# uzh-rpg/rpg_ramnet

Measured on AMD Instinct MI355X. Metric: depth samples/sec (346x260 cropped to 256x344, 5-bin grids, K=5 grids + 1 frame per sample; training step), higher is better.
Workload: dtype f32; 1 GPU; EventScape-shaped 346x260 -> 256x344 crop, 5 event bins, K=5, batch 8/GPU, seq-len 8, 1xMI355X-per-rank train, state=convgru, SI loss on [image,events4], Adam, backward-weights co-scheduled on a side stream, decoders on a second stream; global_batch=8, seq_len=8, parallelism=dp1

## Files before the change

include/ramnet_hip.h:

```cpp
#ifndef RAMNET_HIP_H
#define RAMNET_HIP_H
#include <stddef.h>
#include <stdint.h>

#ifdef __cplusplus
extern "C" {
#endif

#define RAMNET_ABI_VERSION 27
#define RAMNET_E_BADARG 10001
#define RAMNET_E_UNSUPPORTED 10002

enum ramnet_in_mode {
    RAMNET_IN_PLAIN = 0,
    RAMNET_IN_CAT = 1,
    RAMNET_IN_CAT_MUL = 2,
    RAMNET_IN_UP2X = 3,
    RAMNET_IN_UP2X_SKIP = 4,
    RAMNET_IN_RELUMASK = 5,
    RAMNET_IN_S2D = 6,
    RAMNET_IN_PARITY4 = 7
};

enum ramnet_algo { RAMNET_ALGO_DIRECT = 0, RAMNET_ALGO_WINOGRAD = 1, RAMNET_ALGO_HEAD = 2, RAMNET_ALGO_WINOGRAD24 = 3, RAMNET_ALGO_WINOGRAD_2X4 = 4,
                   RAMNET_ALGO_WINOGRAD_2X4_SPLIT = 5, RAMNET_ALGO_DIRECT_SPLIT = 6, RAMNET_ALGO_WINOGRAD24_2X3 = 7 };

enum ramnet_epilogue {
    RAMNET_EPI_LINEAR = 0,
    RAMNET_EPI_RELU = 1,
    RAMNET_EPI_SIGMOID = 2,
    RAMNET_EPI_RES_RELU = 3,
    RAMNET_EPI_GRU_BLEND = 4,
    RAMNET_EPI_LSTM = 5,
    RAMNET_EPI_GRU_BWD = 6,
    RAMNET_EPI_SIGMOID_HR = 7
};

typedef struct ramnet_conv_desc {
    const float *x0, *x1, *xm;
    int ld0, ld1, ldm;
    int C0, C1;
    int in_mode;
    int B, Hin, Win;
    int ntaps, stride;
    int8_t dy[25], dx[25];
    uint8_t wtap[25];
    const float *w;
    const float *bias;
    int Cout;
    int Ho, Wo;
    int HoF, WoF;
    int osy, osx, ooy, oox;
    int epi;
    float beta;
    const float *e0, *e1;
    int lde0, lde1;
    float *out, *o1, *o2;
    int ldo, ldo1, ldo2;
    int algo;
    int frame;
    int out_s2d;
    int head_cin;
    int s2d_5x5;
    float *splitk_ws;
    size_t splitk_floats;
    const int *active;
} ramnet_conv_desc;

#define RAMNET_WGRAD_MAX_SEGMENTS 48
typedef struct ramnet_wgrad_seg {
    const float *x0, *x1, *xm, *dout, *gmask;
} ramnet_wgrad_seg;

typedef struct ramnet_wgrad_desc {
    const float *x0, *x1, *xm;
    int ld0, ld1, ldm, C0, C1, in_mode;
    int B, Hin, Win;
    int ntaps, stride;
    int8_t dy[25], dx[25];
    const float *dout, *gmask;
    int ldg, ldgm;
    int Cout, Ho, Wo;
    float *dw;
    float *dbias;
    int algo;
    int gsy, gsx, goy, gox;
    int HoG, WoG;
    int head_cin;
    int dw_slabs;
    int nseg;
    const ramnet_wgrad_seg *segs;
} ramnet_wgrad_desc;

int ramnet_set_option(const char *name, int value);
int ramnet_get_option(const char *name);
const char *ramnet_last_error(void);
int ramnet_abi_version(void);
const char *ramnet_last_kernel(void);
int ramnet_stream_fork(void *from, void *to);

int ramnet_gemm(const float *A, const float *B, float *C, int M, int N, int K, int lda, int ldb, int ldc, int trans_a,
                int accumulate, int batch, long stride_a, long stride_b, long stride_c, void *stream);
int ramnet_gemm2(const float *A, const float *B, float *C, int M, long stride_a, long stride_b, long stride_c, int batch, const float *A2,
                 const float *B2, float *C2, int M2, long stride_a2, long stride_b2, long stride_c2, int batch2, int N, int K, int K2, int lda,
                 int ldb, int ldc, int trans_a, int accumulate, void *stream);

size_t ramnet_gemm_partial_floats(int M, int N, int K, int batch, int M2, int K2, int batch2);
int ramnet_gemm_ordered(const float *A, const float *B, float *C, int M, int N, int K, int lda, int ldb, int ldc, int trans_a, int batch,
                        long stride_a, long stride_b, long stride_c, float *partial, void *stream);
int ramnet_gemm2_ordered(const float *A, const float *B, float *C, int M, long stride_a, long stride_b, long stride_c, int batch, const float *A2,
                         const float *B2, float *C2, int M2, long stride_a2, long stride_b2, long stride_c2, int batch2, int N, int K, int K2,
                         int lda, int ldb, int ldc, int trans_a, float *partial, void *stream);

int ramnet_nchw_to_nhwc_pad(const float *src, float *dst, int B, int C, int H, int W, int Cpad, void *stream);
int ramnet_reflect_pad(const float *src, float *dst, int B, int C, int H, int W, int Cpad, int top, int left, int Hc, int Wc, int nhwc,
                       void *stream);
int ramnet_wgrad_wino_slabs(int Cin, int Cout);
int ramnet_wgrad_wino2x4_slabs(int Cin, int Cout);
int ramnet_wgrad_dsplit_slabs(int Cin, int Cout);
#define RAMNET_WGRAD_SLAB_CAP 64
int ramnet_wgrad_slabs(const ramnet_wgrad_desc *d);
size_t ramnet_wgrad_dsplit_ws_floats(int Cin, int Cout);
int ramnet_unpack_wgrad_dsplit(const float *ws, float *grad, int Cout, int Cin, int CinWs, int CoutWs, int n_off, void *stream);
size_t ramnet_wgrad_wino2x4_ws_floats(int Cin, int Cout);
int ramnet_reduce_slabs(float *ws, int slabs, size_t n, void *stream);
size_t ramnet_packed_weight_elems(int Cout, int Cin, int KH, int KW, int transposed, int gates);
size_t ramnet_packed_weight_elems_wino(int Cout, int Cin, int transposed, int gates);
int ramnet_pack_weight_wino(const float *w_oihw, float *wp, int Cout, int Cin, int transposed, int gates, void *stream);
size_t ramnet_packed_weight_elems_wino2x4(int Cout, int Cin, int transposed);
int ramnet_pack_weight_wino2x4(const float *w_oihw, float *wp, int Cout, int Cin, int transposed, void *stream);
size_t ramnet_packed_weight_elems_wino2x4_gates(int Cout, int Cin, int transposed, int gates);
int ramnet_pack_weight_wino2x4_gates(const float *w_oihw, float *wp, int Cout, int Cin, int transposed, int gates, void *stream);
int ramnet_conv_wino_variant(const ramnet_conv_desc *d, int force);
int ramnet_conv_wino_split_ok(const ramnet_conv_desc *d, int force);
size_t ramnet_packed_weight_elems_wino2x4_split(int Cout, int Cin, int transposed);
int ramnet_pack_weight_wino2x4_split(const float *w_oihw, float *wp, int Cout, int Cin, int transposed, void *stream);
size_t ramnet_conv_splitk_floats(const ramnet_conv_desc *d);
int ramnet_wino2x4_config(int min_wgs);
int ramnet_fold_wino_supported(int Cout, int Cin);
size_t ramnet_packed_weight_elems_fold_wino(int Cout, int Cin);
int ramnet_pack_weight_fold_wino(const float *w_oihw, float *wp, int Cout, int Cin, void *stream);
int ramnet_pack_weight_fold_wino_dgrad(const float *w_oihw, float *wp, int Cout, int Cin, void *stream);
int ramnet_pack_border_weights(const float *w_oihw, float *rows, float *cols, float *rows_t, float *cols_t, int Cout, int Cin, void *stream);
int ramnet_fold_wino_variant(const ramnet_conv_desc *d, int force);
size_t ramnet_packed_weight_elems_fold_wino2x3(int Cout, int Cin);
int ramnet_pack_weight_fold_wino2x3(const float *w_oihw, float *wp, int Cout, int Cin, void *stream);
int ramnet_pack_weight_fold_wino2x3_dgrad(const float *w_oihw, float *wp, int Cout, int Cin, void *stream);
int ramnet_fold_unpack_wgrad(float *w4, float *dU, float *wr, float *wc, float *grad, int Cout, int Cin, int CinWs, void *stream);
int ramnet_fold_wgrad_variant(const ramnet_wgrad_desc *d, int force);
int ramnet_fold_unpack_wgrad2x3(float *w4, float *dU, float *dU3, float *wr, float *wc, float *grad, int Cout, int Cin, int CinWs, void *stream);
size_t ramnet_packed_weight_elems_head(int Cin);
int ramnet_head_supported(int Cin, int Cout);
int ramnet_pack_weight_head(const float *w_oihw, float *wp, int Cout, int Cin, void *stream);
int ramnet_pack_weight(const float *w_oihw, float *wp, int Cout, int Cin, int KH, int KW,
                       int transposed, int gates, void *stream);
int ramnet_unpack_wgrad(const float *ws, float *grad_oihw, int Cout, int Cin, int CinWs, int CoutWs, int n_off,
                        int KH, int KW, void *stream);

int ramnet_unpack_wgrad_wino(const float *ws, float *grad_oihw, int Cout, int Cin, int CinWs, int CoutWs, int n_off,
                             void *stream);
int ramnet_unpack_wgrad_wino2x4(const float *ws, float *grad_oihw, int Cout, int Cin, int CinWs, int CoutWs, int n_off,
                                void *stream);

int ramnet_conv_launch(const ramnet_conv_desc *d, void *stream);
int ramnet_conv_launch_multi(const ramnet_conv_desc *descs, int n, void *stream);
int ramnet_wgrad_launch(const ramnet_wgrad_desc *d, void *stream);

int ramnet_pred_sigmoid_fwd(const float *x, int ldx, int C, const float *w, const float *b, float *y,
                            size_t npix, void *stream);
int ramnet_pred_sigmoid_bwd(const float *x, int ldx, int C, const float *w, const float *y, const float *dy,
                            float *dx, int lddx, float *dw, float *db, size_t npix, void *stream);
#define RAMNET_PRED_SI_MAX_SEGMENTS 8
size_t ramnet_pred_si_scratch_doubles(size_t seg_pix, int nseg);
int ramnet_pred_sigmoid_si_fwd(const float *x, int ldx, int C, const float *w, const float *b, float *y, size_t seg_pix, int nseg,
                               const float *const *targets, float weight, float lambda, double *scratch, double *stats, float *loss,
                               void *stream);
int ramnet_pred_sigmoid_si_bwd(const float *x, int ldx, int C, const float *w, const float *y, const float *dy, size_t seg_pix, int nseg,
                               const float *const *targets, const double *stats, const float *gscale, float weight, float lambda,
                               float *dx, int lddx, float *dw, float *db, double *scratch, int mask_x, void *stream);
int ramnet_pred_linear_fwd(const float *x, int ldx, int C, const float *w, const float *b, float *z, size_t npix, void *stream);
int ramnet_pred_linear_bwd(const float *x, int ldx, int C, const float *w, const float *dz, float *dx, int lddx, float *dw, float *db,
                           size_t npix, void *stream);
int ramnet_pred_sigmoid_dgrad(int C, const float *w, const float *y, const float *dy, float *dx, int lddx, size_t npix, void *stream);
int ramnet_pred_linear_dgrad(int C, const float *w, const float *dz, float *dx, int lddx, size_t npix, void *stream);
int ramnet_pred_sigmoid_si_dgrad(const float *x, int ldx, int C, const float *w, const float *y, const float *dy, size_t seg_pix, int nseg,
                                 const float *const *targets, const double *stats, const float *gscale, float weight, float lambda,
                                 float *dx, int lddx, int mask_x, void *stream);
int ramnet_relu_bwd(const float *dy, const float *y, float *dx, size_t n, void *stream);
int ramnet_pad2_sum(const float *x, const float *skip, float *out, int B, int H, int W, int C, void *stream);
int ramnet_up2x_border_im2col(const float *x, const float *skip, float *rows, float *cols, int B, int H, int W, int C, void *stream);
int ramnet_pad2_sum_im2col(const float *x, const float *skip, float *out, float *rows, float *cols, int B, int H, int W, int C, void *stream);
int ramnet_unpad2_fold(const float *dxpad, float *dx, int B, int H, int W, int C, void *stream);
int ramnet_up2x_border_col2im(const float *rows, const float *cols, float *dx, int B, int H, int W, int C, void *stream);
int ramnet_frame_gather(const float *dy, const float *mask, float *rows, float *cols, int B, int H2, int W2, int C, void *stream);
int ramnet_space_to_depth2(const float *x, float *out, int B, int H, int W, int C, int inverse, void *stream);
int ramnet_upsample2x_bwd(const float *dup, float *dx, int B, int H, int W, int C, void *stream);
int ramnet_gru_bwd_a(const float *dhn, const float *ur, const float *o, const float *h, float *dpo,
                     float *dpur, float *dh, size_t npix, int C, int ld_dhn ,
                     void *stream);
int ramnet_gru_bwd_a2(const float *dhn, const float *ur, const float *o, const float *h, float *dpo,
                      float *dpur, float *dh, size_t npix, int C, int ld_dhn, int ld_dh ,
                      void *stream);
int ramnet_gru_bwd_b(const float *dxhr, const float *ur, const float *h, float *dpur, float *dh,
                     size_t npix, int C, void *stream);
int ramnet_lstm_bwd(const float *gates, const float *cprev, const float *cnew, const float *dhn,
                    const float *dcn, float *dpre, float *dcprev, size_t npix, int C, void *stream);
int ramnet_lstm_bwd_masked(const float *gates, const float *cprev, const float *cnew, const float *dhn, const float *dcn,
                           const int *active, float *dpre, float *dcprev, float *dxh, size_t npix, int hw, int C, void *stream);
int ramnet_bias_grad(const float *dy, const float *mask, float *db, size_t npix, int C, void *stream);
size_t ramnet_bias_grad_partial_floats(int C);
int ramnet_bias_grad_ordered(const float *dy, const float *mask, float *db, size_t npix, int C, float *partial, void *stream);
size_t ramnet_pred_bwd_partial_floats(void);
int ramnet_pred_sigmoid_bwd_ordered(const float *x, int ldx, int C, const float *w, const float *y, const float *dy, float *dx, int lddx,
                                    float *dw, float *db, size_t npix, float *partial, void *stream);
int ramnet_pred_linear_bwd_ordered(const float *x, int ldx, int C, const float *w, const float *dz, float *dx, int lddx, float *dw, float *db,
                                   size_t npix, float *partial, void *stream);
int ramnet_norm_slabs(int groups, long npix, int C);
int ramnet_norm_partial(const float *a, int lda, const float *y, int ldy, int act, const float *b, int ldb, int groups, long npix,
                        int C, int nslab, double *part, void *stream);
int ramnet_norm_finalize(const double *part, int groups, int nslab, int C, long npix, double eps, const float *gamma, const float *beta,
                         float *running_mean, float *running_var, double momentum, int update_running, int use_running,
                         long long *num_batches_tracked, double *mean, double *rstd, float *scale, float *shift, void *stream);
int ramnet_norm_finalize_bwd(const double *part, int groups, int nslab, int C, long npix, const double *mean, const double *rstd,
                             const float *gamma, int batch_stats, float *c1, float *c2, float *c3, float *dgamma, float *dbeta, void *stream);
int ramnet_norm_apply(const float *x, int ldx, const float *scale, const float *shift, const float *res, int ldr, int act, float *out,
                      int ldo, int groups, long npix, int C, void *stream);
int ramnet_norm_bwd(const float *dy, int lddy, const float *y, int ldy, int act, const float *x, int ldx, const float *c1, const float *c2,
                    const float *c3, float *dx, int lddx, float *dres, int lddres, int groups, long npix, int C, void *stream);
int ramnet_add(const float *a, const float *b, float *y, size_t n, void *stream);
int ramnet_concat2(const float *a, int lda, int Ca, const float *b, int ldb, int Cb, float *y, size_t npix, void *stream);
int ramnet_cat_batch_add(const float *const *parts, int n, size_t npix, int C, int ld, const float *base, float *out, void *stream);
int ramnet_cat_batch_add_masked(const float *const *parts, int n, size_t npix, int C, int ld, const float *base, const float *mask, float *out,
                                void *stream);
int ramnet_split2(const float *y, int ldy, int Ca, int Cb, float *a, float *b, size_t npix, void *stream);

int ramnet_si_loss_fwd(const float *pred, const float *target, size_t n, float weight, float lambda,
                       double *stats, float *loss, void *stream);
int ramnet_si_loss_from_stats(const double *stats, float weight, float lambda, float *loss, void *stream);
int ramnet_si_loss_bwd(const float *pred, const float *target, size_t n, float weight, float lambda,
                       const double *stats, const float *gscale, float *dpred, void *stream);

int ramnet_si_log_loss_fwd(const float *pred, const float *target, size_t n, float lambda, double *stats, float *loss, void *stream);
int ramnet_si_log_loss_bwd(const float *pred, const float *target, size_t n, float lambda, const double *stats, const float *gscale,
                           float *dpred, void *stream);
int ramnet_mse_loss_fwd(const float *pred, const float *target, int B, int H, int W, int half, double *stats, float *loss, void *stream);
int ramnet_mse_loss_bwd(const float *pred, const float *target, int B, int H, int W, int half, const double *stats, const float *gscale,
                        float *dpred, void *stream);

int ramnet_depth_metrics(const float *pred, const float *target, size_t n, float clip_distance, float reg_factor,
                         float cutoff, double *out11, void *stream);

size_t ramnet_msg_workspace_elems(int B, int H, int W, int num_scales);
int ramnet_msg_loss_fwd(const float *pred, const float *target, int B, int H, int W, int num_scales, float *ws,
                        double *stats, float *loss, void *stream);
int ramnet_msg_loss_bwd(const float *ws, const double *stats, const float *gscale, int B, int H, int W, int num_scales,
                        float *dws, float *dpred, void *stream);

int ramnet_voxelize(const double *events, size_t n_events, int bins, int W, int H, float *grid, void *stream);
int ramnet_voxel_indices(const double *events, size_t n_events, int bins, int W, int H,
                         long long *idx_left, long long *idx_right, void *stream);
int ramnet_normalize_nonzero(float *grid, size_t n, double *scratch, void *stream);
int ramnet_voxelize_batch(const double *events, const long long *offsets, int n_grids, size_t max_events, int bins, int W, int H,
                          float *grids, void *stream);
int ramnet_normalize_nonzero_batch(float *grids, int n_grids, size_t n, double *scratch, void *stream);
int ramnet_nonzero_stats_batch(const float *grids, int n_grids, size_t n, double *stats, void *stream);

int ramnet_voxelize_batch_sorted(const double *events, const long long *offsets, int n_grids, size_t max_events, int bins, int W, int H,
                                 float *grids, void *stream);
size_t ramnet_nonzero_stats_scratch_doubles(int n_grids, size_t n);
int ramnet_nonzero_stats_batch_ordered(const float *grids, int n_grids, size_t n, double *stats, double *scratch, void *stream);
int ramnet_normalize_nonzero_batch_ordered(float *grids, int n_grids, size_t n, double *stats, double *scratch, void *stream);
int ramnet_normalize_nonzero_ordered(float *grid, size_t n, double *stats, double *scratch, void *stream);

int ramnet_augment_batch(const float *const *src, float *const *dst, const int *pidx, const float *theta, const int *win,
                         const int *win_host, const double *stats, const float *bx, const float *by, int G, int n_params, int C,
                         int H, int W, int th, int tw, int Cpad, int nhwc, void *stream);

#define RAMNET_BATCH_METRICS_TICKET_BYTES 262144
size_t ramnet_batch_metrics_workspace(int G, int N, size_t npix);
int ramnet_batch_metrics(const float *const *pred, const float *const *target, int G, int N, size_t npix, void *workspace,
                         double *out, void *stream);

#define RAMNET_EVAL_TABLE_TICKET_BYTES 262144
int ramnet_metric_depth(const float *y, size_t n, float clip_distance, float reg_factor, int clamp, float *out, void *stream);
size_t ramnet_eval_table_workspace(int G, size_t npix, int ncut, int has_mask);
int ramnet_eval_table(const float *const *pred, const float *const *target, const unsigned char *const *mask, int G, size_t npix,
                      float clip_distance, float reg_factor, const float *cutoffs, int ncut, void *workspace, double *out, void *stream);
#define RAMNET_EVAL_RESCALE 1
#define RAMNET_EVAL_TARGET_METRIC 2
size_t ramnet_eval_table_ex_workspace(int G, size_t npix, int ncut, int has_mask, int flags);
int ramnet_eval_table_ex(const float *const *pred, const float *const *target, const unsigned char *const *mask, int G, size_t npix,
                         float clip_distance, float reg_factor, const float *cutoffs, int ncut, int flags, void *workspace, double *out,
                         void *stream);
int ramnet_resize_metric_target(const float *const *target, int G, int H, int W, double scale_factor, float clip_distance, float reg_factor,
                                float *out, void *stream);

int ramnet_fill_pointer_table(const void **table, const void *const *host_ptrs, int n, void *stream);
size_t ramnet_grad_loss_workspace(int G, int B, int H, int W);
int ramnet_grad_loss_stats(const float *const *pred, const float *const *target, int G, int B, int H, int W, int num_scales,
                           void *workspace, double *stats, const float *weights, float *loss, float *wsum, void *stream);
int ramnet_grad_loss_from_stats(const double *stats, int G, int num_scales, double Bg, const double *Bg_dev, const float *weights,
                                float *loss, float *wsum, void *stream);
int ramnet_grad_loss_bwd(const float *const *pred, const float *const *target, int G, int B, int H, int W, int num_scales,
                         const double *stats, double Bg, const double *Bg_dev, double gain, const float *weights, const float *up,
                         const float *up_sum, float *dpred, void *stream);

#define RAMNET_RENDER_TICKET_BYTES 262144
#define RAMNET_RENDER_EVENTS 0
#define RAMNET_RENDER_FRAME 1
size_t ramnet_render_depth_workspace(int G, int n_scale, size_t npix);
int ramnet_render_depth(const float *const *maps, int G, int H, int W, double vmin, double vmax, const unsigned char *lut,
                        const float *const *scale_pred, const float *const *scale_target, int n_scale, float clip_distance,
                        float reg_factor, void *workspace, unsigned char *grey, unsigned char *color, double *scale, void *stream);
int ramnet_least_squares_scale(const float *const *pred, const float *const *target, int G, size_t npix, float clip_distance,
                               float reg_factor, void *workspace, double *scale, void *stream);
int ramnet_render_inputs(const float *const *inputs, const int *channels, const int *kinds, int G, int H, int W, unsigned char *rgb,
                         void *stream);

#ifdef __cplusplus
}
#endif
#endif
```

rpg_ramnet_amd/_hip.py:

```python
import ctypes as C
import os

_PKG = os.path.dirname(os.path.abspath(__file__))
LIB_PATH = os.environ.get("RAMNET_HIP_LIB") or os.path.join(_PKG, "librpg_ramnet_hip.so")

IN_PLAIN, IN_CAT, IN_CAT_MUL, IN_UP2X, IN_UP2X_SKIP, IN_RELUMASK, IN_S2D, IN_PARITY4 = range(8)
ALGO_DIRECT, ALGO_WINOGRAD, ALGO_HEAD, ALGO_WINOGRAD24, ALGO_WINOGRAD_2X4, ALGO_WINOGRAD_2X4_SPLIT, ALGO_DIRECT_SPLIT = 0, 1, 2, 3, 4, 5, 6
ALGO_WINOGRAD24_2X3 = 7
EPI_LINEAR, EPI_RELU, EPI_SIGMOID, EPI_RES_RELU, EPI_GRU_BLEND, EPI_LSTM, EPI_GRU_BWD, EPI_SIGMOID_HR = range(8)

_fp = C.c_void_p


class ConvDesc(C.Structure):
    _fields_ = [
        ("x0", _fp), ("x1", _fp), ("xm", _fp),
        ("ld0", C.c_int), ("ld1", C.c_int), ("ldm", C.c_int),
        ("C0", C.c_int), ("C1", C.c_int), ("in_mode", C.c_int),
        ("B", C.c_int), ("Hin", C.c_int), ("Win", C.c_int),
        ("ntaps", C.c_int), ("stride", C.c_int),
        ("dy", C.c_int8 * 25), ("dx", C.c_int8 * 25), ("wtap", C.c_uint8 * 25),
        ("w", _fp), ("bias", _fp),
        ("Cout", C.c_int), ("Ho", C.c_int), ("Wo", C.c_int), ("HoF", C.c_int), ("WoF", C.c_int),
        ("osy", C.c_int), ("osx", C.c_int), ("ooy", C.c_int), ("oox", C.c_int),
        ("epi", C.c_int), ("beta", C.c_float),
        ("e0", _fp), ("e1", _fp), ("lde0", C.c_int), ("lde1", C.c_int),
        ("out", _fp), ("o1", _fp), ("o2", _fp),
        ("ldo", C.c_int), ("ldo1", C.c_int), ("ldo2", C.c_int),
        ("algo", C.c_int),
        ("frame", C.c_int),
        ("out_s2d", C.c_int),
        ("head_cin", C.c_int),
        ("s2d_5x5", C.c_int),
        ("splitk_ws", C.c_void_p), ("splitk_floats", C.c_size_t),
        ("active", _fp),
    ]


class WgradSeg(C.Structure):
    _fields_ = [("x0", _fp), ("x1", _fp), ("xm", _fp), ("dout", _fp), ("gmask", _fp)]


WGRAD_MAX_SEGMENTS = 48


class WgradDesc(C.Structure):
    _fields_ = [
        ("x0", _fp), ("x1", _fp), ("xm", _fp),
        ("ld0", C.c_int), ("ld1", C.c_int), ("ldm", C.c_int),
        ("C0", C.c_int), ("C1", C.c_int), ("in_mode", C.c_int),
        ("B", C.c_int), ("Hin", C.c_int), ("Win", C.c_int),
        ("ntaps", C.c_int), ("stride", C.c_int),
        ("dy", C.c_int8 * 25), ("dx", C.c_int8 * 25),
        ("dout", _fp), ("gmask", _fp), ("ldg", C.c_int), ("ldgm", C.c_int),
        ("Cout", C.c_int), ("Ho", C.c_int), ("Wo", C.c_int),
        ("dw", _fp), ("dbias", _fp),
        ("algo", C.c_int),
        ("gsy", C.c_int), ("gsx", C.c_int), ("goy", C.c_int), ("gox", C.c_int), ("HoG", C.c_int), ("WoG", C.c_int),
        ("head_cin", C.c_int),
        ("dw_slabs", C.c_int),
        ("nseg", C.c_int), ("segs", C.POINTER(WgradSeg)),
    ]


_SIGS = {
    "ramnet_abi_version": (C.c_int, []),
    "ramnet_last_error": (C.c_char_p, []),
    "ramnet_set_option": (C.c_int, [C.c_char_p, C.c_int]),
    "ramnet_get_option": (C.c_int, [C.c_char_p]),
    "ramnet_last_kernel": (C.c_char_p, []),
    "ramnet_stream_fork": (C.c_int, [_fp, _fp]),
    "ramnet_gemm": (C.c_int, [_fp, _fp, _fp] + [C.c_int] * 9 + [C.c_long] * 3 + [_fp]),
    "ramnet_gemm2": (C.c_int, [_fp, _fp, _fp, C.c_int, C.c_long, C.c_long, C.c_long, C.c_int, _fp, _fp, _fp, C.c_int, C.c_long, C.c_long, C.c_long,
                               C.c_int, C.c_int, C.c_int, C.c_int, C.c_int, C.c_int, C.c_int, C.c_int, C.c_int, _fp]),
    "ramnet_nchw_to_nhwc_pad": (C.c_int, [_fp, _fp, C.c_int, C.c_int, C.c_int, C.c_int, C.c_int, _fp]),
    "ramnet_reflect_pad": (C.c_int, [_fp, _fp] + [C.c_int] * 10 + [_fp]),
    "ramnet_wgrad_wino_slabs": (C.c_int, [C.c_int, C.c_int]),
    "ramnet_wgrad_wino2x4_slabs": (C.c_int, [C.c_int, C.c_int]),
    "ramnet_wgrad_dsplit_slabs": (C.c_int, [C.c_int, C.c_int]),
    "ramnet_wgrad_dsplit_ws_floats": (C.c_size_t, [C.c_int, C.c_int]),
    "ramnet_unpack_wgrad_dsplit": (C.c_int, [_fp, _fp, C.c_int, C.c_int, C.c_int, C.c_int, C.c_int, _fp]),
    "ramnet_wgrad_wino2x4_ws_floats": (C.c_size_t, [C.c_int, C.c_int]),
    "ramnet_reduce_slabs": (C.c_int, [_fp, C.c_int, C.c_size_t, _fp]),
    "ramnet_packed_weight_elems": (C.c_size_t, [C.c_int] * 6),
    "ramnet_pack_weight": (C.c_int, [_fp, _fp, C.c_int, C.c_int, C.c_int, C.c_int, C.c_int, C.c_int, _fp]),
    "ramnet_packed_weight_elems_wino": (C.c_size_t, [C.c_int] * 4),
    "ramnet_pack_weight_wino": (C.c_int, [_fp, _fp, C.c_int, C.c_int, C.c_int, C.c_int, _fp]),
    "ramnet_packed_weight_elems_wino2x4": (C.c_size_t, [C.c_int] * 3),
    "ramnet_pack_weight_wino2x4": (C.c_int, [_fp, _fp, C.c_int, C.c_int, C.c_int, _fp]),
    "ramnet_packed_weight_elems_wino2x4_gates": (C.c_size_t, [C.c_int] * 4),
    "ramnet_pack_weight_wino2x4_gates": (C.c_int, [_fp, _fp, C.c_int, C.c_int, C.c_int, C.c_int, _fp]),
    "ramnet_wino2x4_config": (C.c_int, [C.c_int]),
    "ramnet_conv_wino_variant": (C.c_int, [C.POINTER(ConvDesc), C.c_int]),
    "ramnet_conv_wino_split_ok": (C.c_int, [C.POINTER(ConvDesc), C.c_int]),
    "ramnet_packed_weight_elems_wino2x4_split": (C.c_size_t, [C.c_int] * 3),
    "ramnet_pack_weight_wino2x4_split": (C.c_int, [_fp, _fp, C.c_int, C.c_int, C.c_int, _fp]),
    "ramnet_conv_splitk_floats": (C.c_size_t, [C.POINTER(ConvDesc)]),
    "ramnet_packed_weight_elems_head": (C.c_size_t, [C.c_int]),
    "ramnet_head_supported": (C.c_int, [C.c_int, C.c_int]),
    "ramnet_pack_weight_head": (C.c_int, [_fp, _fp, C.c_int, C.c_int, _fp]),
    "ramnet_fold_wino_supported": (C.c_int, [C.c_int, C.c_int]),
    "ramnet_packed_weight_elems_fold_wino": (C.c_size_t, [C.c_int, C.c_int]),
    "ramnet_pack_weight_fold_wino": (C.c_int, [_fp, _fp, C.c_int, C.c_int, _fp]),
    "ramnet_pack_weight_fold_wino_dgrad": (C.c_int, [_fp, _fp, C.c_int, C.c_int, _fp]),
    "ramnet_fold_wino_variant": (C.c_int, [C.POINTER(ConvDesc), C.c_int]),
    "ramnet_packed_weight_elems_fold_wino2x3": (C.c_size_t, [C.c_int, C.c_int]),
    "ramnet_pack_weight_fold_wino2x3": (C.c_int, [_fp, _fp, C.c_int, C.c_int, _fp]),
    "ramnet_pack_weight_fold_wino2x3_dgrad": (C.c_int, [_fp, _fp, C.c_int, C.c_int, _fp]),
    "ramnet_pack_border_weights": (C.c_int, [_fp] * 5 + [C.c_int, C.c_int, _fp]),
    "ramnet_fold_unpack_wgrad": (C.c_int, [_fp] * 5 + [C.c_int, C.c_int, C.c_int, _fp]),
    "ramnet_fold_unpack_wgrad2x3": (C.c_int, [_fp] * 6 + [C.c_int, C.c_int, C.c_int, _fp]),
    "ramnet_unpad2_fold": (C.c_int, [_fp, _fp, C.c_int, C.c_int, C.c_int, C.c_int, _fp]),
    "ramnet_up2x_border_col2im": (C.c_int, [_fp, _fp, _fp, C.c_int, C.c_int, C.c_int, C.c_int, _fp]),
    "ramnet_pad2_sum": (C.c_int, [_fp, _fp, _fp, C.c_int, C.c_int, C.c_int, C.c_int, _fp]),
    "ramnet_up2x_border_im2col": (C.c_int, [_fp, _fp, _fp, _fp, C.c_int, C.c_int, C.c_int, C.c_int, _fp]),
    "ramnet_pad2_sum_im2col": (C.c_int, [_fp, _fp, _fp, _fp, _fp, C.c_int, C.c_int, C.c_int, C.c_int, _fp]),
    "ramnet_space_to_depth2": (C.c_int, [_fp, _fp, C.c_int, C.c_int, C.c_int, C.c_int, C.c_int, _fp]),
    "ramnet_frame_gather": (C.c_int, [_fp, _fp, _fp, _fp, C.c_int, C.c_int, C.c_int, C.c_int, _fp]),
    "ramnet_unpack_wgrad": (C.c_int, [_fp, _fp] + [C.c_int] * 7 + [_fp]),
    "ramnet_unpack_wgrad_wino": (C.c_int, [_fp, _fp] + [C.c_int] * 5 + [_fp]),
    "ramnet_unpack_wgrad_wino2x4": (C.c_int, [_fp, _fp] + [C.c_int] * 5 + [_fp]),
    "ramnet_conv_launch": (C.c_int, [C.POINTER(ConvDesc), _fp]),
    "ramnet_conv_launch_multi": (C.c_int, [C.POINTER(ConvDesc), C.c_int, _fp]),
    "ramnet_wgrad_launch": (C.c_int, [C.POINTER(WgradDesc), _fp]),
    "ramnet_fold_wgrad_variant": (C.c_int, [C.POINTER(WgradDesc), C.c_int]),
    "ramnet_pred_sigmoid_fwd": (C.c_int, [_fp, C.c_int, C.c_int, _fp, _fp, _fp, C.c_size_t, _fp]),
    "ramnet_pred_sigmoid_bwd": (C.c_int, [_fp, C.c_int, C.c_int, _fp, _fp, _fp, _fp, C.c_int, _fp, _fp, C.c_size_t, _fp]),
    "ramnet_pred_si_scratch_doubles": (C.c_size_t, [C.c_size_t, C.c_int]),
    "ramnet_pred_sigmoid_si_fwd": (C.c_int, [_fp, C.c_int, C.c_int, _fp, _fp, _fp, C.c_size_t, C.c_int, C.POINTER(C.c_void_p), C.c_float, C.c_float,
                                             _fp, _fp, _fp, _fp]),
    "ramnet_pred_sigmoid_si_bwd": (C.c_int, [_fp, C.c_int, C.c_int, _fp, _fp, _fp, C.c_size_t, C.c_int, C.POINTER(C.c_void_p), _fp, _fp, C.c_float,
                                             C.c_float, _fp, C.c_int, _fp, _fp, _fp, C.c_int, _fp]),
    "ramnet_pred_linear_fwd": (C.c_int, [_fp, C.c_int, C.c_int, _fp, _fp, _fp, C.c_size_t, _fp]),
    "ramnet_pred_linear_bwd": (C.c_int, [_fp, C.c_int, C.c_int, _fp, _fp, _fp, C.c_int, _fp, _fp, C.c_size_t, _fp]),
    "ramnet_pred_sigmoid_dgrad": (C.c_int, [C.c_int, _fp, _fp, _fp, _fp, C.c_int, C.c_size_t, _fp]),
    "ramnet_pred_linear_dgrad": (C.c_int, [C.c_int, _fp, _fp, _fp, C.c_int, C.c_size_t, _fp]),
    "ramnet_pred_sigmoid_si_dgrad": (C.c_int, [_fp, C.c_int, C.c_int, _fp, _fp, _fp, C.c_size_t, C.c_int, C.POINTER(C.c_void_p), _fp, _fp, C.c_float,
                                               C.c_float, _fp, C.c_int, C.c_int, _fp]),
    "ramnet_cat_batch_add": (C.c_int, [_fp, C.c_int, C.c_size_t, C.c_int, C.c_int, _fp, _fp, _fp]),
    "ramnet_cat_batch_add_masked": (C.c_int, [_fp, C.c_int, C.c_size_t, C.c_int, C.c_int, _fp, _fp, _fp, _fp]),
    "ramnet_relu_bwd": (C.c_int, [_fp, _fp, _fp, C.c_size_t, _fp]),
    "ramnet_upsample2x_bwd": (C.c_int, [_fp, _fp, C.c_int, C.c_int, C.c_int, C.c_int, _fp]),
    "ramnet_gru_bwd_a": (C.c_int, [_fp] * 7 + [C.c_size_t, C.c_int, C.c_int, _fp]),
    "ramnet_gru_bwd_a2": (C.c_int, [_fp] * 7 + [C.c_size_t, C.c_int, C.c_int, C.c_int, _fp]),
    "ramnet_gru_bwd_b": (C.c_int, [_fp] * 5 + [C.c_size_t, C.c_int, _fp]),
    "ramnet_lstm_bwd": (C.c_int, [_fp] * 7 + [C.c_size_t, C.c_int, _fp]),
    "ramnet_lstm_bwd_masked": (C.c_int, [_fp, _fp, _fp, _fp, _fp, _fp, _fp, _fp, _fp, C.c_size_t, C.c_int, C.c_int, _fp]),
    "ramnet_norm_slabs": (C.c_int, [C.c_int, C.c_long, C.c_int]),
    "ramnet_norm_partial": (C.c_int, [_fp, C.c_int, _fp, C.c_int, C.c_int, _fp, C.c_int, C.c_int, C.c_long, C.c_int, C.c_int, _fp, _fp]),
    "ramnet_norm_finalize": (C.c_int, [_fp, C.c_int, C.c_int, C.c_int, C.c_long, C.c_double, _fp, _fp, _fp, _fp, C.c_double, C.c_int, C.c_int,
                                       _fp, _fp, _fp, _fp, _fp, _fp]),
    "ramnet_norm_finalize_bwd": (C.c_int, [_fp, C.c_int, C.c_int, C.c_int, C.c_long, _fp, _fp, _fp, C.c_int, _fp, _fp, _fp, _fp, _fp, _fp]),
    "ramnet_norm_apply": (C.c_int, [_fp, C.c_int, _fp, _fp, _fp, C.c_int, C.c_int, _fp, C.c_int, C.c_int, C.c_long, C.c_int, _fp]),
    "ramnet_norm_bwd": (C.c_int, [_fp, C.c_int, _fp, C.c_int, C.c_int, _fp, C.c_int, _fp, _fp, _fp, _fp, C.c_int, _fp, C.c_int,
                                  C.c_int, C.c_long, C.c_int, _fp]),
    "ramnet_add": (C.c_int, [_fp, _fp, _fp, C.c_size_t, _fp]),
    "ramnet_split2": (C.c_int, [_fp, C.c_int, C.c_int, C.c_int, _fp, _fp, C.c_size_t, _fp]),
    "ramnet_concat2": (C.c_int, [_fp, C.c_int, C.c_int, _fp, C.c_int, C.c_int, _fp, C.c_size_t, _fp]),
    "ramnet_bias_grad": (C.c_int, [_fp, _fp, _fp, C.c_size_t, C.c_int, _fp]),
    "ramnet_si_loss_fwd": (C.c_int, [_fp, _fp, C.c_size_t, C.c_float, C.c_float, _fp, _fp, _fp]),
    "ramnet_si_loss_from_stats": (C.c_int, [_fp, C.c_float, C.c_float, _fp, _fp]),
    "ramnet_si_loss_bwd": (C.c_int, [_fp, _fp, C.c_size_t, C.c_float, C.c_float, _fp, _fp, _fp, _fp]),
    "ramnet_si_log_loss_fwd": (C.c_int, [_fp, _fp, C.c_size_t, C.c_float, _fp, _fp, _fp]),
    "ramnet_si_log_loss_bwd": (C.c_int, [_fp, _fp, C.c_size_t, C.c_float, _fp, _fp, _fp, _fp]),
    "ramnet_mse_loss_fwd": (C.c_int, [_fp, _fp, C.c_int, C.c_int, C.c_int, C.c_int, _fp, _fp, _fp]),
    "ramnet_mse_loss_bwd": (C.c_int, [_fp, _fp, C.c_int, C.c_int, C.c_int, C.c_int, _fp, _fp, _fp, _fp]),
    "ramnet_depth_metrics": (C.c_int, [_fp, _fp, C.c_size_t, C.c_float, C.c_float, C.c_float, _fp, _fp]),
    "ramnet_msg_workspace_elems": (C.c_size_t, [C.c_int] * 4),
    "ramnet_msg_loss_fwd": (C.c_int, [_fp, _fp, C.c_int, C.c_int, C.c_int, C.c_int, _fp, _fp, _fp, _fp]),
    "ramnet_msg_loss_bwd": (C.c_int, [_fp, _fp, _fp, C.c_int, C.c_int, C.c_int, C.c_int, _fp, _fp, _fp]),
    "ramnet_voxelize": (C.c_int, [_fp, C.c_size_t, C.c_int, C.c_int, C.c_int, _fp, _fp]),
    "ramnet_voxel_indices": (C.c_int, [_fp, C.c_size_t, C.c_int, C.c_int, C.c_int, _fp, _fp, _fp]),
    "ramnet_normalize_nonzero": (C.c_int, [_fp, C.c_size_t, _fp, _fp]),
    "ramnet_voxelize_batch": (C.c_int, [_fp, _fp, C.c_int, C.c_size_t, C.c_int, C.c_int, C.c_int, _fp, _fp]),
    "ramnet_normalize_nonzero_batch": (C.c_int, [_fp, C.c_int, C.c_size_t, _fp, _fp]),
    "ramnet_nonzero_stats_batch": (C.c_int, [_fp, C.c_int, C.c_size_t, _fp, _fp]),
    "ramnet_augment_batch": (C.c_int, [_fp] * 9 + [C.c_int] * 9 + [_fp]),
    "ramnet_batch_metrics_workspace": (C.c_size_t, [C.c_int, C.c_int, C.c_size_t]),
    "ramnet_batch_metrics": (C.c_int, [_fp, _fp, C.c_int, C.c_int, C.c_size_t, _fp, _fp, _fp]),
    "ramnet_metric_depth": (C.c_int, [_fp, C.c_size_t, C.c_float, C.c_float, C.c_int, _fp, _fp]),
    "ramnet_eval_table_workspace": (C.c_size_t, [C.c_int, C.c_size_t, C.c_int, C.c_int]),
    "ramnet_eval_table": (C.c_int, [_fp, _fp, _fp, C.c_int, C.c_size_t, C.c_float, C.c_float, C.POINTER(C.c_float), C.c_int, _fp, _fp, _fp]),
    "ramnet_eval_table_ex_workspace": (C.c_size_t, [C.c_int, C.c_size_t, C.c_int, C.c_int, C.c_int]),
    "ramnet_eval_table_ex": (C.c_int, [_fp, _fp, _fp, C.c_int, C.c_size_t, C.c_float, C.c_float, C.POINTER(C.c_float), C.c_int, C.c_int, _fp, _fp,
                                       _fp]),
    "ramnet_resize_metric_target": (C.c_int, [_fp, C.c_int, C.c_int, C.c_int, C.c_double, C.c_float, C.c_float, _fp, _fp]),
    "ramnet_fill_pointer_table": (C.c_int, [_fp, C.POINTER(C.c_void_p), C.c_int, _fp]),
    "ramnet_grad_loss_workspace": (C.c_size_t, [C.c_int] * 4),
    "ramnet_grad_loss_stats": (C.c_int, [_fp, _fp] + [C.c_int] * 5 + [_fp] * 6),
    "ramnet_grad_loss_from_stats": (C.c_int, [_fp, C.c_int, C.c_int, C.c_double, _fp, _fp, _fp, _fp, _fp]),
    "ramnet_grad_loss_bwd": (C.c_int, [_fp, _fp] + [C.c_int] * 5 + [_fp, C.c_double, _fp, C.c_double, _fp, _fp, _fp, _fp, _fp]),
    "ramnet_render_depth_workspace": (C.c_size_t, [C.c_int, C.c_int, C.c_size_t]),
    "ramnet_render_depth": (C.c_int, [_fp, C.c_int, C.c_int, C.c_int, C.c_double, C.c_double, _fp, _fp, _fp, C.c_int, C.c_float, C.c_float,
                                      _fp, _fp, _fp, _fp, _fp]),
    "ramnet_least_squares_scale": (C.c_int, [_fp, _fp, C.c_int, C.c_size_t, C.c_float, C.c_float, _fp, _fp, _fp]),
    "ramnet_render_inputs": (C.c_int, [_fp, C.POINTER(C.c_int), C.POINTER(C.c_int), C.c_int, C.c_int, C.c_int, _fp, _fp]),
    "ramnet_wgrad_slabs": (C.c_int, [C.POINTER(WgradDesc)]),
    "ramnet_gemm_partial_floats": (C.c_size_t, [C.c_int] * 7),
    "ramnet_gemm_ordered": (C.c_int, [_fp, _fp, _fp] + [C.c_int] * 8 + [C.c_long] * 3 + [_fp, _fp]),
    "ramnet_gemm2_ordered": (C.c_int, [_fp, _fp, _fp, C.c_int, C.c_long, C.c_long, C.c_long, C.c_int, _fp, _fp, _fp, C.c_int, C.c_long, C.c_long, C.c_long,
                                       C.c_int, C.c_int, C.c_int, C.c_int, C.c_int, C.c_int, C.c_int, C.c_int, _fp, _fp]),
    "ramnet_bias_grad_partial_floats": (C.c_size_t, [C.c_int]),
    "ramnet_bias_grad_ordered": (C.c_int, [_fp, _fp, _fp, C.c_size_t, C.c_int, _fp, _fp]),
    "ramnet_pred_bwd_partial_floats": (C.c_size_t, []),
    "ramnet_pred_sigmoid_bwd_ordered": (C.c_int, [_fp, C.c_int, C.c_int, _fp, _fp, _fp, _fp, C.c_int, _fp, _fp, C.c_size_t, _fp, _fp]),
    "ramnet_pred_linear_bwd_ordered": (C.c_int, [_fp, C.c_int, C.c_int, _fp, _fp, _fp, C.c_int, _fp, _fp, C.c_size_t, _fp, _fp]),
    "ramnet_voxelize_batch_sorted": (C.c_int, [_fp, _fp, C.c_int, C.c_size_t, C.c_int, C.c_int, C.c_int, _fp, _fp]),
    "ramnet_nonzero_stats_scratch_doubles": (C.c_size_t, [C.c_int, C.c_size_t]),
    "ramnet_nonzero_stats_batch_ordered": (C.c_int, [_fp, C.c_int, C.c_size_t, _fp, _fp, _fp]),
    "ramnet_normalize_nonzero_batch_ordered": (C.c_int, [_fp, C.c_int, C.c_size_t, _fp, _fp, _fp]),
    "ramnet_normalize_nonzero_ordered": (C.c_int, [_fp, C.c_size_t, _fp, _fp, _fp]),
}
EXPORTS = tuple(_SIGS)

_lib = None
_tracer = None


class _Traced:
    def __init__(self, l):
        self._l = l

    def __getattr__(self, name):
        fn = getattr(self._l, name)
        tr = _tracer
        if tr is None:
            return fn
        return lambda *a: tr(name, fn, a)


def set_tracer(fn):
    global _tracer
    _tracer = fn


class HipLibraryMissing(RuntimeError):
    pass


def lib():
    global _lib
    if _lib is None:
        if not os.path.exists(LIB_PATH):
            raise HipLibraryMissing(
                "%s not found: build it with `python -c 'import __graft_entry__ as g; g.build()'` "
                "(hipcc --offload-arch=gfx950). rpg_ramnet_amd has no CPU fallback." % LIB_PATH)
        import torch
        rt = os.path.join(os.path.dirname(torch.__file__), "lib", "libamdhip64.so")
        if os.path.exists(rt):
            C.CDLL(rt, mode=C.RTLD_GLOBAL)
        l = C.CDLL(LIB_PATH)
        for name, (res, args) in _SIGS.items():
            fn = getattr(l, name)
            fn.restype, fn.argtypes = res, args
        if l.ramnet_abi_version() != 27:
            raise RuntimeError("ABI version mismatch in %s" % LIB_PATH)
        _lib = l
    return _lib if _tracer is None else _Traced(_lib)


def check(code, what):
    if code != 0:
        msg = lib().ramnet_last_error()
        raise RuntimeError("%s failed (code %d): %s" % (what, code, msg.decode() if msg else "?"))
```

rpg_ramnet_amd/csrc/common.hpp:

```cpp
#pragma once
#include <hip/hip_runtime.h>
#include <stdint.h>
#include <stdio.h>
#include "../../include/ramnet_hip.h"

typedef float f32x16 __attribute__((ext_vector_type(16)));

namespace ramnet {

constexpr int CK = 16;
constexpr int LDP = CK + 4;
constexpr int TWID = 16;
constexpr int WCK = 32;

extern int g_opt_voxel_sorted, g_opt_fold_pair, g_opt_wgrad_blocks, g_opt_wgrad_wino_blocks, g_opt_wino_ksplit, g_opt_wgrad_wino_nf, g_opt_pred_si_cap, g_opt_pred_si_bwd_cap, g_opt_ordered_only;
void set_error(const char *fmt, ...);
void note_kernel(const char *fmt, ...);
int launch_wino(const ramnet_conv_desc &d, hipStream_t st);
size_t wino24_splitk_floats(const ramnet_conv_desc &d);
int launch_wino6(const ramnet_conv_desc &d, hipStream_t st);
int launch_wino6s(const ramnet_conv_desc &d, hipStream_t st);
int launch_head(const ramnet_conv_desc &d, hipStream_t st);
int launch_wino24(const ramnet_conv_desc &d, hipStream_t st);
int launch_wgrad_wino24(const ramnet_wgrad_desc &d, hipStream_t st);
int launch_head_wgrad(const ramnet_wgrad_desc &d, hipStream_t st);
int wgrad_wino24_splits(const ramnet_wgrad_desc &d);
int head_wgrad_slabs(const ramnet_wgrad_desc &d);
int launch_wgrad_wino(const ramnet_wgrad_desc &d, hipStream_t st);
int launch_wgrad_wino6(const ramnet_wgrad_desc &d, hipStream_t st);
int launch_wgrad_dsplit(const ramnet_wgrad_desc &d, hipStream_t st);

#define RAMNET_CHECK_ARG(cond)                                                        \
    do {                                                                              \
        if (!(cond)) {                                                                \
            ramnet::set_error("%s:%d: bad argument: %s", __FILE__, __LINE__, #cond);  \
            return RAMNET_E_BADARG;                                                   \
        }                                                                             \
    } while (0)

#define RAMNET_HIP(call)                                                                        \
    do {                                                                                        \
        hipError_t e_ = (call);                                                                 \
        if (e_ != hipSuccess) {                                                                 \
            ramnet::set_error("%s:%d: %s -> %s", __FILE__, __LINE__, #call, hipGetErrorString(e_)); \
            return (int)e_;                                                                     \
        }                                                                                       \
    } while (0)

#define RAMNET_LAUNCH_CHECK() RAMNET_HIP(hipGetLastError())

hipError_t allow_full_lds(const void *kernel);
#define RAMNET_FULL_LDS(kern) RAMNET_HIP(ramnet::allow_full_lds(reinterpret_cast<const void *>(kern)))

__device__ __forceinline__ float4 ld4(const float *p) { return *reinterpret_cast<const float4 *>(p); }
__device__ __forceinline__ void st4(float *p, float4 v) { *reinterpret_cast<float4 *>(p) = v; }
__device__ __forceinline__ float4 f4zero() { return make_float4(0.f, 0.f, 0.f, 0.f); }
__device__ __forceinline__ float4 f4add(float4 a, float4 b) { return make_float4(a.x + b.x, a.y + b.y, a.z + b.z, a.w + b.w); }
__device__ __forceinline__ float4 f4mul(float4 a, float4 b) { return make_float4(a.x * b.x, a.y * b.y, a.z * b.z, a.w * b.w); }
__device__ __forceinline__ float4 f4scale(float4 a, float s) { return make_float4(a.x * s, a.y * s, a.z * s, a.w * s); }
__device__ __forceinline__ float sigmoidf_(float x) { return __builtin_amdgcn_rcpf(1.0f + __expf(-x)); }
__device__ __forceinline__ float tanhf_(float x) { return 1.0f - 2.0f * __builtin_amdgcn_rcpf(1.0f + __expf(2.0f * x)); }

__device__ __forceinline__ auto wino_rsrc(const void *p, unsigned bytes) {
    const unsigned long long a = (unsigned long long)p;
    const unsigned lo = __builtin_amdgcn_readfirstlane((unsigned)a), hi = __builtin_amdgcn_readfirstlane((unsigned)(a >> 32));
    return __builtin_amdgcn_make_buffer_rsrc((void *)(((unsigned long long)hi << 32) | lo), (short)0, (int)bytes, 0x00020000);
}
constexpr unsigned WOOB = 0x7fffff00u;

struct InSrc {
    const float *x0, *x1, *xm;
    int ld0, ld1, ldm, C0, Cin, mode, Hin, Win;
};

__device__ __forceinline__ void up2x_coord(int d, int n_src, int &i0, int &i1, float &l1) {
    float s = fmaxf(0.5f * (float)d - 0.25f, 0.0f);
    i0 = (int)s;
    i1 = i0 + (i0 < n_src - 1 ? 1 : 0);
    l1 = s - (float)i0;
}

__device__ __forceinline__ float4 load_in4(const InSrc &s, int b, int iy, int ix, int c) {
    if ((unsigned)iy >= (unsigned)s.Hin || (unsigned)ix >= (unsigned)s.Win || c >= s.Cin) return f4zero();
    if (s.mode == RAMNET_IN_UP2X || s.mode == RAMNET_IN_UP2X_SKIP) {
        const int Hs = s.Hin >> 1, Ws = s.Win >> 1;
        int y0, y1, x0, x1;
        float ly, lx;
        up2x_coord(iy, Hs, y0, y1, ly);
        up2x_coord(ix, Ws, x0, x1, lx);
        const float hy = 1.0f - ly, hx = 1.0f - lx;
        const size_t r0 = ((size_t)b * Hs + y0) * Ws, r1 = ((size_t)b * Hs + y1) * Ws;
        float4 v00 = ld4(s.x0 + (r0 + x0) * s.ld0 + c), v01 = ld4(s.x0 + (r0 + x1) * s.ld0 + c);
        float4 v10 = ld4(s.x0 + (r1 + x0) * s.ld0 + c), v11 = ld4(s.x0 + (r1 + x1) * s.ld0 + c);
        if (s.mode == RAMNET_IN_UP2X_SKIP) {
            v00 = f4add(v00, ld4(s.x1 + (r0 + x0) * s.ld1 + c));
            v01 = f4add(v01, ld4(s.x1 + (r0 + x1) * s.ld1 + c));
            v10 = f4add(v10, ld4(s.x1 + (r1 + x0) * s.ld1 + c));
            v11 = f4add(v11, ld4(s.x1 + (r1 + x1) * s.ld1 + c));
        }
        float4 top = f4add(f4scale(v00, hx), f4scale(v01, lx));
        float4 bot = f4add(f4scale(v10, hx), f4scale(v11, lx));
        return f4add(f4scale(top, hy), f4scale(bot, ly));
    }
    const size_t pix = ((size_t)b * s.Hin + iy) * s.Win + ix;
    if (s.mode == RAMNET_IN_PLAIN) return ld4(s.x0 + pix * s.ld0 + c);
    if (s.mode == RAMNET_IN_RELUMASK) {
        float4 v = ld4(s.x0 + pix * s.ld0 + c), m = ld4(s.xm + pix * s.ldm + c);
        return make_float4(m.x > 0.f ? v.x : 0.f, m.y > 0.f ? v.y : 0.f, m.z > 0.f ? v.z : 0.f, m.w > 0.f ? v.w : 0.f);
    }
    if (c < s.C0) return ld4(s.x0 + pix * s.ld0 + c);
    float4 v = ld4(s.x1 + pix * s.ld1 + (c - s.C0));
    if (s.mode == RAMNET_IN_CAT_MUL) v = f4mul(v, ld4(s.xm + pix * s.ldm + (c - s.C0)));
    return v;
}

template <int QPP, int LDX, int NB, int NT>
__device__ __forceinline__ void stage_patch(float *__restrict__ patch, const InSrc &s, int b, int iy0, int ix0, int c0,
                                            int PH, int PW, int tid) {
    constexpr int PXS = LDX, QS = 4;
    const int nslots = PH * PW * QPP;
    if (s.mode == RAMNET_IN_UP2X || s.mode == RAMNET_IN_UP2X_SKIP) {
        for (int sl = tid; sl < nslots; sl += NT) {
            const int pix = sl / QPP, qd = sl - pix * QPP;
            const int py = pix / PW, px = pix - py * PW;
            st4(patch + pix * PXS + qd * QS, load_in4(s, b, iy0 + py, ix0 + px, c0 + qd * 4));
        }
        return;
    }
    const bool two = s.mode == RAMNET_IN_CAT_MUL || s.mode == RAMNET_IN_RELUMASK;
    for (int base = tid; base < nslots; base += NB * NT) {
        float4 v[NB], m[NB];
        int dst[NB];
        bool ok[NB], hasm[NB];
#pragma unroll
        for (int i = 0; i < NB; ++i) {
            const int sl = base + i * NT;
            const int pix = sl / QPP, qd = sl - pix * QPP;
            const int py = pix / PW, px = pix - py * PW;
            const int iy = iy0 + py, ix = ix0 + px, c = c0 + qd * 4;
            ok[i] = sl < nslots && (unsigned)iy < (unsigned)s.Hin && (unsigned)ix < (unsigned)s.Win && c < s.Cin;
            dst[i] = sl < nslots ? pix * PXS + qd * QS : -1;
            const size_t gp = ((size_t)b * s.Hin + iy) * s.Win + ix;
            const bool second = s.mode != RAMNET_IN_PLAIN && s.mode != RAMNET_IN_RELUMASK && c >= s.C0;
            const float *p0 = second ? s.x1 + gp * s.ld1 + (c - s.C0) : s.x0 + gp * s.ld0 + c;
            hasm[i] = two && (s.mode == RAMNET_IN_RELUMASK || second);
            const float *p1 = s.mode == RAMNET_IN_RELUMASK ? s.xm + gp * s.ldm + c : s.xm + gp * s.ldm + (c - s.C0);
            v[i] = ld4(ok[i] ? p0 : s.x0);
            if (two) m[i] = ld4(ok[i] && hasm[i] ? p1 : s.x0);
        }
#pragma unroll
        for (int i = 0; i < NB; ++i) {
            float4 r = v[i];
            if (two && hasm[i]) {
                if (s.mode == RAMNET_IN_RELUMASK)
                    r = make_float4(m[i].x > 0.f ? r.x : 0.f, m[i].y > 0.f ? r.y : 0.f, m[i].z > 0.f ? r.z : 0.f, m[i].w > 0.f ? r.w : 0.f);
                else
                    r = f4mul(r, m[i]);
            }
            if (!ok[i]) r = f4zero();
            if (dst[i] >= 0) st4(patch + dst[i], r);
        }
    }
}

template <int QPP, int NB, int NT>
struct PatchRegs {
    float4 v[NB], m[NB];
    unsigned okmask, mmask;

    __device__ __forceinline__ void load(const InSrc &s, int b, int iy0, int ix0, int c0, int PH, int PW, int tid) {
        const int nslots = PH * PW * QPP;
        const bool two = s.mode == RAMNET_IN_CAT_MUL || s.mode == RAMNET_IN_RELUMASK;
        okmask = 0, mmask = 0;
#pragma unroll
        for (int i = 0; i < NB; ++i) {
            const int sl = tid + i * NT;
            const int pix = sl / QPP, qd = sl - pix * QPP;
            const int py = pix / PW, px = pix - py * PW;
            const int iy = iy0 + py, ix = ix0 + px, c = c0 + qd * 4;
            const bool ok = sl < nslots && (unsigned)iy < (unsigned)s.Hin && (unsigned)ix < (unsigned)s.Win && c < s.Cin;
            const size_t gp = ((size_t)b * s.Hin + iy) * s.Win + ix;
            const bool second = s.mode != RAMNET_IN_PLAIN && s.mode != RAMNET_IN_RELUMASK && c >= s.C0;
            const float *p0 = second ? s.x1 + gp * s.ld1 + (c - s.C0) : s.x0 + gp * s.ld0 + c;
            const bool hm = two && (s.mode == RAMNET_IN_RELUMASK || second);
            const float *p1 = s.mode == RAMNET_IN_RELUMASK ? s.xm + gp * s.ldm + c : s.xm + gp * s.ldm + (c - s.C0);
            v[i] = ld4(ok ? p0 : s.x0);
            m[i] = two ? ld4(ok && hm ? p1 : s.x0) : f4zero();
            okmask |= (ok ? 1u : 0u) << i;
            mmask |= (hm ? 1u : 0u) << i;
        }
    }

    __device__ __forceinline__ float4 value(const InSrc &s, int i) const {
        float4 r = v[i];
        if ((mmask >> i) & 1u) {
            if (s.mode == RAMNET_IN_RELUMASK)
                r = make_float4(m[i].x > 0.f ? r.x : 0.f, m[i].y > 0.f ? r.y : 0.f, m[i].z > 0.f ? r.z : 0.f, m[i].w > 0.f ? r.w : 0.f);
            else
                r = f4mul(r, m[i]);
        }
        if (!((okmask >> i) & 1u)) r = f4zero();
        return r;
    }

    template <int ROWF, int PS>
    __device__ __forceinline__ void store_planes(float *__restrict__ patch, const InSrc &s, int PH, int PW, int tid) const {
        const int nslots = PH * PW * QPP;
#pragma unroll
        for (int i = 0; i < NB; ++i) {
            const int sl = tid + i * NT;
            const float4 r = value(s, i);
            const int pix = sl / QPP, qd = sl - pix * QPP;
            const int py = pix / PW, px = pix - py * PW;
            if (sl < nslots) {
                float *d = patch + (2 * qd) * PS + py * ROWF + px * 2;
                *reinterpret_cast<float2 *>(d) = make_float2(r.x, r.y);
                *reinterpret_cast<float2 *>(d + PS) = make_float2(r.z, r.w);
            }
        }
    }

    template <int LDX>
    __device__ __forceinline__ void store(float *__restrict__ patch, const InSrc &s, int PH, int PW, int tid) const {
        const int nslots = PH * PW * QPP;
#pragma unroll
        for (int i = 0; i < NB; ++i) {
            const int sl = tid + i * NT;
            float4 r = v[i];
            if ((mmask >> i) & 1u) {
                if (s.mode == RAMNET_IN_RELUMASK)
                    r = make_float4(m[i].x > 0.f ? r.x : 0.f, m[i].y > 0.f ? r.y : 0.f, m[i].z > 0.f ? r.z : 0.f, m[i].w > 0.f ? r.w : 0.f);
                else
                    r = f4mul(r, m[i]);
            }
            if (!((okmask >> i) & 1u)) r = f4zero();
            if (sl < nslots) st4(patch + (sl / QPP) * LDX + (sl % QPP) * 4, r);
        }
    }
};

inline int cdiv(int a, int b) { return (a + b - 1) / b; }
inline int roundup(int a, int b) { return cdiv(a, b) * b; }

}
```

rpg_ramnet_amd/csrc/conv_wino24.hip:

```cpp
#include <stdlib.h>
#include "common.hpp"
#include "conv_plan.hpp"
#include "conv_epilogue.hpp"

typedef float f32x4 __attribute__((ext_vector_type(4)));

namespace ramnet {

constexpr int W24_PS = 512;
constexpr int W24_V = 25 * W24_PS;
constexpr int W23_V = 30 * W24_PS;

__device__ __forceinline__ float2 ld2f(const float *p) { return *reinterpret_cast<const float2 *>(p); }

__device__ __forceinline__ auto make_rsrc(const void *p, unsigned bytes) {
    const unsigned long long a = (unsigned long long)p;
    const unsigned lo = __builtin_amdgcn_readfirstlane((unsigned)a), hi = __builtin_amdgcn_readfirstlane((unsigned)(a >> 32));
    return __builtin_amdgcn_make_buffer_rsrc((void *)(((unsigned long long)hi << 32) | lo), (short)0, (int)bytes, 0x00020000);
}

#ifdef W24_TRACE
__device__ unsigned long long *g_w24_trace;
#define W24_STAMP(chunk_, slot)                                                                                          \
    do {                                                                                                                 \
        if (lane == 0 && (chunk_) <= 16) g_w24_trace[(((size_t)blockIdx.x * 8 + wave) * 17 + (chunk_)) * 6 + (slot)] = __builtin_amdgcn_s_memtime(); \
    } while (0)
#else
#define W24_STAMP(chunk_, slot)
#endif

struct Wino24Params {
    const float *x;
    const float *wp;
    int Hp, Wp, ldx, nchunks, nblk, tiles_x, tiles_y, Hc, Wc;
    int cpc;
    unsigned xbytes, wbytes;
    int ksplit;
    float *ws;
    int *cnt;
};

template <int NCQ, bool DG, int TXW, bool PAIR = false, int TW = 2>
__global__ void __launch_bounds__(512, 1) conv_wino24_kernel(const ramnet_conv_desc p, const Wino24Params q) {
    static_assert(!PAIR || (NCQ == 4 && !DG), "pair mode: forward, 64-column workgroups");
    static_assert(TW == 2 || (TW == 3 && NCQ == 4), "F(2x3): 64-column workgroups");
    constexpr int WC = TW + 3, NP = 5 * WC;
    constexpr int VSZ = NP * W24_PS;
    constexpr int W24_K = NCQ == 4 ? 16 : 8;
    constexpr int W24_TX = TXW, W24_TY = (NCQ == 4 ? 32 : 64) / TXW;
    constexpr int VEC = W24_K / 4;
    constexpr int W24_U = NP * NCQ * 64 * VEC;
    extern __shared__ __attribute__((aligned(16))) float smem[];
    float *V = smem;
    const int tid = threadIdx.x, lane = tid & 63;
    const int wave = __builtin_amdgcn_readfirstlane(tid >> 6);
    const int l15 = lane & 15, ks = lane >> 4;
    const int th = NCQ == 4 ? wave & 1 : wave & 3, cq = NCQ == 4 ? wave >> 1 : wave >> 2;

    int bid = blockIdx.x;
    const int cls = DG ? 0 : PAIR ? bid & 1 : bid & 3;
    if (!DG) bid >>= PAIR ? 1 : 2;
    const int nb = bid % q.nblk;
    bid /= q.nblk;
    const int tbx = bid % q.tiles_x;
    bid /= q.tiles_x;
    const int tby = bid % q.tiles_y, b = bid / q.tiles_y;
    const int py = PAIR ? cls : cls >> 1, px = PAIR ? 0 : cls & 1;
    const int n0 = nb * 16 * NCQ;

    const int it = tid / W24_K, ik = tid % W24_K;
    const int iy0 = 2 * (tby * W24_TY + it / W24_TX) + py, ix0 = TW * (tbx * W24_TX + it % W24_TX) + px;
    unsigned rowo[5], colo[WC];
    int cur_cls = -1;
    auto set_class = [&](int c) {
        cur_cls = c;
        const int cy = c >> 1, cx = c & 1;
        const int u0 = 2 * (tby * W24_TY + it / W24_TX), v0 = TW * (tbx * W24_TX + it % W24_TX);
#pragma unroll
        for (int r = 0; r < WC; ++r) {
            const int i = u0 - cy - 3 + r, j = v0 - cx - 3 + r;
            if (r < 5) rowo[r] = (unsigned)i < (unsigned)q.Hc ? 4u * (unsigned)((b * q.Hp + 2 * i + cy) * q.Wp * q.ldx) : 0x40000000u;
            colo[r] = (unsigned)j < (unsigned)q.Wc ? 4u * (unsigned)((2 * j + cx) * q.ldx + ik) : 0x40000000u;
        }
    };
    if (!DG) {
#pragma unroll
        for (int r = 0; r < WC; ++r) {
            if (r < 5) rowo[r] = 4u * (unsigned)((b * q.Hp + min(iy0 + r, q.Hp - 1)) * q.Wp * q.ldx);
            colo[r] = 4u * (unsigned)(min(ix0 + r, q.Wp - 1) * q.ldx + ik);
        }
    }
    const int ksp = (DG || TW != 2) ? 1 : q.ksplit;
    const int cps = ((q.nchunks / 2 + ksp - 1) / ksp) * 2, cbeg = DG ? 0 : (int)blockIdx.y * cps;
    const auto xrs = make_rsrc(q.x + cbeg * W24_K, q.xbytes - (unsigned)cbeg * W24_K * 4u);
    const int vdst = NCQ == 4 ? it * 16 + (((ik >> 2) ^ ((it >> 2) & 3)) << 2) + (ik & 3) : it * 8 + (((ik >> 1) ^ ((it >> 3) & 1)) << 1) + (ik & 1);
    float raw[5 * WC];
    auto load_raw = [&](int chunk) {
        int soff = chunk * (W24_K * 4);
        if (DG) {
            const int c = chunk / q.cpc;
            if (c != cur_cls) set_class(c);
            soff = (chunk - c * q.cpc) * (W24_K * 4);
        }
#pragma unroll
        for (int r = 0; r < 5; ++r)
#pragma unroll
            for (int c = 0; c < WC; ++c)
                raw[r * WC + c] = __builtin_bit_cast(float, __builtin_amdgcn_raw_buffer_load_b32(xrs, (int)(rowo[r] + colo[c]), soff, 0));
    };
    int lr_soff = 0;
    auto load_row_begin = [&](int chunk) {
        lr_soff = chunk * (W24_K * 4);
        if (DG) {
            const int c = chunk / q.cpc;
            if (c != cur_cls) set_class(c);
            lr_soff = (chunk - c * q.cpc) * (W24_K * 4);
        }
    };
    auto load_row = [&](int r) {
#pragma unroll
        for (int c = 0; c < WC; ++c)
            raw[r * WC + c] = __builtin_bit_cast(float, __builtin_amdgcn_raw_buffer_load_b32(xrs, (int)(rowo[r] + colo[c]), lr_soff, 0));
    };
    auto tr_col = [&](int c) {
        const float d0 = raw[c], d1 = raw[WC + c], d2 = raw[2 * WC + c], d3 = raw[3 * WC + c], d4 = raw[4 * WC + c];
        raw[c] = 2.f * (d0 - d2) - d1 + d3;
        raw[WC + c] = d3 - d2 - 2.f * d1;
        raw[2 * WC + c] = 2.f * d1 - 3.f * d2 + d3;
        raw[3 * WC + c] = d3 - d1;
        raw[4 * WC + c] = 2.f * (d1 - d3) - d2 + d4;
    };
    auto tr_row = [&](float *vbuf, int i) {
        float *dst = TW == 2 ? vbuf + (i * WC) * W24_PS + vdst : vbuf + (i * WC) * W24_PS;
        if constexpr (TW == 2) {
            const float d0 = raw[i * 5], d1 = raw[i * 5 + 1], d2 = raw[i * 5 + 2], d3 = raw[i * 5 + 3], d4 = raw[i * 5 + 4];
            dst[0 * W24_PS] = 2.f * (d0 - d2) - d1 + d3;
            dst[1 * W24_PS] = d3 - d2 - 2.f * d1;
            dst[2 * W24_PS] = 2.f * d1 - 3.f * d2 + d3;
            dst[3 * W24_PS] = d3 - d1;
            dst[4 * W24_PS] = 2.f * (d1 - d3) - d2 + d4;
        } else {
            const float d0 = raw[i * 6], d1 = raw[i * 6 + 1], d2 = raw[i * 6 + 2], d3 = raw[i * 6 + 3], d4 = raw[i * 6 + 4], d5 = raw[i * 6 + 5];
            const float u = d3 - d1, v = d4 - d2;
            dst[0 * W24_PS] = fmaf(-1.25f, d2, fmaf(0.25f, d0, d4));
            dst[1 * W24_PS] = fmaf(-0.25f, d1 + d2, d3 + d4);
            dst[2 * W24_PS] = fmaf(0.25f, d1 - d2, d4 - d3);
            dst[3 * W24_PS] = fmaf(0.5f, u, v);
            dst[4 * W24_PS] = fmaf(-0.5f, u, v);
            dst[5 * W24_PS] = fmaf(-1.25f, d3, fmaf(0.25f, d1, d5));
        }
    };

    const int tile = th * 16 + l15;
    const int aoff = NCQ == 4 ? tile * 16 + ((ks ^ ((tile >> 2) & 3)) << 2) : tile * 8 + ((ks ^ ((tile >> 3) & 1)) << 1);
    constexpr int WPOS = NCQ * 64 * VEC;
    const auto wrs = make_rsrc(q.wp, q.wbytes);
    const int wsrc = (((cls * q.nchunks + cbeg) * q.nblk + nb) * W24_U + cq * (64 * VEC)) * 4;
    const int wlane = lane * VEC * 4;
    auto ldv = [&](const float *ptr) {
        if (VEC == 4) return ld4(ptr);
        const float2 t = ld2f(ptr);
        return make_float4(t.x, t.y, 0.f, 0.f);
    };
    auto ldw = [&](int soff) {
        if constexpr (VEC == 4) {
            return __builtin_bit_cast(float4, __builtin_amdgcn_raw_buffer_load_b128(wrs, wlane, soff, 0));
        } else {
            const float2 t = __builtin_bit_cast(float2, __builtin_amdgcn_raw_buffer_load_b64(wrs, wlane, soff, 0));
            return make_float4(t.x, t.y, 0.f, 0.f);
        }
    };
    const int wchunk = q.nblk * W24_U * 4;
    int abuf1 = VSZ + aoff, dbuf1 = VSZ + vdst;
    if constexpr (TW == 3) asm volatile("" : "+v"(abuf1), "+v"(dbuf1));

    f32x4 acc[NP];
#pragma unroll
    for (int i = 0; i < NP; ++i) acc[i] = f32x4{0.f, 0.f, 0.f, 0.f};

    const int nch = DG ? q.nchunks : min(cps, q.nchunks - cbeg);
    W24_STAMP(16, 0);
    load_raw(0);
    constexpr int RING = TW == 2 || DG ? 10 : 6, DIST = RING - 2;
    static_assert((2 * NP) % RING == 0, "ring slots repeat every chunk pair");
    float4 bq[RING];
#pragma unroll
    for (int i = 0; i < DIST; ++i) bq[i] = ldw(wsrc + i * (WPOS * 4));
#pragma unroll
    for (int c = 0; c < WC; ++c) tr_col(c);
#pragma unroll
    for (int i = 0; i < 5; ++i) tr_row(TW == 2 ? V : V + vdst, i);
    load_raw(min(1, nch - 1));
    __syncthreads();

    W24_STAMP(16, 1);
    for (int chunk0 = 0; chunk0 < nch; chunk0 += 2) {
#pragma unroll
        for (int half = 0; half < 2; ++half) {
            const int chunk = chunk0 + half;
            const float *vb = V + half * VSZ;
            float *vn = TW == 2 ? V + (half ^ 1) * VSZ : V + (half ? vdst : dbuf1);
            auto lda = [&](int pos) {
                if constexpr (TW == 2) return ldv(vb + pos * W24_PS + aoff);
                else return ldv(V + (half ? abuf1 : aoff) + pos * W24_PS);
            };
            const int cnext = min(chunk + 1, nch - 1), cnext2 = min(chunk + 2, nch - 1);
            const int wcur = wsrc + chunk * wchunk, wnext = wsrc + cnext * wchunk;
            W24_STAMP(chunk, 0);
            float4 aq[2][2];
            aq[0][0] = lda(0), aq[0][1] = lda(1);
#pragma unroll
            for (int pp = 0; pp < (NP + 1) / 2; ++pp) {
                const int pos = 2 * pp, g = half * NP + pos;
                const bool two = pos + 1 < NP;
                if (pos + 2 < NP) aq[(pp + 1) & 1][0] = lda(pos + 2);
                if (pos + 3 < NP) aq[(pp + 1) & 1][1] = lda(pos + 3);
                const float4 a0 = aq[pp & 1][0], a1 = aq[pp & 1][1];
#if !defined(W24_ABLATE) || !(W24_ABLATE & 2)
                bq[(g + DIST) % RING] = pos + DIST < NP ? ldw(wcur + (pos + DIST) * (WPOS * 4)) : ldw(wnext + (pos + DIST - NP) * (WPOS * 4));
                if (two) bq[(g + 1 + DIST) % RING] = pos + 1 + DIST < NP ? ldw(wcur + (pos + 1 + DIST) * (WPOS * 4)) : ldw(wnext + (pos + 1 + DIST - NP) * (WPOS * 4));
#endif
                const float4 b0 = bq[g % RING], b1 = bq[(g + 1) % RING];
                __builtin_amdgcn_sched_barrier(0);
                acc[pos] = __builtin_amdgcn_mfma_f32_16x16x4f32(a0.x, b0.x, acc[pos], 0, 0, 0);
                if (two) acc[pos + 1] = __builtin_amdgcn_mfma_f32_16x16x4f32(a1.x, b1.x, acc[pos + 1], 0, 0, 0);
                acc[pos] = __builtin_amdgcn_mfma_f32_16x16x4f32(a0.y, b0.y, acc[pos], 0, 0, 0);
                if (two) acc[pos + 1] = __builtin_amdgcn_mfma_f32_16x16x4f32(a1.y, b1.y, acc[pos + 1], 0, 0, 0);
                __builtin_amdgcn_sched_barrier(0);
                constexpr int R0 = 4 + WC;
                auto slot = [&](int sl) {
                    if (sl == 4) W24_STAMP(chunk, 1);
                    if (sl >= 4 && sl < R0) tr_col(sl - 4);
                    if (sl == R0) W24_STAMP(chunk, 2);
                    if (sl >= R0 && sl <= R0 + 8 && !((sl - R0) & 1)) tr_row(vn, (sl - R0) >> 1);
#if !defined(W24_ABLATE) || !(W24_ABLATE & 1)
                    if (sl == R0 + 1) load_row_begin(cnext2);
                    if (sl > R0 && sl <= R0 + 9 && ((sl - R0) & 1)) load_row((sl - R0 - 1) >> 1);
#endif
                    if (sl == R0 + 9) W24_STAMP(chunk, 3);
                };
                slot(2 * pp);
                __builtin_amdgcn_sched_barrier(0);
                if (VEC == 4) {
                    acc[pos] = __builtin_amdgcn_mfma_f32_16x16x4f32(a0.z, b0.z, acc[pos], 0, 0, 0);
                    if (two) acc[pos + 1] = __builtin_amdgcn_mfma_f32_16x16x4f32(a1.z, b1.z, acc[pos + 1], 0, 0, 0);
                    acc[pos] = __builtin_amdgcn_mfma_f32_16x16x4f32(a0.w, b0.w, acc[pos], 0, 0, 0);
                    if (two) acc[pos + 1] = __builtin_amdgcn_mfma_f32_16x16x4f32(a1.w, b1.w, acc[pos + 1], 0, 0, 0);
                }
                __builtin_amdgcn_sched_barrier(0);
                slot(2 * pp + 1);
                __builtin_amdgcn_sched_barrier(0);
            }
            W24_STAMP(chunk, 4);
            __syncthreads();
            W24_STAMP(chunk, 5);
        }
    }
    W24_STAMP(16, 2);

    const int ncol = n0 + cq * 16 + l15;
    const int pxc = PAIR ? ncol >> 5 : px, n = PAIR ? ncol & 31 : ncol;
    if (n >= p.Cout) return;
    const int epi = p.epi;
    const float bias_n = (!DG && p.bias) ? p.bias[n] : 0.f;
    const bool relu = epi == RAMNET_EPI_RELU;
    constexpr int NOUT = 8 * TW;
    float ov[NOUT];
    size_t op[NOUT];
    bool oo[NOUT];
#pragma unroll
    for (int r = 0; r < 4; ++r) {
        float s[2][WC];
#pragma unroll
        for (int j = 0; j < WC; ++j) {
            const float m0 = acc[j][r], m1 = acc[WC + j][r], m2 = acc[2 * WC + j][r], m3 = acc[3 * WC + j][r], m4 = acc[4 * WC + j][r];
            s[0][j] = m0 + m1 + m2 + m3;
            s[1][j] = m1 - m2 + 2.f * m3 + m4;
        }
#pragma unroll
        for (int a2 = 0; a2 < 2; ++a2) {
            if constexpr (TW == 2) {
                ov[(r * 2 + a2) * 2] = s[a2][0] + s[a2][1] + s[a2][2] + s[a2][3];
                ov[(r * 2 + a2) * 2 + 1] = s[a2][1] - s[a2][2] + 2.f * s[a2][3] + s[a2][4];
            } else {
                ov[(r * 2 + a2) * 3] = s[a2][0] + s[a2][1] + s[a2][2] + s[a2][3] + s[a2][4];
                ov[(r * 2 + a2) * 3 + 1] = fmaf(0.5f, s[a2][3] - s[a2][4], s[a2][1] - s[a2][2]);
                ov[(r * 2 + a2) * 3 + 2] = fmaf(0.25f, s[a2][3] + s[a2][4], s[a2][1] + s[a2][2]) + s[a2][5];
            }
        }
    }
    if (!DG && ksp > 1) {
        typedef unsigned u32x4 __attribute__((ext_vector_type(4)));
        constexpr int AUX_SC1 = 16;
        const auto wr = make_rsrc(q.ws + (size_t)blockIdx.x * ksp * 8192, (unsigned)(ksp * 8192 * 4));
#pragma unroll
        for (int i = 0; i < 4; ++i)
            __builtin_amdgcn_raw_buffer_store_b128(__builtin_bit_cast(u32x4, make_float4(ov[4 * i], ov[4 * i + 1], ov[4 * i + 2], ov[4 * i + 3])), wr,
                                                   (i * 512 + tid) * 16, (int)blockIdx.y * 32768, AUX_SC1);
        __builtin_amdgcn_fence(__ATOMIC_RELEASE, "workgroup");
        __syncthreads();
        if (tid == 0) {
            const int arrived = __hip_atomic_fetch_add(q.cnt + blockIdx.x, 1, __ATOMIC_RELAXED, __HIP_MEMORY_SCOPE_AGENT);
            if (arrived == ksp - 1) __hip_atomic_store(q.cnt + blockIdx.x, 0, __ATOMIC_RELAXED, __HIP_MEMORY_SCOPE_AGENT);
            reinterpret_cast<int *>(smem)[0] = arrived == ksp - 1;
        }
        __syncthreads();
        if (!reinterpret_cast<int *>(smem)[0]) return;
#pragma unroll
        for (int i = 0; i < 16; ++i) ov[i] = 0.f;
        for (int sp = 0; sp < ksp; ++sp)
#pragma unroll
            for (int i = 0; i < 4; ++i) {
                const float4 t = __builtin_bit_cast(float4, __builtin_amdgcn_raw_buffer_load_b128(wr, (i * 512 + tid) * 16, sp * 32768, AUX_SC1));
                ov[4 * i] += t.x, ov[4 * i + 1] += t.y, ov[4 * i + 2] += t.z, ov[4 * i + 3] += t.w;
            }
    }
#pragma unroll
    for (int r = 0; r < 4; ++r) {
        const int t = th * 16 + 4 * ks + r;
        const int oy0 = 2 * (tby * W24_TY + t / W24_TX), ox0 = TW * (tbx * W24_TX + t % W24_TX) - (PAIR ? pxc : 0);
#pragma unroll
        for (int a2 = 0; a2 < 2; ++a2) {
#pragma unroll
            for (int c2 = 0; c2 < TW; ++c2) {
                const int oy = oy0 + a2, ox = ox0 + c2, idx = (r * 2 + a2) * TW + c2;
                if (DG) {
                    oo[idx] = oy < p.Ho && ox < p.Wo;
                    op[idx] = (((size_t)b * p.Ho + oy) * p.Wo + ox) * p.ldo + n;
                    continue;
                }
                oo[idx] = !(oy >= q.Hc || ox >= q.Wc || (PAIR && ox < 0));
                const int oyF = 2 * oy + py, oxF = 2 * ox + pxc;
                op[idx] = (((size_t)b * p.HoF + oyF) * p.WoF + oxF) * p.ldo + n;
                float v = ov[idx] + bias_n;
                if (oo[idx]) v += epilogue_side(p, epi, b, oyF, oxF, n);
                ov[idx] = relu ? fmaxf(v, 0.f) : v;
            }
        }
    }
#pragma unroll
    for (int idx = 0; idx < NOUT; ++idx)
        if (oo[idx]) p.out[op[idx]] = ov[idx];
    W24_STAMP(16, 3);
}

__device__ __forceinline__ int fold_wino_g6(int a, int t) {
    const int G6[5][4] = {{3, 0, 0, 0}, {-3, -3, -3, -3}, {-1, 1, -1, 1}, {1, 2, 4, 8}, {0, 0, 0, 6}};
    return G6[a][t];
}
__device__ __forceinline__ int fold_wino_gc3(int b, int s) {
    const int G3[6][4] = {{12, 0, 0, 0}, {2, 2, 2, 2}, {2, -2, 2, -2}, {-8, -4, -2, -1}, {-8, 4, -2, 1}, {0, 0, 0, 3}};
    return G3[b][s];
}
__device__ __forceinline__ int fold_fa4(int p, int t, int k) {
    const int FA4[2][4][5] = {{{1, 0, 0, 0, 0}, {3, 3, 1, 0, 0}, {0, 1, 3, 3, 1}, {0, 0, 0, 1, 3}}, {{3, 1, 0, 0, 0}, {1, 3, 3, 1, 0}, {0, 0, 1, 3, 3}, {0, 0, 0, 0, 1}}};
    return FA4[p][t][k];
}
__device__ __forceinline__ int fold_wino_gci(int tw, int b, int s) { return tw == 2 ? fold_wino_g6(b, s) : fold_wino_gc3(b, s); }
__device__ __forceinline__ float fold_wino_u(int tw, int a, int b, int py, int px, bool flip, const float *__restrict__ wk) {
    int ga[5], gb[5];
    for (int kh = 0; kh < 5; ++kh) {
        ga[kh] = 0, gb[kh] = 0;
        for (int t = 0; t < 4; ++t) {
            const int tt = flip ? 3 - t : t;
            ga[kh] += fold_wino_g6(a, t) * fold_fa4(py, tt, kh), gb[kh] += fold_wino_gci(tw, b, t) * fold_fa4(px, tt, kh);
        }
    }
    double u = 0;
    for (int kh = 0; kh < 5; ++kh)
        for (int kw = 0; kw < 5; ++kw) u += (double)(ga[kh] * gb[kw]) * (double)wk[kh * 5 + kw];
    return (float)(u / (tw == 2 ? 576.0 : 288.0));
}

template <int TW>
__global__ void pack_weight_fold_wino_kernel(const float *__restrict__ w, float *__restrict__ wp, int Cout, int Cin, int kc, int ncq,
                                             int pair, size_t total) {
    constexpr int WC = TW + 3, NP = 5 * WC;
    const int vec = kc / 4, nblk = pair ? 1 : Cout / (16 * ncq), nch = Cin / kc;
    for (size_t i = blockIdx.x * (size_t)blockDim.x + threadIdx.x; i < total; i += (size_t)gridDim.x * blockDim.x) {
        size_t r = i;
        const int j = (int)(r % vec);
        r /= vec;
        const int l15 = (int)(r % 16);
        r /= 16;
        const int ks = (int)(r % 4);
        r /= 4;
        const int cq = (int)(r % ncq);
        r /= ncq;
        const int pos = (int)(r % NP);
        r /= NP;
        const int nb = (int)(r % nblk);
        r /= nblk;
        const int chunk = (int)(r % nch), cls = (int)(r / nch);
        const int k = chunk * kc + ks * vec + j, col = (nb * ncq + cq) * 16 + l15;
        const int n = pair ? col & 31 : col;
        const int py = pair ? cls : cls >> 1, px = pair ? col >> 5 : cls & 1, a = pos / WC, b = pos % WC;
        wp[i] = fold_wino_u(TW, a, b, py, px, false, w + ((size_t)n * Cin + k) * 25);
    }
}

static bool fold_wino_pair(int Cout, int Cin) {
    return Cout == 32 && Cin % 32 == 0 && g_opt_fold_pair;
}

static bool fold_wino_geometry(int Cout, int Cin, int &kc, int &ncq) {
    kc = ((Cout % 64 == 0 && Cin % 16 == 0) || fold_wino_pair(Cout, Cin)) ? 16 : 8, ncq = kc == 16 ? 4 : 2;
    return Cout % 32 == 0 && Cin % (2 * kc) == 0;
}

static long wino23_tile(int Ho, int Wt, int &tx) {
    const int shapes[3] = {4, 2, 16};
    long best = -1;
    for (int s = 0; s < 3; ++s) {
        const int t = shapes[s], th = 2 * (32 / t), tw = 3 * t;
        const long a = (long)cdiv(Ho, th) * th * cdiv(Wt, tw) * tw;
        if (best < 0 || a < best) best = a, tx = t;
    }
    return best;
}

template <bool DG, bool PAIR>
static int launch_wino23(int tx, dim3 grid, size_t lds, const ramnet_conv_desc &d, const Wino24Params &q, hipStream_t st) {
#define W23_GO(T)                                                                                                         \
    if (tx == T) {                                                                                                        \
        RAMNET_FULL_LDS((conv_wino24_kernel<4, DG, T, PAIR, 3>));                                                           \
        note_kernel("conv_wino24_kernel<4,%d,%d,%d,3>", (int)DG, T, (int)PAIR);                                            \
        hipLaunchKernelGGL((conv_wino24_kernel<4, DG, T, PAIR, 3>), grid, dim3(512), lds, st, d, q);                        \
    }
    W23_GO(2) W23_GO(4) W23_GO(16)
#undef W23_GO
    RAMNET_LAUNCH_CHECK();
    return 0;
}

static int launch_wino24_dgrad(const ramnet_conv_desc &d, hipStream_t st) {
    RAMNET_CHECK_ARG(d.stride == 1 && d.C0 % 16 == 0 && d.Cout % 64 == 0);
    RAMNET_CHECK_ARG(d.Hin % 2 == 0 && d.Win % 2 == 0 && d.Ho == d.Hin / 2 + 4 && d.Wo == d.Win / 2 + 4 && d.HoF == d.Ho && d.WoF == d.Wo);
    RAMNET_CHECK_ARG(d.epi == RAMNET_EPI_LINEAR && !d.bias && d.beta == 0.f && d.frame == 0 && d.out_s2d == 0);
    Wino24Params q;
    q.x = d.x0, q.wp = d.w, q.Hp = d.Hin, q.Wp = d.Win, q.ldx = d.ld0;
    q.cpc = d.C0 / 16, q.nchunks = 4 * q.cpc, q.nblk = d.Cout / 64;
    q.ksplit = 1, q.ws = nullptr, q.cnt = nullptr;
    q.Hc = d.Hin / 2, q.Wc = d.Win / 2;
    const bool w23 = d.algo == RAMNET_ALGO_WINOGRAD24_2X3;
    const size_t xb = (size_t)d.B * d.Hin * d.Win * d.ld0 * sizeof(float), wb = (size_t)(w23 ? 120 : 100) * d.C0 * d.Cout * sizeof(float);
    RAMNET_CHECK_ARG(xb < 0x40000000ull && wb < 0x7fffffffull);
    q.xbytes = (unsigned)xb, q.wbytes = (unsigned)wb;
    if (w23) {
        int tx;
        wino23_tile(d.Ho, d.Wo, tx);
        q.tiles_x = cdiv(d.Wo, 3 * tx), q.tiles_y = cdiv(d.Ho, 64 / tx);
        return launch_wino23<true, false>(tx, dim3((unsigned)(q.tiles_x * q.tiles_y * d.B * q.nblk)), (size_t)2 * W23_V * sizeof(float), d, q, st);
    }
    const bool flat = cdiv(d.Wo, 16) * cdiv(d.Ho, 8) < cdiv(d.Wo, 8) * cdiv(d.Ho, 16);
    q.tiles_x = cdiv(d.Wo, flat ? 16 : 8), q.tiles_y = cdiv(d.Ho, flat ? 8 : 16);
    const size_t lds = (size_t)2 * W24_V * sizeof(float);
    const dim3 grid((unsigned)(q.tiles_x * q.tiles_y * d.B * q.nblk));
    if (flat) {
        RAMNET_FULL_LDS((conv_wino24_kernel<4, true, 8>));
        note_kernel("conv_wino24_kernel<4,1,8,0>");
        hipLaunchKernelGGL((conv_wino24_kernel<4, true, 8>), grid, dim3(512), lds, st, d, q);
    } else {
        RAMNET_FULL_LDS((conv_wino24_kernel<4, true, 4>));
        note_kernel("conv_wino24_kernel<4,1,4,0>");
        hipLaunchKernelGGL((conv_wino24_kernel<4, true, 4>), grid, dim3(512), lds, st, d, q);
    }
    RAMNET_LAUNCH_CHECK();
    return 0;
}

static int wino24_ksplit(const ramnet_conv_desc &d, int gridx, int nchunks) {
    if (!g_opt_wino_ksplit || d.in_mode != RAMNET_IN_PLAIN) return 1;
    const bool pair = fold_wino_pair(d.Cout, d.C0), wide = pair || (d.Cout % 64 == 0 && d.C0 % 16 == 0);
    if (!pair && d.Cout % (wide ? 64 : 32) != 0) return 1;
    int ks = 256 / gridx < 4 ? 256 / gridx : 4;
    if (nchunks / 4 < ks) ks = nchunks / 4;
    if (g_opt_wino_ksplit > 1) ks = g_opt_wino_ksplit < nchunks / 2 ? g_opt_wino_ksplit : nchunks / 2;
    if (ks < 1) ks = 1;
    while (ks > 1 && (ks - 1) * (cdiv(nchunks / 2, ks) * 2) >= nchunks) --ks;
    return ks;
}
static size_t wino24_ksplit_floats(unsigned gridx, int ks) { return (size_t)cdiv((int)gridx, 64) * 64 + (size_t)gridx * ks * 8192; }

size_t wino24_splitk_floats(const ramnet_conv_desc &d) {
    if (d.in_mode != RAMNET_IN_PLAIN || d.C0 % 16 != 0 || d.Cout % 32 != 0) return 0;
    const bool pair = fold_wino_pair(d.Cout, d.C0), wide = pair || (d.Cout % 64 == 0 && d.C0 % 16 == 0);
    if (d.C0 % (wide ? 32 : 16) != 0) return 0;
    const int nchunks = d.C0 / (wide ? 16 : 8), nblk = pair ? 1 : d.Cout / (wide ? 64 : 32);
    const int Wt = pair ? d.Wo + 2 : d.Wo;
    const bool flat = wide && cdiv(Wt, 16) * cdiv(d.Ho, 8) < cdiv(Wt, 8) * cdiv(d.Ho, 16);
    const int tiles_x = cdiv(Wt, wide && !flat ? 8 : 16), tiles_y = cdiv(d.Ho, flat ? 8 : 16);
    const unsigned gridx = (unsigned)(tiles_x * tiles_y * d.B * nblk * (pair ? 2 : 4));
    const int ks = wino24_ksplit(d, (int)gridx, nchunks);
    return ks > 1 ? wino24_ksplit_floats(gridx, ks) : 0;
}

static int fold_wino_variant(const ramnet_conv_desc &d, int force) {
    if (d.algo != RAMNET_ALGO_WINOGRAD24 || d.stride != 1) return 0;
    long wgs22, wgs23;
    int tx;
    if (d.in_mode == RAMNET_IN_PARITY4) {
        if (d.C0 % 16 != 0 || d.Cout % 64 != 0) return 0;
        const bool flat = cdiv(d.Wo, 16) * cdiv(d.Ho, 8) < cdiv(d.Wo, 8) * cdiv(d.Ho, 16);
        wgs22 = (long)cdiv(d.Wo, flat ? 16 : 8) * cdiv(d.Ho, flat ? 8 : 16) * d.B * (d.Cout / 64);
        wgs23 = wino23_tile(d.Ho, d.Wo, tx) / 192 * d.B * (d.Cout / 64);
    } else if (d.in_mode == RAMNET_IN_PLAIN) {
        const bool pair = fold_wino_pair(d.Cout, d.C0), wide = pair || (d.Cout % 64 == 0 && d.C0 % 16 == 0);
        if (!wide || d.C0 % 32 != 0 || d.Ho < 2 || d.Wo < 2) return 0;
        const int Wt = pair ? d.Wo + 2 : d.Wo, nblk = pair ? 1 : d.Cout / 64, ncls = pair ? 2 : 4;
        const bool flat = cdiv(Wt, 16) * cdiv(d.Ho, 8) < cdiv(Wt, 8) * cdiv(d.Ho, 16);
        wgs22 = (long)cdiv(Wt, flat ? 16 : 8) * cdiv(d.Ho, flat ? 8 : 16) * d.B * nblk * ncls;
        wgs23 = wino23_tile(d.Ho, pair ? d.Wo + 1 : d.Wo, tx) / 192 * d.B * nblk * ncls;
        if (!force && wino24_ksplit(d, (int)wgs22, d.C0 / 16) > 1) return 0;
    } else {
        return 0;
    }
    if (force) return 1;
    return wgs23 >= 256 && 6 * ((wgs23 + 255) / 256) < 5 * ((wgs22 + 255) / 256) ? 1 : 0;
}

int launch_wino24(const ramnet_conv_desc &d, hipStream_t st) {
    if (d.in_mode == RAMNET_IN_PARITY4) return launch_wino24_dgrad(d, st);
    RAMNET_CHECK_ARG(d.in_mode == RAMNET_IN_PLAIN && d.stride == 1);
    const bool pair = fold_wino_pair(d.Cout, d.C0);
    const bool wide = pair || (d.Cout % 64 == 0 && d.C0 % 16 == 0);
    RAMNET_CHECK_ARG(d.C0 % (wide ? 32 : 16) == 0);
    RAMNET_CHECK_ARG(d.C0 % 8 == 0 && d.Cout % 32 == 0 && d.Hin == d.Ho + 4 && d.Win == d.Wo + 4 && d.HoF == 2 * d.Ho && d.WoF == 2 * d.Wo);
    RAMNET_CHECK_ARG((d.epi == RAMNET_EPI_RELU || d.epi == RAMNET_EPI_LINEAR) && d.beta == 0.f && d.out_s2d == 0 && d.Ho >= 2 && d.Wo >= 2);
    const bool w23 = d.algo == RAMNET_ALGO_WINOGRAD24_2X3;
    if (w23) RAMNET_CHECK_ARG(wide && d.splitk_ws == nullptr);
    Wino24Params q;
    q.x = d.x0, q.wp = d.w, q.Hp = d.Hin, q.Wp = d.Win, q.ldx = d.ld0;
    q.nchunks = d.C0 / (wide ? 16 : 8), q.nblk = pair ? 1 : d.Cout / (wide ? 64 : 32);
    q.Hc = d.Ho, q.Wc = d.Wo, q.cpc = 1;
    const size_t xb = (size_t)d.B * d.Hin * d.Win * d.ld0 * sizeof(float), wb = (size_t)(w23 ? 120 : 100) * d.C0 * d.Cout * sizeof(float);
    RAMNET_CHECK_ARG(xb < 0xffffffffull && wb < 0x7fffffffull);
    q.xbytes = (unsigned)xb, q.wbytes = (unsigned)wb;
    if (w23) {
        int tx;
        wino23_tile(d.Ho, pair ? d.Wo + 1 : d.Wo, tx);
        q.tiles_x = cdiv(pair ? d.Wo + 1 : d.Wo, 3 * tx), q.tiles_y = cdiv(d.Ho, 64 / tx);
        q.ksplit = 1, q.ws = nullptr, q.cnt = nullptr;
        const dim3 grid((unsigned)(q.tiles_x * q.tiles_y * d.B * q.nblk * (pair ? 2 : 4)));
        const size_t lds = (size_t)2 * W23_V * sizeof(float);
        return pair ? launch_wino23<false, true>(tx, grid, lds, d, q, st) : launch_wino23<false, false>(tx, grid, lds, d, q, st);
    }
    const int Wt = pair ? d.Wo + 2 : d.Wo;
    const bool flat = wide && cdiv(Wt, 16) * cdiv(d.Ho, 8) < cdiv(Wt, 8) * cdiv(d.Ho, 16);
    q.tiles_x = cdiv(Wt, wide && !flat ? 8 : 16), q.tiles_y = cdiv(d.Ho, flat ? 8 : 16);
    const size_t lds = (size_t)2 * W24_V * sizeof(float);
    const unsigned gridx = (unsigned)(q.tiles_x * q.tiles_y * d.B * q.nblk * (pair ? 2 : 4));
    const int want = wino24_ksplit(d, (int)gridx, q.nchunks);
    q.ksplit = d.splitk_ws ? want : 1;
    q.cnt = reinterpret_cast<int *>(d.splitk_ws);
    q.ws = d.splitk_ws ? d.splitk_ws + cdiv((int)gridx, 64) * 64 : nullptr;
    if (q.ksplit > 1) RAMNET_CHECK_ARG(d.splitk_floats >= wino24_ksplit_floats(gridx, want) && ((uintptr_t)d.splitk_ws & 15) == 0);
    const dim3 grid(gridx, q.ksplit);
    if (pair && flat) {
        RAMNET_FULL_LDS((conv_wino24_kernel<4, false, 8, true>));
        note_kernel("conv_wino24_kernel<4,0,8,1>");
        hipLaunchKernelGGL((conv_wino24_kernel<4, false, 8, true>), grid, dim3(512), lds, st, d, q);
    } else if (pair) {
        RAMNET_FULL_LDS((conv_wino24_kernel<4, false, 4, true>));
        note_kernel("conv_wino24_kernel<4,0,4,1>");
        hipLaunchKernelGGL((conv_wino24_kernel<4, false, 4, true>), grid, dim3(512), lds, st, d, q);
    } else if (wide && flat) {
        RAMNET_FULL_LDS((conv_wino24_kernel<4, false, 8>));
        note_kernel("conv_wino24_kernel<4,0,8,0>");
        hipLaunchKernelGGL((conv_wino24_kernel<4, false, 8>), grid, dim3(512), lds, st, d, q);
    } else if (wide) {
        RAMNET_FULL_LDS((conv_wino24_kernel<4, false, 4>));
        note_kernel("conv_wino24_kernel<4,0,4,0>");
        hipLaunchKernelGGL((conv_wino24_kernel<4, false, 4>), grid, dim3(512), lds, st, d, q);
    } else {
        RAMNET_FULL_LDS((conv_wino24_kernel<2, false, 8>));
        note_kernel("conv_wino24_kernel<2,0,8,0>");
        hipLaunchKernelGGL((conv_wino24_kernel<2, false, 8>), grid, dim3(512), lds, st, d, q);
    }
    RAMNET_LAUNCH_CHECK();
    return 0;
}

template <int TW>
__global__ void pack_weight_fold_wino_dgrad_kernel(const float *__restrict__ w, float *__restrict__ wp, int Cout, int Cin, size_t total) {
    constexpr int WC = TW + 3, NP = 5 * WC;
    const int NB = Cin / 64;
    for (size_t i = blockIdx.x * (size_t)blockDim.x + threadIdx.x; i < total; i += (size_t)gridDim.x * blockDim.x) {
        size_t r = i;
        const int j = (int)(r & 3), l15 = (int)((r >> 2) & 15), ks = (int)((r >> 6) & 3), cq = (int)((r >> 8) & 3);
        r >>= 10;
        const int pos = (int)(r % NP);
        r /= NP;
        const int nb = (int)(r % NB), chunk = (int)(r / NB);
        const int k = chunk * 16 + ks * 4 + j, c = nb * 64 + cq * 16 + l15;
        const int pq = k / Cout, n = k - pq * Cout, pp = pq >> 1, qq = pq & 1, a = pos / WC, b = pos % WC;
        wp[i] = fold_wino_u(TW, a, b, pp, qq, true, w + ((size_t)n * Cin + c) * 25);
    }
}

__global__ void pack_border_weights_kernel(const float *__restrict__ w, float *__restrict__ rows, float *__restrict__ cols, float *__restrict__ rows_t,
                                           float *__restrict__ cols_t, int Cout, int Cin, size_t total) {
    for (size_t i = blockIdx.x * (size_t)blockDim.x + threadIdx.x; i < total; i += (size_t)gridDim.x * blockDim.x) {
        size_t r = i;
        const int co = (int)(r % Cout);
        r /= Cout;
        const int slot = (int)(r & 1);
        r >>= 1;
        const int ci = (int)(r % Cin);
        r /= Cin;
        const int kb = (int)(r % 5), side = (int)(r / 5);
        const int a0 = side == 0 ? 0 : (slot == 0 ? 4 : 3), na = side == 0 ? (slot == 0 ? 2 : 1) : (slot == 0 ? 1 : 2);
        const float *wk = w + ((size_t)co * Cin + ci) * 25;
        float sr = 0.f, sc = 0.f;
        for (int e = 0; e < na; ++e) sr += wk[(a0 + e) * 5 + kb], sc += wk[kb * 5 + (a0 + e)];
        const size_t K = (size_t)kb * Cin + ci, N = (size_t)slot * Cout + co;
        rows[((size_t)side * 5 * Cin + K) * 2 * Cout + N] = -sr;
        cols[((size_t)side * 5 * Cin + K) * 2 * Cout + N] = -sc;
        rows_t[((size_t)side * 2 * Cout + N) * 5 * Cin + K] = -sr;
        cols_t[((size_t)side * 2 * Cout + N) * 5 * Cin + K] = -sc;
    }
}

__global__ void fold_unpack_wgrad_kernel(float *__restrict__ w4, float *__restrict__ dU, float *__restrict__ dU3, float *__restrict__ wr,
                                         float *__restrict__ wc, float *__restrict__ grad, int Cout, int Cin, int CinWs) {
    const size_t total = (size_t)Cout * Cin;
    for (size_t idx = blockIdx.x * (size_t)blockDim.x + threadIdx.x; idx < total; idx += (size_t)gridDim.x * blockDim.x) {
        const int o = (int)(idx % Cout), i = (int)(idx / Cout);
        double g5[25];
        for (int e = 0; e < 25; ++e) g5[e] = 0.0;
        for (int pq = 0; pq < 4; ++pq) {
            const int pp = pq >> 1, qq = pq & 1;
            double d4[16];
            for (int ts = 0; ts < 16; ++ts) {
                float *cell = w4 + ((size_t)(pq * 16 + ts) * CinWs + i) * Cout + o;
                d4[ts] = 36.0 * (double)*cell;
                *cell = 0.f;
            }
            if (dU != nullptr) {
                for (int ab = 0; ab < 25; ++ab) {
                    float *cell = dU + ((size_t)(pq * 25 + ab) * CinWs + i) * Cout + o;
                    const double u = (double)*cell;
                    *cell = 0.f;
                    const int a = ab / 5, b = ab % 5;
                    for (int t = 0; t < 4; ++t)
                        for (int s = 0; s < 4; ++s) d4[t * 4 + s] += (double)(fold_wino_g6(a, t) * fold_wino_g6(b, s)) * u;
                }
            }
            if (dU3 != nullptr) {
                for (int ab = 0; ab < 30; ++ab) {
                    float *cell = dU3 + ((size_t)(pq * 30 + ab) * CinWs + i) * Cout + o;
                    const double u = (double)*cell;
                    *cell = 0.f;
                    const int a = ab / 6, b = ab % 6;
                    for (int t = 0; t < 4; ++t)
                        for (int s = 0; s < 4; ++s) d4[t * 4 + s] += (double)(2 * fold_wino_g6(a, t) * fold_wino_gc3(b, s)) * u;
                }
            }
            for (int t = 0; t < 4; ++t)
                for (int s = 0; s < 4; ++s) {
                    const double v = d4[t * 4 + s];
                    for (int k = 0; k < 5; ++k) {
                        const int fk = fold_fa4(pp, t, k);
                        if (fk == 0) continue;
                        for (int l = 0; l < 5; ++l) g5[k * 5 + l] += (double)(fk * fold_fa4(qq, s, l)) * v;
                    }
                }
        }
        for (int e = 0; e < 25; ++e) g5[e] /= 576.0;
        for (int side = 0; side < 2; ++side)
            for (int slot = 0; slot < 2; ++slot) {
                const int a0 = side == 0 ? 0 : (slot == 0 ? 4 : 3), na = side == 0 ? (slot == 0 ? 2 : 1) : (slot == 0 ? 1 : 2);
                for (int kb = 0; kb < 5; ++kb) {
                    float *rc = wr + (((size_t)side * 5 + kb) * Cin + i) * 2 * Cout + (size_t)slot * Cout + o;
                    float *cc = wc + (((size_t)side * 5 + kb) * Cin + i) * 2 * Cout + (size_t)slot * Cout + o;
                    const double r = (double)*rc, c = (double)*cc;
                    *rc = 0.f, *cc = 0.f;
                    for (int e = 0; e < na; ++e) g5[(a0 + e) * 5 + kb] -= r, g5[kb * 5 + (a0 + e)] -= c;
                }
            }
        float *g = grad + ((size_t)o * Cin + i) * 25;
        for (int e = 0; e < 25; ++e) g[e] = (float)((double)g[e] + g5[e]);
    }
}

}

using namespace ramnet;

extern "C" int ramnet_fold_wino_supported(int Cout, int Cin) {
    int kc, ncq;
    return fold_wino_geometry(Cout, Cin, kc, ncq) ? 1 : 0;
}

extern "C" size_t ramnet_packed_weight_elems_fold_wino(int Cout, int Cin) { return (size_t)100 * Cout * Cin; }

extern "C" int ramnet_pack_weight_fold_wino(const float *w, float *wp, int Cout, int Cin, void *stream) {
    int kc, ncq;
    RAMNET_CHECK_ARG(w && wp && Cout > 0 && Cin > 0 && fold_wino_geometry(Cout, Cin, kc, ncq));
    const size_t total = (size_t)100 * Cout * Cin;
    return launch_1d(pack_weight_fold_wino_kernel<2>, total, stream, w, wp, Cout, Cin, kc, ncq, (int)fold_wino_pair(Cout, Cin), total);
}

extern "C" int ramnet_pack_weight_fold_wino_dgrad(const float *w, float *wp, int Cout, int Cin, void *stream) {
    RAMNET_CHECK_ARG(w && wp && Cout > 0 && Cin > 0 && Cin % 64 == 0 && (4 * Cout) % 16 == 0);
    const size_t total = (size_t)100 * Cout * Cin;
    return launch_1d(pack_weight_fold_wino_dgrad_kernel<2>, total, stream, w, wp, Cout, Cin, total);
}

extern "C" size_t ramnet_packed_weight_elems_fold_wino2x3(int Cout, int Cin) { return (size_t)120 * Cout * Cin; }

extern "C" int ramnet_pack_weight_fold_wino2x3(const float *w, float *wp, int Cout, int Cin, void *stream) {
    int kc, ncq;
    RAMNET_CHECK_ARG(w && wp && Cout > 0 && Cin > 0 && fold_wino_geometry(Cout, Cin, kc, ncq) && kc == 16);
    const size_t total = (size_t)120 * Cout * Cin;
    return launch_1d(pack_weight_fold_wino_kernel<3>, total, stream, w, wp, Cout, Cin, kc, ncq, (int)fold_wino_pair(Cout, Cin), total);
}

extern "C" int ramnet_pack_weight_fold_wino2x3_dgrad(const float *w, float *wp, int Cout, int Cin, void *stream) {
    RAMNET_CHECK_ARG(w && wp && Cout > 0 && Cin > 0 && Cin % 64 == 0 && (4 * Cout) % 16 == 0);
    const size_t total = (size_t)120 * Cout * Cin;
    return launch_1d(pack_weight_fold_wino_dgrad_kernel<3>, total, stream, w, wp, Cout, Cin, total);
}

extern "C" int ramnet_fold_wino_variant(const ramnet_conv_desc *d, int force) { return d ? fold_wino_variant(*d, force) : 0; }

extern "C" int ramnet_pack_border_weights(const float *w, float *rows, float *cols, float *rows_t, float *cols_t, int Cout, int Cin, void *stream) {
    RAMNET_CHECK_ARG(w && rows && cols && rows_t && cols_t && Cout > 0 && Cin > 0);
    const size_t total = (size_t)2 * 5 * Cin * 2 * Cout;
    return launch_1d(pack_border_weights_kernel, total, stream, w, rows, cols, rows_t, cols_t, Cout, Cin, total);
}

extern "C" int ramnet_fold_unpack_wgrad(float *w4, float *dU, float *wr, float *wc, float *grad, int Cout, int Cin, int CinWs, void *stream) {
    RAMNET_CHECK_ARG(w4 && wr && wc && grad && Cout > 0 && Cin > 0 && CinWs >= Cin);
    const size_t total = (size_t)Cout * Cin;
    return launch_1d<128>(fold_unpack_wgrad_kernel, total, stream, w4, dU, (float *)nullptr, wr, wc, grad, Cout, Cin, CinWs);
}

extern "C" int ramnet_fold_unpack_wgrad2x3(float *w4, float *dU, float *dU3, float *wr, float *wc, float *grad, int Cout, int Cin, int CinWs,
                                           void *stream) {
    RAMNET_CHECK_ARG(w4 && wr && wc && grad && Cout > 0 && Cin > 0 && CinWs >= Cin);
    const size_t total = (size_t)Cout * Cin;
    return launch_1d<128>(fold_unpack_wgrad_kernel, total, stream, w4, dU, dU3, wr, wc, grad, Cout, Cin, CinWs);
}
```

rpg_ramnet_amd/csrc/pointwise.hip:

```cpp
#include <stdarg.h>
#include <mutex>
#include <unordered_map>
#include <unordered_set>
#include <stdlib.h>
#include <string.h>
#include "common.hpp"

namespace ramnet {

static thread_local char g_err[512] = "";
void set_error(const char *fmt, ...) {
    va_list ap;
    va_start(ap, fmt);
    vsnprintf(g_err, sizeof(g_err), fmt, ap);
    va_end(ap);
}

static thread_local char g_kernel[96] = "";
void note_kernel(const char *fmt, ...) {
    va_list ap;
    va_start(ap, fmt);
    vsnprintf(g_kernel, sizeof(g_kernel), fmt, ap);
    va_end(ap);
}
// ... 632 lines not shown
    return (i0 == src ? 1.0f - l1 : 0.f) + (i1 == src ? l1 : 0.f);
}

__global__ void upsample2x_bwd_kernel(const float *__restrict__ dup, float *__restrict__ dx, int B, int H, int W, int C) {
    const int C4 = C / 4;
    const size_t total = (size_t)B * H * W * C4;
    for (size_t i = blockIdx.x * (size_t)blockDim.x + threadIdx.x; i < total; i += (size_t)gridDim.x * blockDim.x) {
        const int c = (int)(i % C4) * 4;
        size_t j = i / C4;
        const int x = (int)(j % W);
        j /= W;
        const int y = (int)(j % H), b = (int)(j / H);
        float4 s = f4zero();
        for (int Y = 2 * y - 1; Y <= 2 * y + 2; ++Y) {
            if (Y < 0 || Y >= 2 * H) continue;
            const float wy = up2x_weight(Y, y, H);
            if (wy == 0.f) continue;
            for (int X = 2 * x - 1; X <= 2 * x + 2; ++X) {
                if (X < 0 || X >= 2 * W) continue;
                const float wgt = wy * up2x_weight(X, x, W);
                if (wgt == 0.f) continue;
                s = f4add(s, f4scale(ld4(dup + (((size_t)b * 2 * H + Y) * 2 * W + X) * C + c), wgt));
            }
        }
        st4(dx + i * 4, s);
    }
}

__device__ __forceinline__ void pad2_sum_item(const float *__restrict__ x, const float *__restrict__ skip, float *__restrict__ out, size_t i, int H,
                                              int W, int C) {
    const int C4 = C / 4, Hp = H + 4, Wp = W + 4;
    const int c = (int)(i % C4) * 4;
    size_t j = i / C4;
    const int xx = (int)(j % Wp);
    j /= Wp;
    const int yy = (int)(j % Hp), b = (int)(j / Hp);
    const int sy = min(max(yy - 2, 0), H - 1), sx = min(max(xx - 2, 0), W - 1);
    const size_t src = (((size_t)b * H + sy) * W + sx) * C + c;
    float4 v = ld4(x + src);
    if (skip) v = f4add(v, ld4(skip + src));
    st4(out + i * 4, v);
}

__global__ void pad2_sum_kernel(const float *__restrict__ x, const float *__restrict__ skip, float *__restrict__ out, int B, int H, int W, int C) {
    const size_t total = (size_t)B * (H + 4) * (W + 4) * (C / 4);
    for (size_t i = blockIdx.x * (size_t)blockDim.x + threadIdx.x; i < total; i += (size_t)gridDim.x * blockDim.x) pad2_sum_item(x, skip, out, i, H, W, C);
}

__device__ __forceinline__ float4 up2x_at(const float *__restrict__ x, const float *__restrict__ skip, int b, int H, int W, int C,
                                          int r, int c, int ch) {
    int y0, y1, x0, x1;
    float ly, lx;
    up2x_coord(r, H, y0, y1, ly);
    up2x_coord(c, W, x0, x1, lx);
    const float hy = 1.0f - ly, hx = 1.0f - lx;
    const size_t r0 = ((size_t)b * H + y0) * W, r1 = ((size_t)b * H + y1) * W;
    float4 v00 = ld4(x + (r0 + x0) * C + ch), v01 = ld4(x + (r0 + x1) * C + ch);
    float4 v10 = ld4(x + (r1 + x0) * C + ch), v11 = ld4(x + (r1 + x1) * C + ch);
    if (skip) {
        v00 = f4add(v00, ld4(skip + (r0 + x0) * C + ch)), v01 = f4add(v01, ld4(skip + (r0 + x1) * C + ch));
        v10 = f4add(v10, ld4(skip + (r1 + x0) * C + ch)), v11 = f4add(v11, ld4(skip + (r1 + x1) * C + ch));
    }
    const float4 top = f4add(f4scale(v00, hx), f4scale(v01, lx)), bot = f4add(f4scale(v10, hx), f4scale(v11, lx));
    return f4add(f4scale(top, hy), f4scale(bot, ly));
}

__device__ __forceinline__ void up2x_border_im2col_item(const float *__restrict__ x, const float *__restrict__ skip, float *__restrict__ rows,
                                                        float *__restrict__ cols, size_t i, int B, int H, int W, int C) {
    const int C4 = C / 4, H2 = 2 * H, W2 = 2 * W;
    const size_t nrows = (size_t)2 * B * W2 * 5 * C4;
    const bool isrow = i < nrows;
    size_t j = isrow ? i : i - nrows;
    const int ch = (int)(j % C4) * 4;
    j /= C4;
    const int k = (int)(j % 5);
    j /= 5;
    const int L = isrow ? W2 : H2;
    const int o = (int)(j % L);
    j /= L;
    const int b = (int)(j % B), side = (int)(j / B);
    float4 v = f4zero();
    if (isrow) {
        v = up2x_at(x, skip, b, H, W, C, side ? H2 - 1 : 0, min(max(o + k - 2, 0), W2 - 1), ch);
    } else {
        const int r = o + k - 2;
        if (r >= 0 && r < H2) v = up2x_at(x, skip, b, H, W, C, r, side ? W2 - 1 : 0, ch);
    }
    st4((isrow ? rows : cols) + (isrow ? i : i - nrows) * 4, v);
}

__global__ void up2x_border_im2col_kernel(const float *__restrict__ x, const float *__restrict__ skip, float *__restrict__ rows,
                                          float *__restrict__ cols, int B, int H, int W, int C) {
    const size_t n = (size_t)2 * B * (2 * W + 2 * H) * 5 * (C / 4);
    for (size_t i = blockIdx.x * (size_t)blockDim.x + threadIdx.x; i < n; i += (size_t)gridDim.x * blockDim.x)
        up2x_border_im2col_item(x, skip, rows, cols, i, B, H, W, C);
}

__global__ void pad2_sum_im2col_kernel(const float *__restrict__ x, const float *__restrict__ skip, float *__restrict__ out, float *__restrict__ rows,
                                       float *__restrict__ cols, int B, int H, int W, int C) {
    const size_t npad = (size_t)B * (H + 4) * (W + 4) * (C / 4), n = npad + (size_t)2 * B * (2 * W + 2 * H) * 5 * (C / 4);
    for (size_t i = blockIdx.x * (size_t)blockDim.x + threadIdx.x; i < n; i += (size_t)gridDim.x * blockDim.x) {
        if (i < npad) pad2_sum_item(x, skip, out, i, H, W, C);
        else up2x_border_im2col_item(x, skip, rows, cols, i - npad, B, H, W, C);
    }
}

__global__ void unpad2_fold_kernel(const float *__restrict__ dxpad, float *__restrict__ dx, int B, int H, int W, int C) {
    const int C4 = C / 4, Wp = W + 4;
    const size_t total = (size_t)B * H * W * C4;
    for (size_t idx = blockIdx.x * (size_t)blockDim.x + threadIdx.x; idx < total; idx += (size_t)gridDim.x * blockDim.x) {
        const int ch = (int)(idx % C4) * 4;
        size_t j = idx / C4;
        const int x = (int)(j % W);
        j /= W;
        const int y = (int)(j % H), b = (int)(j / H);
        const int y0 = y == 0 ? 0 : y + 2, y1 = y == H - 1 ? H + 3 : y + 2;
        const int x0 = x == 0 ? 0 : x + 2, x1 = x == W - 1 ? W + 3 : x + 2;
        float4 acc = f4zero();
        for (int r = y0; r <= y1; ++r)
            for (int c = x0; c <= x1; ++c) acc = f4add(acc, ld4(dxpad + (((size_t)b * (H + 4) + r) * Wp + c) * C + ch));
        st4(dx + idx * 4, acc);
    }
}

__global__ void up2x_border_col2im_kernel(const float *__restrict__ rows, const float *__restrict__ cols, float *__restrict__ dx, int B,
                                          int H, int W, int C, int part) {
    const int C4 = C / 4, H2 = 2 * H, W2 = 2 * W;
    const int L = part ? H : W, L2 = 2 * L;
    const float *src = part ? cols : rows;
    const size_t total = (size_t)2 * B * L * C4;
    for (size_t idx = blockIdx.x * (size_t)blockDim.x + threadIdx.x; idx < total; idx += (size_t)gridDim.x * blockDim.x) {
        const int ch = (int)(idx % C4) * 4;
        size_t t = idx / C4;
        const int j = (int)(t % L);
        t /= L;
        const int b = (int)(t % B), side = (int)(t / B);
        const float *line = src + ((size_t)(side * B + b) * L2) * 5 * C + ch;
        float4 acc = f4zero();
        for (int cu = max(2 * j - 1, 0); cu <= min(2 * j + 2, L2 - 1); ++cu) {
            int p0, p1;
            float l1;
            up2x_coord(cu, L, p0, p1, l1);
            const float wgt = (p0 == j ? 1.0f - l1 : 0.0f) + (p1 == j ? l1 : 0.0f);
            if (wgt == 0.0f) continue;
            float4 sum = f4zero();
            for (int k = 0; k < 5; ++k) {
                int olo = cu + 2 - k, ohi = olo;
                if (!part) {
                    if (cu == 0) olo = 0;
                    if (cu == L2 - 1) ohi = L2 - 1;
                }
                olo = max(olo, 0), ohi = min(ohi, L2 - 1);
                for (int o = olo; o <= ohi; ++o) sum = f4add(sum, ld4(line + ((size_t)o * 5 + k) * C));
            }
            acc = f4add(acc, f4scale(sum, wgt));
        }
        const int y = part ? j : (side ? H - 1 : 0), x = part ? (side ? W - 1 : 0) : j;
        float *dst = dx + (((size_t)b * H + y) * W + x) * C + ch;
        st4(dst, f4add(ld4(dst), acc));
    }
}

__global__ void frame_gather_kernel(const float *__restrict__ dy, const float *__restrict__ mask, float *__restrict__ rows,
                                    float *__restrict__ cols, int B, int H2, int W2, int C) {
    const int C4 = C / 4;
    const size_t nrows = (size_t)2 * B * W2 * 2 * C4, ncols = (size_t)2 * B * H2 * 2 * C4;
    for (size_t i = blockIdx.x * (size_t)blockDim.x + threadIdx.x; i < nrows + ncols; i += (size_t)gridDim.x * blockDim.x) {
        const bool isrow = i < nrows;
        size_t j = isrow ? i : i - nrows;
        const int ch = (int)(j % C4) * 4;
        j /= C4;
        const int slot = (int)(j % 2);
        j /= 2;
        const int L = isrow ? W2 : H2;
        const int o = (int)(j % L);
        j /= L;
        const int b = (int)(j % B), side = (int)(j / B);
        const int edge = side ? (isrow ? H2 : W2) - 2 + slot : slot;
        const int oy = isrow ? edge : o, ox = isrow ? o : edge;
        const size_t src = (((size_t)b * H2 + oy) * W2 + ox) * C + ch;
        float4 v = ld4(dy + src);
        if (mask) {
            const float4 m = ld4(mask + src);
            v = make_float4(m.x > 0.f ? v.x : 0.f, m.y > 0.f ? v.y : 0.f, m.z > 0.f ? v.z : 0.f, m.w > 0.f ? v.w : 0.f);
        }
        st4((isrow ? rows : cols) + (isrow ? i : i - nrows) * 4, v);
    }
}

__global__ void space_to_depth2_kernel(const float *__restrict__ x, float *__restrict__ out, int B, int Ho, int Wo, int C, int inverse) {
    const int C4 = C / 4;
    const size_t total = (size_t)B * Ho * Wo * 4 * C4;
    for (size_t i = blockIdx.x * (size_t)blockDim.x + threadIdx.x; i < total; i += (size_t)gridDim.x * blockDim.x) {
        const int ch = (int)(i % C4) * 4;
        size_t j = i / C4;
        const int par = (int)(j % 4);
        j /= 4;
        const int xx = (int)(j % Wo);
        j /= Wo;
        const int yy = (int)(j % Ho), b = (int)(j / Ho);
        const size_t deep = i * 4;
        const size_t flat = ((((size_t)b * 2 * Ho + 2 * yy + (par >> 1)) * 2 * Wo) + 2 * xx + (par & 1)) * C + ch;
        if (inverse) st4(out + flat, ld4(x + deep));
        else st4(out + deep, ld4(x + flat));
    }
}

__global__ void gru_bwd_a_kernel(const float *__restrict__ dhn, const float *__restrict__ ur, const float *__restrict__ o,
                                 const float *__restrict__ h, float *__restrict__ dpo, float *__restrict__ dpur,
                                 float *__restrict__ dh, size_t npix, int C, int ldg, int lddh) {
    const int C4 = C / 4;
    const size_t total = npix * C4;
    for (size_t i = blockIdx.x * (size_t)blockDim.x + threadIdx.x; i < total; i += (size_t)gridDim.x * blockDim.x) {
        const size_t pix = i / C4;
        const int c = (int)(i - pix * C4) * 4;
        const float4 g = ld4(dhn + pix * ldg + c), u = ld4(ur + pix * 2 * C + c), oo = ld4(o + pix * C + c);
        const float4 hh = h ? ld4(h + pix * C + c) : f4zero();
        float4 a, bq, d;
#define RN_ONE(f)                                   \
    a.f = g.f * u.f * (1.0f - oo.f * oo.f);         \
    bq.f = g.f * (oo.f - hh.f) * u.f * (1.0f - u.f); \
    d.f = g.f * (1.0f - u.f);
        RN_ONE(x) RN_ONE(y) RN_ONE(z) RN_ONE(w)
#undef RN_ONE
        st4(dpo + pix * C + c, a);
        st4(dpur + pix * 2 * C + c, bq);
        st4(dh + pix * lddh + c, d);
    }
}

__global__ void gru_bwd_b_kernel(float *__restrict__ dxhr, const float *__restrict__ ur, const float *__restrict__ h,
                                 float *__restrict__ dpur, const float *__restrict__ dh, size_t npix, int C) {
    const int C4 = C / 4;
    const size_t total = npix * C4;
    for (size_t i = blockIdx.x * (size_t)blockDim.x + threadIdx.x; i < total; i += (size_t)gridDim.x * blockDim.x) {
        const size_t pix = i / C4;
        const int c = (int)(i - pix * C4) * 4;
        const float4 dhr = ld4(dxhr + pix * 2 * C + C + c), r = ld4(ur + pix * 2 * C + C + c), d0 = ld4(dh + pix * C + c);
        const float4 hh = h ? ld4(h + pix * C + c) : f4zero();
        float4 pr, d;
#define RN_ONE(f)                                   \
    pr.f = dhr.f * hh.f * r.f * (1.0f - r.f);       \
    d.f = d0.f + dhr.f * r.f;
        RN_ONE(x) RN_ONE(y) RN_ONE(z) RN_ONE(w)
#undef RN_ONE
        st4(dpur + pix * 2 * C + C + c, pr);
        st4(dxhr + pix * 2 * C + C + c, d);
    }
}

template <bool MASK>
__global__ void lstm_bwd_kernel(const float *__restrict__ gates, const float *__restrict__ cprev, const float *__restrict__ cnew,
                                const float *__restrict__ dhn, const float *__restrict__ dcn, float *__restrict__ dpre,
                                float *__restrict__ dcprev, size_t npix, int C, const int *__restrict__ active = nullptr,
                                float *__restrict__ dxh = nullptr, int hw = 1) {
    const int C4 = C / 4;
    const size_t total = npix * C4;
    for (size_t i = blockIdx.x * (size_t)blockDim.x + threadIdx.x; i < total; i += (size_t)gridDim.x * blockDim.x) {
        const size_t pix = i / C4;
        const int c = (int)(i - pix * C4) * 4;
        const float *gp = gates + pix * 4 * C + c;
        const float4 dh = dhn ? ld4(dhn + pix * C + c) : f4zero(), dc = dcn ? ld4(dcn + pix * C + c) : f4zero();
        if (MASK) {
            const bool act = active[pix / (size_t)hw] != 0;
            st4(dxh + pix * 2 * C + c, f4zero());
            st4(dxh + pix * 2 * C + C + c, act ? f4zero() : dh);
            if (!act) {
                float *op = dpre + pix * 4 * C + c;
                st4(op, f4zero()), st4(op + C, f4zero()), st4(op + 2 * C, f4zero()), st4(op + 3 * C, f4zero());
                st4(dcprev + pix * C + c, dc);
                continue;
            }
        }
        const float4 gi = ld4(gp), gf = ld4(gp + C), go = ld4(gp + 2 * C), gc = ld4(gp + 3 * C);
        const float4 cp = cprev ? ld4(cprev + pix * C + c) : f4zero(), cn = ld4(cnew + pix * C + c);
        float4 pi, pf, po, pg, dp;
#define RN_ONE(f)                                                   \
    {                                                               \
        const float tc = tanhf_(cn.f);                               \
        const float dct = dc.f + dh.f * go.f * (1.0f - tc * tc);    \
        po.f = dh.f * tc * go.f * (1.0f - go.f);                    \
        pf.f = dct * cp.f * gf.f * (1.0f - gf.f);                   \
        pi.f = dct * gc.f * gi.f * (1.0f - gi.f);                   \
        pg.f = dct * gi.f * (1.0f - gc.f * gc.f);                   \
        dp.f = dct * gf.f;                                          \
    }
        RN_ONE(x) RN_ONE(y) RN_ONE(z) RN_ONE(w)
#undef RN_ONE
        float *op = dpre + pix * 4 * C + c;
        st4(op, pi), st4(op + C, pf), st4(op + 2 * C, po), st4(op + 3 * C, pg);
        st4(dcprev + pix * C + c, dp);
    }
}

}

using namespace ramnet;

extern "C" const char *ramnet_last_error(void) { return g_err; }
extern "C" const char *ramnet_last_kernel(void) { return g_kernel; }
extern "C" int ramnet_abi_version(void) { return RAMNET_ABI_VERSION; }

namespace ramnet {
int g_opt_voxel_sorted = 1, g_opt_fold_pair = 1, g_opt_wgrad_blocks = 512, g_opt_wgrad_wino_blocks = 384, g_opt_wino_ksplit = 1, g_opt_wgrad_wino_nf = 1, g_opt_pred_si_cap = 256, g_opt_pred_si_bwd_cap = 1024, g_opt_ordered_only = 0;
}
extern "C" int ramnet_set_option(const char *name, int value) {
    RAMNET_CHECK_ARG(name != nullptr);
    if (!strcmp(name, "voxel_sorted")) ramnet::g_opt_voxel_sorted = value != 0;
    else if (!strcmp(name, "fold_pair")) ramnet::g_opt_fold_pair = value != 0;
    else if (!strcmp(name, "wgrad_blocks")) { RAMNET_CHECK_ARG(value >= 1); ramnet::g_opt_wgrad_blocks = value; }
    else if (!strcmp(name, "wgrad_wino_nf")) { RAMNET_CHECK_ARG(value == 1 || value == 2); ramnet::g_opt_wgrad_wino_nf = value; }
    else if (!strcmp(name, "wino_ksplit")) { RAMNET_CHECK_ARG(value >= 0 && value <= 16); ramnet::g_opt_wino_ksplit = value; }
    else if (!strcmp(name, "wgrad_wino_blocks")) { RAMNET_CHECK_ARG(value >= 1 && value <= 384); ramnet::g_opt_wgrad_wino_blocks = value; }
    else if (!strcmp(name, "pred_si_bwd_cap")) { RAMNET_CHECK_ARG(value >= 8 && value <= 65536); ramnet::g_opt_pred_si_bwd_cap = value; }
    else if (!strcmp(name, "pred_si_cap")) { RAMNET_CHECK_ARG(value >= 8 && value <= 65536); ramnet::g_opt_pred_si_cap = value; }
    else if (!strcmp(name, "ordered_only")) ramnet::g_opt_ordered_only = value != 0;
    else RAMNET_CHECK_ARG(!"ramnet_set_option: unknown option");
    return 0;
}
extern "C" int ramnet_get_option(const char *name) {
    if (name == nullptr) return -1;
    if (!strcmp(name, "voxel_sorted")) return ramnet::g_opt_voxel_sorted;
    if (!strcmp(name, "fold_pair")) return ramnet::g_opt_fold_pair;
    if (!strcmp(name, "wgrad_blocks")) return ramnet::g_opt_wgrad_blocks;
    if (!strcmp(name, "wgrad_wino_blocks")) return ramnet::g_opt_wgrad_wino_blocks;
    if (!strcmp(name, "wino_ksplit")) return ramnet::g_opt_wino_ksplit;
    if (!strcmp(name, "wgrad_wino_nf")) return ramnet::g_opt_wgrad_wino_nf;
    if (!strcmp(name, "pred_si_bwd_cap")) return ramnet::g_opt_pred_si_bwd_cap;
    if (!strcmp(name, "pred_si_cap")) return ramnet::g_opt_pred_si_cap;
    if (!strcmp(name, "ordered_only")) return ramnet::g_opt_ordered_only;
    return -1;
}

extern "C" int ramnet_nchw_to_nhwc_pad(const float *src, float *dst, int B, int C, int H, int W, int Cpad, void *stream) {
    RAMNET_CHECK_ARG(src && dst && B > 0 && C > 0 && H > 0 && W > 0 && Cpad >= C && Cpad % 4 == 0);
    const size_t npix = (size_t)B * H * W;
    hipLaunchKernelGGL(nchw_to_nhwc_pad_kernel, dim3(grid_for(npix)), dim3(256), 0, (hipStream_t)stream, src, dst, B, C, H * W, Cpad);
    RAMNET_LAUNCH_CHECK();
    return 0;
}

extern "C" int ramnet_reflect_pad(const float *src, float *dst, int B, int C, int H, int W, int Cpad, int top, int left, int Hc, int Wc, int nhwc,
                                  void *stream) {
    RAMNET_CHECK_ARG(src && dst && B > 0 && C > 0 && H > 0 && W > 0 && top >= 0 && left >= 0 && Hc >= H + top && Wc >= W + left);
    RAMNET_CHECK_ARG(top < H && Hc - H - top < H && left < W && Wc - W - left < W);
    RAMNET_CHECK_ARG(!nhwc || (Cpad >= C && Cpad % 4 == 0));
    const size_t npix = (size_t)B * Hc * Wc;
    hipLaunchKernelGGL(reflect_pad_kernel, dim3(grid_for(npix)), dim3(256), 0, (hipStream_t)stream, src, dst, B, C, H, W, Cpad, top, left, Hc, Wc, nhwc);
    RAMNET_LAUNCH_CHECK();
    return 0;
}

static void pack_geometry(int Cout, int Cin, int transposed, int gates, int &R, int &N, int &nchunks, int &NPad) {
    R = transposed ? Cout : Cin;
    N = transposed ? Cin : Cout;
    nchunks = cdiv(R, CK);
    NPad = gates > 1 ? gates * roundup(N / gates, 32) : roundup(N, 32);
}

extern "C" size_t ramnet_packed_weight_elems(int Cout, int Cin, int KH, int KW, int transposed, int gates) {
    int R, N, nchunks, NPad;
    pack_geometry(Cout, Cin, transposed, gates, R, N, nchunks, NPad);
    return (size_t)KH * KW * nchunks * NPad * CK;
}

extern "C" int ramnet_pack_weight(const float *w, float *wp, int Cout, int Cin, int KH, int KW, int transposed, int gates, void *stream) {
    RAMNET_CHECK_ARG(w && wp && Cout > 0 && Cin > 0 && KH > 0 && KW > 0 && KH * KW <= 64);
    RAMNET_CHECK_ARG(gates == 1 || (gates == 4 && !transposed && Cout % 4 == 0));
    int R, N, nchunks, NPad;
    pack_geometry(Cout, Cin, transposed, gates, R, N, nchunks, NPad);
    const size_t total = (size_t)KH * KW * nchunks * NPad * CK;
    hipLaunchKernelGGL(pack_weight_kernel, dim3(grid_for(total)), dim3(256), 0, (hipStream_t)stream, w, wp, Cout, Cin, KH * KW,
                       transposed, gates, R, N, nchunks, NPad, total);
    RAMNET_LAUNCH_CHECK();
    return 0;
}

extern "C" int ramnet_unpack_wgrad(const float *ws, float *grad, int Cout, int Cin, int CinWs, int CoutWs, int n_off, int KH, int KW,
                                   void *stream) {
    RAMNET_CHECK_ARG(ws && grad && Cout > 0 && Cin > 0 && CinWs >= Cin && n_off >= 0 && CoutWs >= n_off + Cout);
    const size_t total = (size_t)Cout * Cin * KH * KW;
    hipLaunchKernelGGL(unpack_wgrad_kernel, dim3(grid_for(total)), dim3(256), 0, (hipStream_t)stream, ws, grad, Cout, Cin, CinWs, CoutWs, n_off, KH * KW, total);
    RAMNET_LAUNCH_CHECK();
    return 0;
}

struct CatParts {
    const float *p[8];
};
__global__ void cat_batch_add_kernel(const CatParts parts, int n, size_t npix, int C, int ld, const float *__restrict__ base,
                                     const float *__restrict__ mask, float *__restrict__ out) {
    const int C4 = C / 4;
    const size_t per = npix * C4, total = per * n;
    for (size_t i = blockIdx.x * (size_t)blockDim.x + threadIdx.x; i < total; i += (size_t)gridDim.x * blockDim.x) {
        const int k = (int)(i / per);
        const size_t r = i - (size_t)k * per, pix = r / C4;
        const int c = (int)(r - pix * C4) * 4;
        const float *src = k == 0 ? parts.p[0] : k == 1 ? parts.p[1] : k == 2 ? parts.p[2] : k == 3 ? parts.p[3] : k == 4 ? parts.p[4]
                           : k == 5 ? parts.p[5] : k == 6 ? parts.p[6] : parts.p[7];
        float4 v = ld4(src + pix * ld + c);
        if (base) v = f4add(v, ld4(base + i * 4));
        if (mask) {
            const float4 m = ld4(mask + i * 4);
            v.x = m.x > 0.f ? v.x : 0.f, v.y = m.y > 0.f ? v.y : 0.f, v.z = m.z > 0.f ? v.z : 0.f, v.w = m.w > 0.f ? v.w : 0.f;
        }
        st4(out + i * 4, v);
    }
}

static int cat_batch_add(const float *const *parts, int n, size_t npix, int C, int ld, const float *base, const float *mask, float *out, void *stream) {
    RAMNET_CHECK_ARG(parts && out && n >= 1 && n <= 8 && npix > 0 && C > 0 && C % 4 == 0 && ld >= C && ld % 4 == 0);
    CatParts q;
    for (int k = 0; k < 8; ++k) {
        q.p[k] = k < n ? parts[k] : nullptr;
        if (k < n) RAMNET_CHECK_ARG(parts[k] && ((uintptr_t)parts[k] & 15) == 0);
    }
    hipLaunchKernelGGL(cat_batch_add_kernel, dim3(grid_for((size_t)n * npix * (C / 4))), dim3(256), 0, (hipStream_t)stream, q, n, npix, C, ld, base, mask, out);
    RAMNET_LAUNCH_CHECK();
    return 0;
}
extern "C" int ramnet_cat_batch_add(const float *const *parts, int n, size_t npix, int C, int ld, const float *base, float *out, void *stream) {
    return cat_batch_add(parts, n, npix, C, ld, base, nullptr, out, stream);
}
extern "C" int ramnet_cat_batch_add_masked(const float *const *parts, int n, size_t npix, int C, int ld, const float *base, const float *mask, float *out,
                                           void *stream) {
    RAMNET_CHECK_ARG(mask != nullptr && ((uintptr_t)mask & 15) == 0);
    return cat_batch_add(parts, n, npix, C, ld, base, mask, out, stream);
}

extern "C" int ramnet_relu_bwd(const float *dy, const float *y, float *dx, size_t n, void *stream) {
    RAMNET_CHECK_ARG(dy && y && dx);
    hipLaunchKernelGGL(relu_bwd_kernel, dim3(grid_for(n / 4 + 1)), dim3(256), 0, (hipStream_t)stream, dy, y, dx, n);
    RAMNET_LAUNCH_CHECK();
    return 0;
}

extern "C" int ramnet_bias_grad(const float *dy, const float *mask, float *db, size_t npix, int C, void *stream) {
    RAMNET_CHECK_ARG(dy && db && C > 0 && C % 4 == 0 && C <= 1024);
    hipLaunchKernelGGL(bias_grad_kernel, dim3(256), dim3(256), 0, (hipStream_t)stream, dy, mask, db, npix, C);
    RAMNET_LAUNCH_CHECK();
    return 0;
}

extern "C" size_t ramnet_bias_grad_partial_floats(int C) { return C > 0 ? (size_t)256 * C : 0; }
extern "C" int ramnet_bias_grad_ordered(const float *dy, const float *mask, float *db, size_t npix, int C, float *partial, void *stream) {
    RAMNET_CHECK_ARG(dy && db && partial && C > 0 && C % 4 == 0 && C <= 1024);
    hipLaunchKernelGGL(bias_grad_ordered_kernel, dim3(256), dim3(256), 0, (hipStream_t)stream, dy, mask, partial, npix, C);
    hipLaunchKernelGGL(bias_grad_join_kernel, dim3((C + 255) / 256), dim3(256), 0, (hipStream_t)stream, partial, 256, db, C);
    RAMNET_LAUNCH_CHECK();
    return 0;
}

extern "C" int ramnet_concat2(const float *a, int lda, int Ca, const float *b, int ldb, int Cb, float *y, size_t npix, void *stream) {
    RAMNET_CHECK_ARG(a && b && y && Ca > 0 && Cb > 0 && Ca % 4 == 0 && Cb % 4 == 0 && lda % 4 == 0 && ldb % 4 == 0 && lda >= Ca && ldb >= Cb);
    hipLaunchKernelGGL(concat2_kernel, dim3(grid_for(npix * ((Ca + Cb) / 4))), dim3(256), 0, (hipStream_t)stream, a, lda, Ca, b, ldb, Cb, y, npix);
    RAMNET_LAUNCH_CHECK();
    return 0;
}

extern "C" int ramnet_split2(const float *y, int ldy, int Ca, int Cb, float *a, float *b, size_t npix, void *stream) {
    RAMNET_CHECK_ARG(y && a && b && Ca > 0 && Cb > 0 && Ca % 4 == 0 && Cb % 4 == 0 && ldy % 4 == 0 && ldy >= Ca + Cb);
    hipLaunchKernelGGL(split2_kernel, dim3(grid_for(npix * ((Ca + Cb) / 4))), dim3(256), 0, (hipStream_t)stream, y, ldy, Ca, Cb, a, b, npix);
    RAMNET_LAUNCH_CHECK();
    return 0;
}

extern "C" int ramnet_add(const float *a, const float *b, float *y, size_t n, void *stream) {
    RAMNET_CHECK_ARG(a && b && y);
    hipLaunchKernelGGL(add_kernel, dim3(grid_for(n / 4 + 1)), dim3(256), 0, (hipStream_t)stream, a, b, y, n);
    RAMNET_LAUNCH_CHECK();
    return 0;
}

extern "C" int ramnet_pred_sigmoid_fwd(const float *x, int ldx, int C, const float *w, const float *b, float *y, size_t npix, void *stream) {
    RAMNET_CHECK_ARG(x && w && y && C > 0 && C % 4 == 0 && ldx % 4 == 0 && ldx >= C);
    hipLaunchKernelGGL(pred_sigmoid_fwd_kernel<true>, dim3(grid_for(npix * 8)), dim3(256), 0, (hipStream_t)stream, x, ldx, C, w, b, y, npix);
    RAMNET_LAUNCH_CHECK();
    return 0;
}

static int pred_bwd(const float *x, int ldx, int C, const float *w, const float *y, const float *dy, float *dx, int lddx, float *dw, float *db,
                    size_t npix, void *stream) {
    RAMNET_CHECK_ARG(ldx >= C);
    if (dx) RAMNET_CHECK_ARG(lddx % 4 == 0 && lddx >= C);
    int g = grid_for(npix * 8);
    if (g > 512) g = 512;
    hipLaunchKernelGGL(pred_sigmoid_bwd_kernel, dim3(g), dim3(256), 0, (hipStream_t)stream, x, ldx, C, w, y, dy, dx, lddx, dw, db, npix);
    RAMNET_LAUNCH_CHECK();
    return 0;
}
extern "C" int ramnet_pred_sigmoid_bwd(const float *x, int ldx, int C, const float *w, const float *y, const float *dy, float *dx,
                                       int lddx, float *dw, float *db, size_t npix, void *stream) {
    RAMNET_CHECK_ARG(x && w && y && dy && dw && db && C > 0 && C % 4 == 0 && C <= 128 && ldx % 4 == 0);
    return pred_bwd(x, ldx, C, w, y, dy, dx, lddx, dw, db, npix, stream);
}
static int pred_bwd_ordered(const float *x, int ldx, int C, const float *w, const float *y, const float *dy, float *dx, int lddx, float *dw, float *db,
                            size_t npix, float *partial, void *stream) {
    RAMNET_CHECK_ARG(partial && ldx >= C);
    if (dx) RAMNET_CHECK_ARG(lddx % 4 == 0 && lddx >= C);
    int g = grid_for(npix * 8);
    if (g > PRED_BWD_WGS) g = PRED_BWD_WGS;
    hipLaunchKernelGGL(pred_sigmoid_bwd_ordered_kernel, dim3(g), dim3(256), 0, (hipStream_t)stream, x, ldx, C, w, y, dy, dx, lddx, partial, npix);
    hipLaunchKernelGGL(pred_bwd_join_kernel, dim3(1), dim3(256), 0, (hipStream_t)stream, partial, g, C, dw, db);
    RAMNET_LAUNCH_CHECK();
    return 0;
}
extern "C" size_t ramnet_pred_bwd_partial_floats(void) { return (size_t)PRED_BWD_WGS * PRED_BWD_LDP; }
extern "C" int ramnet_pred_sigmoid_bwd_ordered(const float *x, int ldx, int C, const float *w, const float *y, const float *dy, float *dx,
                                               int lddx, float *dw, float *db, size_t npix, float *partial, void *stream) {
    RAMNET_CHECK_ARG(x && w && y && dy && dw && db && C > 0 && C % 4 == 0 && C <= 128 && ldx % 4 == 0);
    return pred_bwd_ordered(x, ldx, C, w, y, dy, dx, lddx, dw, db, npix, partial, stream);
}
extern "C" int ramnet_pred_linear_bwd_ordered(const float *x, int ldx, int C, const float *w, const float *dz, float *dx, int lddx, float *dw,
                                              float *db, size_t npix, float *partial, void *stream) {
    RAMNET_CHECK_ARG(x && w && dz && dw && C > 0 && C % 4 == 0 && C <= 128 && ldx % 4 == 0);
    return pred_bwd_ordered(x, ldx, C, w, nullptr, dz, dx, lddx, dw, db, npix, partial, stream);
}
static int pred_si_grid(size_t seg_pix, int nseg) {
    const size_t groups = (seg_pix + 7) / 8;
    const size_t cap = (size_t)ramnet::g_opt_pred_si_cap / (size_t)(nseg > 0 ? nseg : 1);
    constexpr size_t GPW = PRED_SI_THREADS / 8;
    const size_t trips = (groups + cap * GPW - 1) / (cap * GPW);
    size_t g = (groups + GPW * trips - 1) / (GPW * trips);
    if (g > cap) g = cap;
    return g < 1 ? 1 : (int)g;
}

constexpr int PRED_SI_BWD_LDP = 132;
static size_t pred_si_bwd_tickets() { return 1 + ((size_t)ramnet::g_opt_pred_si_bwd_cap + 31) / 32; }
static size_t pred_si_bwd_doubles() { return ((size_t)ramnet::g_opt_pred_si_bwd_cap * PRED_SI_BWD_LDP + 1) / 2; }
extern "C" size_t ramnet_pred_si_scratch_doubles(size_t seg_pix, int nseg) {
    if (nseg <= 0) return 0;
    const size_t fwd = (size_t)nseg * pred_si_grid(seg_pix, nseg) * 3 + nseg, bwd = pred_si_bwd_doubles();
    return (fwd > bwd ? fwd : bwd) + pred_si_bwd_tickets();
}

extern "C" int ramnet_pred_sigmoid_si_fwd(const float *x, int ldx, int C, const float *w, const float *b, float *y, size_t seg_pix, int nseg,
                                          const float *const *targets, float weight, float lambda, double *scratch, double *stats, float *loss,
                                          void *stream) {
    RAMNET_CHECK_ARG(x && w && y && C > 0 && C % 4 == 0 && ldx % 4 == 0 && ldx >= C && seg_pix > 0);
    RAMNET_CHECK_ARG(nseg >= 1 && nseg <= RAMNET_PRED_SI_MAX_SEGMENTS && targets && scratch && stats && loss);
    PredSiTargets tg;
    for (int i = 0; i < RAMNET_PRED_SI_MAX_SEGMENTS; ++i) tg.t[i] = i < nseg ? targets[i] : nullptr;
    for (int i = 0; i < nseg; ++i) RAMNET_CHECK_ARG(tg.t[i] != nullptr);
    const int g = pred_si_grid(seg_pix, nseg);
    hipLaunchKernelGGL(pred_sigmoid_si_fwd_kernel, dim3(g, nseg), dim3(PRED_SI_THREADS), 0, (hipStream_t)stream, x, ldx, C, w, b, y, seg_pix, tg, weight, lambda,
                       scratch, reinterpret_cast<unsigned long long *>(scratch + (size_t)nseg * g * 3), stats, loss);
    RAMNET_LAUNCH_CHECK();
    return 0;
}

extern "C" int ramnet_pred_sigmoid_si_bwd(const float *x, int ldx, int C, const float *w, const float *y, const float *dy, size_t seg_pix, int nseg,
                                          const float *const *targets, const double *stats, const float *gscale, float weight, float lambda,
                                          float *dx, int lddx, float *dw, float *db, double *scratch, int mask_x, void *stream) {
    RAMNET_CHECK_ARG(x && w && y && dw && db && C > 0 && C % 4 == 0 && C <= 128 && ldx % 4 == 0 && ldx >= C && seg_pix > 0);
    RAMNET_CHECK_ARG(nseg >= 1 && nseg <= RAMNET_PRED_SI_MAX_SEGMENTS && targets && stats && gscale);
    if (dx) RAMNET_CHECK_ARG(lddx % 4 == 0 && lddx >= C);
    PredSiTargets tg;
    for (int i = 0; i < RAMNET_PRED_SI_MAX_SEGMENTS; ++i) tg.t[i] = i < nseg ? targets[i] : nullptr;
    for (int i = 0; i < nseg; ++i) RAMNET_CHECK_ARG(tg.t[i] != nullptr);
    int g = grid_for(seg_pix * 8);
    const int cap = scratch ? ramnet::g_opt_pred_si_bwd_cap : (ramnet::g_opt_pred_si_bwd_cap < 512 ? ramnet::g_opt_pred_si_bwd_cap : 512);
    if (g > cap / nseg) g = cap / nseg;
    if (g < 1) g = 1;
    float *part = reinterpret_cast<float *>(scratch);
    unsigned long long *ticket = scratch ? reinterpret_cast<unsigned long long *>(scratch + ramnet_pred_si_scratch_doubles(seg_pix, nseg) - pred_si_bwd_tickets()) : nullptr;
    hipLaunchKernelGGL(pred_sigmoid_si_bwd_kernel, dim3(g, nseg), dim3(256), 0, (hipStream_t)stream, x, ldx, C, w, y, dy, tg, stats, gscale, weight,
                       lambda, dx, lddx, dw, db, seg_pix, part, PRED_SI_BWD_LDP, ticket, mask_x);
    RAMNET_LAUNCH_CHECK();
    return 0;
}

extern "C" int ramnet_pred_linear_fwd(const float *x, int ldx, int C, const float *w, const float *b, float *z, size_t npix, void *stream) {
    RAMNET_CHECK_ARG(x && w && z && C > 0 && C % 4 == 0 && ldx % 4 == 0 && ldx >= C);
    hipLaunchKernelGGL(pred_sigmoid_fwd_kernel<false>, dim3(grid_for(npix * 8)), dim3(256), 0, (hipStream_t)stream, x, ldx, C, w, b, z, npix);
    RAMNET_LAUNCH_CHECK();
    return 0;
}
extern "C" int ramnet_pred_linear_bwd(const float *x, int ldx, int C, const float *w, const float *dz, float *dx, int lddx, float *dw, float *db,
                                      size_t npix, void *stream) {
    RAMNET_CHECK_ARG(x && w && dz && dw && C > 0 && C % 4 == 0 && C <= 128 && ldx % 4 == 0);
    return pred_bwd(x, ldx, C, w, nullptr, dz, dx, lddx, dw, db, npix, stream);
}

template <int MODE>
static int pred_dgrad(const float *x, int ldx, int C, const float *w, const float *y, const float *dy, size_t seg_pix, int nseg,
                      const float *const *targets, const double *stats, const float *gscale, float weight, float lambda, float *dx, int lddx,
                      int mask_x, void *stream) {
    RAMNET_CHECK_ARG(w && dx && C > 0 && C % 4 == 0 && C <= 128 && lddx % 4 == 0 && lddx >= C && seg_pix > 0);
    RAMNET_CHECK_ARG(nseg >= 1 && nseg <= RAMNET_PRED_SI_MAX_SEGMENTS);
    if (mask_x) RAMNET_CHECK_ARG(x && ldx % 4 == 0 && ldx >= C);
    PredSiTargets tg;
    for (int i = 0; i < RAMNET_PRED_SI_MAX_SEGMENTS; ++i) tg.t[i] = (targets && i < nseg) ? targets[i] : nullptr;
    if (MODE == 2)
        for (int i = 0; i < nseg; ++i) RAMNET_CHECK_ARG(tg.t[i] != nullptr);
    size_t g = (size_t)grid_for(seg_pix * 8);
    if (g > (size_t)(2048 / nseg)) g = (size_t)(2048 / nseg);
    const size_t ldmax = (size_t)(mask_x && ldx > lddx ? ldx : lddx);
    const size_t reach = ((size_t)0x7fffffff / (4 * ldmax)) / 128 * 128;
    RAMNET_CHECK_ARG(reach >= 128);
    size_t chunk = ((seg_pix + g - 1) / g + 127) / 128 * 128;
    if (chunk > reach) chunk = reach;
    g = (seg_pix + chunk - 1) / chunk;
    RAMNET_CHECK_ARG(g <= 0x7fffffff);
    hipLaunchKernelGGL(pred_dgrad_kernel<MODE>, dim3((unsigned)g, nseg), dim3(256), 0, (hipStream_t)stream, w, C, y, dy, tg, stats, gscale, weight,
                       lambda, x, ldx, mask_x, dx, lddx, seg_pix, chunk);
    RAMNET_LAUNCH_CHECK();
    return 0;
}
extern "C" int ramnet_pred_sigmoid_dgrad(int C, const float *w, const float *y, const float *dy, float *dx, int lddx, size_t npix, void *stream) {
    RAMNET_CHECK_ARG(y && dy);
    return pred_dgrad<1>(nullptr, 0, C, w, y, dy, npix, 1, nullptr, nullptr, nullptr, 0.f, 0.f, dx, lddx, 0, stream);
}
extern "C" int ramnet_pred_linear_dgrad(int C, const float *w, const float *dz, float *dx, int lddx, size_t npix, void *stream) {
    RAMNET_CHECK_ARG(dz);
    return pred_dgrad<0>(nullptr, 0, C, w, nullptr, dz, npix, 1, nullptr, nullptr, nullptr, 0.f, 0.f, dx, lddx, 0, stream);
}
extern "C" int ramnet_pred_sigmoid_si_dgrad(const float *x, int ldx, int C, const float *w, const float *y, const float *dy, size_t seg_pix, int nseg,
                                            const float *const *targets, const double *stats, const float *gscale, float weight, float lambda,
                                            float *dx, int lddx, int mask_x, void *stream) {
    RAMNET_CHECK_ARG(y && targets && stats && gscale);
    return pred_dgrad<2>(x, ldx, C, w, y, dy, seg_pix, nseg, targets, stats, gscale, weight, lambda, dx, lddx, mask_x, stream);
}

extern "C" int ramnet_upsample2x_bwd(const float *dup, float *dx, int B, int H, int W, int C, void *stream) {
    RAMNET_CHECK_ARG(dup && dx && B > 0 && H > 0 && W > 0 && C > 0 && C % 4 == 0);
    hipLaunchKernelGGL(upsample2x_bwd_kernel, dim3(grid_for((size_t)B * H * W * (C / 4))), dim3(256), 0, (hipStream_t)stream, dup, dx, B, H, W, C);
    RAMNET_LAUNCH_CHECK();
    return 0;
}

extern "C" int ramnet_pad2_sum(const float *x, const float *skip, float *out, int B, int H, int W, int C, void *stream) {
    RAMNET_CHECK_ARG(x && out && B > 0 && H > 0 && W > 0 && C > 0 && C % 4 == 0);
// ... 97 lines not shown
```

rpg_ramnet_amd/ops.py:

```python
import contextlib
import ctypes as C
import os as _os

import torch
from torch.autograd import Function

from . import _hip as H

_NULL = None
_ABL_SKIP_WGRAD = _os.environ.get("RAMNET_ABL_SKIP_WGRAD") == "1"
if _ABL_SKIP_WGRAD:
    import warnings as _warnings
    _warnings.warn("RAMNET_ABL_SKIP_WGRAD=1: backward-weights launches are SKIPPED — every weight gradient of this process is zero "
                   "(tuning runs only; unset the variable for anything else)", RuntimeWarning)

_WINOGRAD = True
_WINO_MIN_CIN = 32


def set_winograd(on):
    global _WINOGRAD
    _WINOGRAD = bool(on)


_WINO_2X4 = "auto"
_WGRAD_SLABS = True
_WGRAD_2X4 = "auto"


def set_wgrad_slabs(on):
    global _WGRAD_SLABS
    if not on and _DETERMINISTIC:
        raise RuntimeError("set_wgrad_slabs(False) has no deterministic form: the atomic join of the backward-weights tile splits "
                           "contradicts set_deterministic(True)")
    _WGRAD_SLABS = bool(on)


_DETERMINISTIC = False


def set_deterministic(on):
    global _DETERMINISTIC
    if on and not _WGRAD_SLABS:
        raise RuntimeError("set_deterministic(True) needs the slab join of the backward-weights launches: set_wgrad_slabs(True) first")
    if on and not _GRAD_LOSS_BATCHED:
        raise RuntimeError("set_deterministic(True) needs the batched multi-scale gradient loss: set_grad_loss_batched(True) first")
    _DETERMINISTIC = bool(on)
    H.check(H.lib().ramnet_set_option(b"ordered_only", int(_DETERMINISTIC)), "set_option")


def deterministic():
    return _DETERMINISTIC


def not_deterministic(what):
    if _DETERMINISTIC:
        raise RuntimeError("%s has no deterministic form: it joins floating-point partial sums by atomic adds (set_deterministic(True) is on)" % what)



def set_winograd_2x4(mode, min_wgs=None):
    global _WINO_2X4
    assert mode in ("auto", "off", "force")
    _WINO_2X4 = mode
    if min_wgs is not None:
        H.check(H.lib().ramnet_wino2x4_config(int(min_wgs)), "wino2x4_config")
        invalidate_descs()


def get_winograd():
    return _WINOGRAD


_FOLD_UP = True


_FOLD_WINO = True
_FOLD_WINO_MIN_COUT = 32
_FOLD_WINO_WGRAD = True
_SAVE_XPAD = False


def set_fold_winograd_wgrad(on):
    global _FOLD_WINO_WGRAD
    _FOLD_WINO_WGRAD = bool(on)


def set_fold_pair(on):
    H.check(H.lib().ramnet_set_option(b"fold_pair", int(bool(on))), "set_option")
    invalidate_packs()
    invalidate_descs()


_GRU_BWD_FUSED = True


def set_gru_bwd_fused(on):
    global _GRU_BWD_FUSED
    _GRU_BWD_FUSED = bool(on)


_GRU_HR = _os.environ.get("RAMNET_GRU_HR", "1") != "0"


def set_gru_materialize_hr(on):
    global _GRU_HR
    _GRU_HR = bool(on)


_SPLIT_OPERANDS = False


def set_split_operands(on):
    global _SPLIT_OPERANDS
    _SPLIT_OPERANDS = bool(on)
    invalidate_descs()


def get_split_operands():
    return _SPLIT_OPERANDS


_SPLIT_WGRAD = _os.environ.get("RAMNET_SPLIT_WGRAD", "0") == "1"


def set_split_wgrad(on):
    global _SPLIT_WGRAD
    _SPLIT_WGRAD = bool(on)


def get_split_wgrad():
    return _SPLIT_WGRAD


def set_wgrad_winograd_2x4(mode):
    global _WGRAD_2X4
    assert mode in ("auto", "off", "force")
    _WGRAD_2X4 = mode


def set_winograd_split(on):
    H.check(H.lib().ramnet_set_option(b"wino_ksplit", int(on)), "set_option")
    invalidate_descs()


def _fold_pair(Cout, Cin):
    return Cout == 32 and Cin % 32 == 0 and bool(H.lib().ramnet_get_option(b"fold_pair"))


def _fold_wino_ok(Cin, Cout):
    kc = 16 if ((Cout % 64 == 0 and Cin % 16 == 0) or _fold_pair(Cout, Cin)) else 8
    return Cout % 32 == 0 and Cout >= _FOLD_WINO_MIN_COUT and Cin % (2 * kc) == 0


def set_fold_winograd(on):
    global _FOLD_WINO
    _FOLD_WINO = bool(on)


_FOLD_2X3 = "auto"


def set_fold_winograd_2x3(mode):
    global _FOLD_2X3
    assert mode in ("auto", "off", "force")
    _FOLD_2X3 = mode


_FOLD_WGRAD_2X3 = "auto"
_FOLD_WGRAD_VARIANT = {}


def set_fold_winograd_wgrad_2x3(mode):
    global _FOLD_WGRAD_2X3
    assert mode in ("auto", "off", "force")
    _FOLD_WGRAD_2X3 = mode


def _fold_wgrad_2x3(B, Hh, W, Cin, Cout):
    if _FOLD_WGRAD_2X3 == "off":
        return False
    key = (B, Hh, W, Cin, Cout, _FOLD_WGRAD_2X3, _DESC_EPOCH)
    hit = _FOLD_WGRAD_VARIANT.get(key)
    if hit is None:
        d = H.WgradDesc()
        d.algo, d.in_mode, d.stride = H.ALGO_WINOGRAD24, H.IN_PLAIN, 1
        d.B, d.Hin, d.Win, d.Ho, d.Wo, d.HoG, d.WoG = B, Hh + 4, W + 4, Hh, W, 2 * Hh, 2 * W
        d.C0 = d.ld0 = Cin
        d.Cout = d.ldg = d.ldgm = Cout
        hit = _FOLD_WGRAD_VARIANT[key] = bool(H.lib().ramnet_fold_wgrad_variant(C.byref(d), int(_FOLD_WGRAD_2X3 == "force")))
    return hit


def set_fold_upsample(on):
    global _FOLD_UP
    _FOLD_UP = bool(on)


def get_fold_upsample():
    return _FOLD_UP


_RAW_STREAM = getattr(torch._C, "_cuda_getCurrentRawStream", None)
_RAW_DEVICE = getattr(torch._C, "_cuda_getDevice", None)


def _st():
    if _RAW_STREAM is not None and _RAW_DEVICE is not None:
        return C.c_void_p(_RAW_STREAM(_RAW_DEVICE()))
    return C.c_void_p(torch.cuda.current_stream().cuda_stream)


def _p(t, off=0):
    return None if t is None else C.c_void_p(t.data_ptr() + 4 * off)


def dense(t):
    if t is None:
        return None
    B, Hh, W, Cc = t.shape
    s = t.stride()
    ok = (s[3] == 1 or Cc == 1) and s[2] % 4 == 0 and s[1] == W * s[2] and s[0] == Hh * s[1] and t.data_ptr() % 16 == 0
    if ok and t.dtype == torch.float32:
        return t
    return t.contiguous().float()


def ld(t):
    return t.stride(2)


class Taps:
    _cache = {}

    def __init__(self, triples):
        self.n = len(triples)
        assert 1 <= self.n <= 25
        self.dy = (C.c_int8 * 25)(*[t[0] for t in triples])
        self.dx = (C.c_int8 * 25)(*[t[1] for t in triples])
        self.wt = (C.c_uint8 * 25)(*[t[2] for t in triples])
        self.wino = False
        self.head = False
        self.flop_taps = self.n

    @classmethod
    def get(cls, kind, k, pad, py=0, px=0):
        key = (kind, k, pad, py, px)
        if key not in cls._cache:
            if kind in ("conv", "conv_s2d"):
                tr = [(kh - pad, kw - pad, kh * k + kw) for kh in range(k) for kw in range(k)]
            elif kind in ("dgrad1", "dgrad1_s2d"):
                tr = [(pad - kh, pad - kw, kh * k + kw) for kh in range(k) for kw in range(k)]
            elif kind == "dgrad2":
                tr = [((py + pad - kh) // 2, (px + pad - kw) // 2, kh * k + kw)
                      for kh in range(k) for kw in range(k)
                      if (py + pad - kh) % 2 == 0 and (px + pad - kw) % 2 == 0]
            elif kind == "fold":
                tr = [(py + ty, px + tx, (py * 2 + px) * 16 + ty * 4 + tx) for ty in range(4) for tx in range(4)]
            else:
                raise KeyError(kind)
            cls._cache[key] = cls(tr)
            cls._cache[key].wino = kind in ("conv", "dgrad1", "conv_s2d", "dgrad1_s2d") and k == 3 and pad == 1
            cls._cache[key].head = kind == "conv" and k == 5 and pad == 2
            if kind.endswith("_s2d"):
                cls._cache[key].flop_taps = 25.0 / 4.0
            if kind == "fold":
                cls._cache[key].flop_taps = 25
        return cls._cache[key]


def conv_launch(x0, taps, w, out, Cout, active=None, **kw):
    d = _conv_desc(x0, taps, w, out, Cout, **kw)
    if active is not None:
        d.active = _p(active)
    H.check(H.lib().ramnet_conv_launch(C.byref(d), _st()), "ramnet_conv_launch")


def conv_launch_multi(x0, w, out, Cout, classes, **kw):
    arr = (H.ConvDesc * len(classes))()
    if isinstance(w, PackRef):
        w = w.cp.pack(w.transposed, False)
    for i, (taps, Ho, Wo, os_) in enumerate(classes):
        arr[i] = _conv_desc(x0, taps, w, out, Cout, Ho=Ho, Wo=Wo, os=os_, **kw)
    H.check(H.lib().ramnet_conv_launch_multi(arr, len(classes), _st()), "ramnet_conv_launch_multi")


def uses_winograd(taps, w, stride, epi, in_mode, C0, C1):
    return bool(isinstance(w, PackRef) and _WINOGRAD and taps.wino and stride == 1
                and (w.cp.gates == 1 or w.transposed or (epi == H.EPI_LSTM and w.cp.Cout % 16 == 0))
                and (epi != H.EPI_LSTM or w.cp.gates == 4) and in_mode not in (H.IN_UP2X, H.IN_UP2X_SKIP)
                and C0 + C1 >= _WINO_MIN_CIN and (C1 == 0 or C0 % 8 == 0))


_HEAD = True


def set_head_kernel(on):
    global _HEAD
    _HEAD = bool(on)


def get_head_kernel():
    return _HEAD


def uses_head(taps, w, stride, epi, in_mode):
    return bool(isinstance(w, PackRef) and _HEAD and taps.head and stride == 1 and not w.transposed
                and w.cp.gates == 1 and len(w.cp.weights) == 1 and in_mode == H.IN_PLAIN and epi in (H.EPI_LINEAR, H.EPI_RELU)
                and H.lib().ramnet_head_supported(w.cp.Cin, w.cp.Cout))


_DESC_CACHE = {}
_DESC_EPOCH = 0
_DESC_CACHE_ON = _os.environ.get("RAMNET_DESC_CACHE", "1") != "0"


def invalidate_descs():
    global _DESC_EPOCH
    _DESC_EPOCH += 1
    _DESC_CACHE.clear()
    _WDESC_CACHE.clear()


def _sd(t):
    return -1 if t is None else t.stride(2)


def _conv_desc(x0, taps, w, out, Cout, *, stride=1, x1=None, xm=None, xm_off=0, in_mode=H.IN_PLAIN,
               C0=None, C1=0, Hin=None, Win=None, bias=None, epi=H.EPI_LINEAR, beta=0.0, e0=None, e1=None,
               o1=None, o2=None, Ho=None, Wo=None, os=(1, 1, 0, 0), out_off=0, frame=0, out_s2d=0, wino24=False, ws_owner=None):
    is_ref = isinstance(w, PackRef)
    al = out.data_ptr() | (4 * out_off)
    for t in (e0, e1, o1, o2, bias):
        if t is not None:
            al |= t.data_ptr()
    key = (id(taps), id(w.cp) if is_ref else 0, w.transposed if is_ref else -1, id(ws_owner), Cout, stride, in_mode, C0, C1, Hin, Win, epi, beta, Ho,
           Wo, os, out_off, frame, out_s2d, wino24, xm_off, tuple(x0.shape), x0.stride(2), _sd(x1), _sd(xm), out.shape[1], out.shape[2],
           out.stride(2), _sd(e0), _sd(e1), _sd(o1), _sd(o2), bias is None, al & 15, _WINOGRAD, _WINO_2X4, _SPLIT_OPERANDS, _HEAD, _S2D_SPARSE, _S2D_2X4,
           _FOLD_2X3, _DESC_EPOCH, x0.device.index)
    hit = _DESC_CACHE.get(key) if _DESC_CACHE_ON else None
    if hit is not None and (not is_ref or hit[3]() is w.cp) and (ws_owner is None or hit[4]() is ws_owner):
        tmpl, kind, nsplit = hit[0], hit[1], hit[2]
        d = H.ConvDesc.from_buffer_copy(tmpl)
        d.x0, d.x1, d.xm = _p(x0), _p(x1), _p(xm, xm_off)
        d.bias, d.e0, d.e1 = _p(bias), _p(e0), _p(e1)
        d.out, d.o1, d.o2 = _p(out, out_off), _p(o1), _p(o2)
        if kind in ("f23", "f23d"):
            d.w = _p(ws_owner.pack_fold_wino2x3_dgrad() if kind == "f23d" else ws_owner.pack_fold_wino2x3())
        else:
            d.w = _p(w) if kind is None else _p(w.cp.pack(0, "head") if kind == "head" else w.cp.pack(w.transposed, kind))
        if nsplit:
            d.splitk_ws = _p((w.cp if is_ref else ws_owner).splitk_ws(nsplit, x0.device))
        return d
    meta = []
    d = _conv_desc_build(x0, taps, w, out, Cout, meta, stride=stride, x1=x1, xm=xm, xm_off=xm_off, in_mode=in_mode, C0=C0, C1=C1, Hin=Hin, Win=Win,
                         bias=bias, epi=epi, beta=beta, e0=e0, e1=e1, o1=o1, o2=o2, Ho=Ho, Wo=Wo, os=os, out_off=out_off, frame=frame,
                         out_s2d=out_s2d, wino24=wino24, ws_owner=ws_owner)
    import weakref
    if len(_DESC_CACHE) > 4096:
        _DESC_CACHE.clear()
    _DESC_CACHE[key] = (H.ConvDesc.from_buffer_copy(d), meta[0], meta[1], weakref.ref(w.cp) if is_ref else None,
                        weakref.ref(ws_owner) if ws_owner is not None else None)
    return d


def _conv_desc_build(x0, taps, w, out, Cout, meta, *, stride=1, x1=None, xm=None, xm_off=0, in_mode=H.IN_PLAIN,
                     C0=None, C1=0, Hin=None, Win=None, bias=None, epi=H.EPI_LINEAR, beta=0.0, e0=None, e1=None,
                     o1=None, o2=None, Ho=None, Wo=None, os=(1, 1, 0, 0), out_off=0, frame=0, out_s2d=0, wino24=False, ws_owner=None):
    B = x0.shape[0]
    kind, nsplit = None, 0
    d = H.ConvDesc()
    d.x0, d.x1, d.xm = _p(x0), _p(x1), _p(xm, xm_off)
    d.ld0, d.ld1, d.ldm = ld(x0), (ld(x1) if x1 is not None else 0), (ld(xm) if xm is not None else 0)
    d.C0, d.C1, d.in_mode = (x0.shape[3] if C0 is None else C0), C1, in_mode
    d.algo = H.ALGO_DIRECT
    ref = None
    cp = w.cp if isinstance(w, PackRef) else ws_owner
    if isinstance(w, PackRef) and beta == 0.0 and frame == 0 and os == (1, 1, 0, 0) and uses_head(taps, w, stride, epi, in_mode):
        d.algo, d.head_cin = H.ALGO_HEAD, w.cp.Cin
        kind = "head"
        w = w.cp.pack(0, "head")
    elif isinstance(w, PackRef):
        wino = uses_winograd(taps, w, stride, epi, in_mode, d.C0, C1)
        d.algo = H.ALGO_WINOGRAD if wino else H.ALGO_DIRECT
        d.s2d_5x5 = int(wino and isinstance(w.cp, S2DConvParam) and _S2D_SPARSE and (in_mode == H.IN_S2D or out_s2d > 0))
        if (wino and (w.cp.gates == 1 or w.transposed or (epi == H.EPI_LSTM and w.cp.gates == 4)) and os == (1, 1, 0, 0)
                and (_S2D_2X4 or not isinstance(w.cp, S2DConvParam))):
            ref = w
        kind = bool(wino)
        w = w.cp.pack(w.transposed, wino)
    d.B, d.Hin, d.Win = B, (x0.shape[1] if Hin is None else Hin), (x0.shape[2] if Win is None else Win)
    d.ntaps, d.stride = taps.n, stride
    d.dy, d.dx, d.wtap = taps.dy, taps.dx, taps.wt
    d.w, d.bias = _p(w), _p(bias)
    d.Cout = Cout
    d.HoF, d.WoF = out.shape[1], out.shape[2]
    d.Ho, d.Wo = (d.HoF if Ho is None else Ho), (d.WoF if Wo is None else Wo)
    d.osy, d.osx, d.ooy, d.oox = os
    d.epi, d.beta, d.frame, d.out_s2d = epi, beta, frame, out_s2d
    d.e0, d.e1 = _p(e0), _p(e1)
    d.lde0, d.lde1 = (ld(e0) if e0 is not None else 0), (ld(e1) if e1 is not None else 0)
    d.out, d.o1, d.o2 = _p(out, out_off), _p(o1), _p(o2)
    d.ldo, d.ldo1, d.ldo2 = ld(out), (ld(o1) if o1 is not None else 0), (ld(o2) if o2 is not None else 0)
    if wino24:
        d.algo = H.ALGO_WINOGRAD24
    if ref is not None and _WINO_2X4 != "off" and H.lib().ramnet_conv_wino_variant(C.byref(d), int(_WINO_2X4 == "force")):
        d.algo, d.s2d_5x5 = H.ALGO_WINOGRAD_2X4, 0
        kind = "2x4g" if epi == H.EPI_LSTM else "2x4"
        if _SPLIT_OPERANDS and H.lib().ramnet_conv_wino_split_ok(C.byref(d), int(_WINO_2X4 == "force")):
            d.algo, kind = H.ALGO_WINOGRAD_2X4_SPLIT, "2x4s"
        d.w = _p(ref.cp.pack(ref.transposed, kind))
    if wino24 and cp is not None and _FOLD_2X3 != "off" and H.lib().ramnet_fold_wino_variant(C.byref(d), int(_FOLD_2X3 == "force")):
        kind = "f23d" if in_mode == H.IN_PARITY4 else "f23"
        d.algo = H.ALGO_WINOGRAD24_2X3
        d.w = _p(cp.pack_fold_wino2x3_dgrad() if kind == "f23d" else cp.pack_fold_wino2x3())
    if d.algo in (H.ALGO_WINOGRAD, H.ALGO_WINOGRAD24) and cp is not None:
        n = H.lib().ramnet_conv_splitk_floats(C.byref(d))
        if n:
            d.splitk_ws, d.splitk_floats = _p(cp.splitk_ws(n, x0.device)), n
            nsplit = n
    meta[:] = [kind, nsplit]
    return d


_WDESC_CACHE = {}

_LAYOUTS = {
    "direct": (0, None, "ramnet_unpack_wgrad", H.ALGO_DIRECT),
    "wino": (16, "ramnet_wgrad_wino_slabs", "ramnet_unpack_wgrad_wino", H.ALGO_WINOGRAD),
    "wino6": ("ramnet_wgrad_wino2x4_ws_floats", "ramnet_wgrad_wino2x4_slabs", "ramnet_unpack_wgrad_wino2x4", H.ALGO_WINOGRAD_2X4),
    "dsplit": ("ramnet_wgrad_dsplit_ws_floats", "ramnet_wgrad_dsplit_slabs", "ramnet_unpack_wgrad_dsplit", H.ALGO_DIRECT_SPLIT),
}


_FOLD_LAYOUTS = {
    "fold24": (25, True),
    "fold23": (30, "2x3"),
}


def _stamp_layout(dw, kind, slabs, head_cin=0, det_slabs=0):
    dw.wino, dw.wino6, dw.wg_dsplit = kind == "wino", kind == "wino6", kind == "dsplit"
    dw.slabs, dw.head_cin = slabs, head_cin
    dw.det_slabs = det_slabs
    return dw


def _det_slabs(dw):
    return getattr(dw, "det_slabs", 0)


_DET_SLAB_QUERIES = {}


def _det_slab_query(algo, Cin, Cout, k):
    key = (algo, Cin, Cout, k, H.lib().ramnet_get_option(b"wgrad_blocks"))
    if key not in _DET_SLAB_QUERIES:
        _DET_SLAB_QUERIES[key] = _det_slab_query_once(algo, Cin, Cout, k)
    return _DET_SLAB_QUERIES[key]


def _det_slab_query_once(algo, Cin, Cout, k):
    d = H.WgradDesc()
    d.algo, d.in_mode, d.stride, d.B, d.C0, d.Cout = algo, H.IN_PLAIN, 1, 64, Cin, Cout
    if algo in (H.ALGO_WINOGRAD24, H.ALGO_WINOGRAD24_2X3):
        d.Ho, d.Wo, d.Hin, d.Win, d.HoG, d.WoG, d.ntaps = 256, 256, 260, 260, 512, 512, 16
    else:
        d.Ho = d.Wo = d.Hin = d.Win = 512
        d.ntaps = k * k
        for t in range(k * k):
            d.dy[t], d.dx[t] = t // k - k // 2, t % k - k // 2
    return max(1, H.lib().ramnet_wgrad_slabs(C.byref(d)))


def _layout_of(dw):
    kind = ("dsplit" if getattr(dw, "wg_dsplit", False) else "wino6" if getattr(dw, "wino6", False) else
            "wino" if getattr(dw, "wino", False) else "direct")
    return kind, getattr(dw, "slabs", 0)


def _wgrad_desc_build(x0, taps, dout, dw, Cout, stride, x1, xm, xm_off, in_mode, C0, C1, Hin, Win, gmask, dbias, Ho, Wo, gview, dw_off, wino24):
    d = H.WgradDesc()
    d.x0, d.x1, d.xm = _p(x0), _p(x1), _p(xm, xm_off)
    d.ld0, d.ld1, d.ldm = ld(x0), (ld(x1) if x1 is not None else 0), (ld(xm) if xm is not None else 0)
    d.C0, d.C1, d.in_mode = (x0.shape[3] if C0 is None else C0), C1, in_mode
    d.B, d.Hin, d.Win = x0.shape[0], (x0.shape[1] if Hin is None else Hin), (x0.shape[2] if Win is None else Win)
    d.ntaps, d.stride = taps.n, stride
    d.dy, d.dx = taps.dy, taps.dx
    d.dout, d.gmask = _p(dout), _p(gmask)
    d.ldg, d.ldgm = ld(dout), (ld(gmask) if gmask is not None else 0)
    d.Cout, d.Ho, d.Wo = Cout, (dout.shape[1] if Ho is None else Ho), (dout.shape[2] if Wo is None else Wo)
    d.dw, d.dbias = _p(dw, dw_off), _p(dbias)
    if gview is not None:
        d.gsy, d.gsx, d.goy, d.gox, d.HoG, d.WoG = gview
    kind, slabs = _layout_of(dw)
    d.algo = _LAYOUTS[kind][3]
    d.dw_slabs = slabs if (kind != "direct" and _WGRAD_SLABS) else 0
    if _det_slabs(dw) and _WGRAD_SLABS and (kind == "direct" or wino24):
        d.dw_slabs = _det_slabs(dw)
    if wino24:
        d.algo = H.ALGO_WINOGRAD24_2X3 if wino24 == "2x3" else H.ALGO_WINOGRAD24
    hc = getattr(dw, "head_cin", 0)
    if hc and _HEAD and taps.head and stride == 1 and in_mode == H.IN_PLAIN and gview is None and dw_off == 0:
        d.algo, d.head_cin = H.ALGO_HEAD, hc
    if d.algo in (H.ALGO_WINOGRAD, H.ALGO_WINOGRAD_2X4) and C1 and d.C0 % 32:
        raise RuntimeError("Winograd backward-weights needs the concatenation boundary at a multiple of 32 channels")
    return d


def wgrad_launch(x0, taps, dout, dw, Cout, *, stride=1, x1=None, xm=None, xm_off=0, in_mode=H.IN_PLAIN, C0=None,
                 C1=0, Hin=None, Win=None, gmask=None, dbias=None, Ho=None, Wo=None, gview=None, dw_off=0, wino24=False, segs=None, stream=None):
    key = (id(taps), id(dw), _layout_of(dw), _det_slabs(dw), getattr(dw, "head_cin", 0), Cout, stride,
           in_mode, C0, C1, Hin, Win, Ho, Wo, gview, dw_off, wino24, xm_off, tuple(x0.shape), x0.stride(2), _sd(x1), _sd(xm), dout.shape[1],
           dout.shape[2], dout.stride(2), _sd(gmask), _WGRAD_SLABS, _HEAD, x0.device.index)
    tmpl = _WDESC_CACHE.get(key) if _DESC_CACHE_ON else None
    if tmpl is not None:
        d = H.WgradDesc.from_buffer_copy(tmpl)
        d.x0, d.x1, d.xm = _p(x0), _p(x1), _p(xm, xm_off)
        d.dout, d.gmask = _p(dout), _p(gmask)
        d.dw, d.dbias = _p(dw, dw_off), _p(dbias)
    else:
        d = _wgrad_desc_build(x0, taps, dout, dw, Cout, stride, x1, xm, xm_off, in_mode, C0, C1, Hin, Win, gmask, dbias, Ho, Wo, gview, dw_off, wino24)
        if len(_WDESC_CACHE) > 4096:
            _WDESC_CACHE.clear()
        _WDESC_CACHE[key] = H.WgradDesc.from_buffer_copy(d)
    if segs is not None:
        d.nseg, d.segs = len(segs), C.cast(segs, C.POINTER(H.WgradSeg))
    if _ABL_SKIP_WGRAD:
        return
    H.check(H.lib().ramnet_wgrad_launch(C.byref(d), _st() if stream is None else stream), "ramnet_wgrad_launch")


_SIDE = {}
_USE_SIDE = False


def set_wgrad_overlap(on):
    global _USE_SIDE
    _USE_SIDE = bool(on)
    H.check(H.lib().ramnet_set_option(b"wgrad_wino_nf", 2 if _USE_SIDE else 1), "set_option")


_DECODE = {}
_USE_DECODE = False
_DECODE_USED = set()


def set_decoder_overlap(on):
    global _USE_DECODE
    _USE_DECODE = bool(on)


def decoder_overlap():
    return _USE_DECODE


def decode_stream(dev):
    st = _DECODE.get(dev)
    if st is None:
        st = _DECODE[dev] = torch.cuda.Stream(device=dev)
    _DECODE_USED.add(dev)
    return st


_BRANCH = {}
_USE_BRANCH = False


def set_branch_overlap(on):
    global _USE_BRANCH
    _USE_BRANCH = bool(on)


def branch_overlap():
    return _USE_BRANCH


def branch_stream(dev, i):
    st = _BRANCH.get((dev, i))
    if st is None:
        st = _BRANCH[(dev, i)] = torch.cuda.Stream(device=dev)
    return st


def _side_stream(dev):
    st = _SIDE.get(dev)
    if st is None:
        st = _SIDE[dev] = torch.cuda.Stream(device=dev)
    return st


@contextlib.contextmanager
def side_work(tensors, dev):
    if not _USE_SIDE:
        yield
        return
    side = _side_stream(dev)
    side.wait_event(torch.cuda.current_stream().record_event())
    with torch.cuda.stream(side):
        yield
    for t in tensors:
        if t is not None:
            t.record_stream(side)
    _Engine.side_used = dev


def wgrad_side(tensors, *args, **kw):
    if not _USE_SIDE:
        return wgrad_launch(*args, **kw)
    dev = args[0].device
    side = _side_stream(dev)
    raw = C.c_void_p(side.cuda_stream)
    H.check(H.lib().ramnet_stream_fork(_st(), raw), "ramnet_stream_fork")
    wgrad_launch(*args, stream=raw, **kw)
    for t in tensors:
        if t is not None:
            t.record_stream(side)
    _Engine.side_used = dev


_WGRAD_DEFER = 0


def set_wgrad_defer(n):
    global _WGRAD_DEFER
    n = int(n)
    assert 0 <= n <= H.WGRAD_MAX_SEGMENTS
    _WGRAD_DEFER = n


def wgrad_defer():
    return _WGRAD_DEFER


def _wgrad_cell(cp, dw, tensors, x0, taps, dout, Cout, **kw):
    if _WGRAD_DEFER <= 1 or _layout_of(dw)[0] != "wino6" or not _WGRAD_SLABS:
        return wgrad_side(tensors, x0, taps, dout, dw, Cout, **kw)
    x1, xm = kw.get("x1"), kw.get("xm")
    key = (id(dw), tuple(x0.shape), ld(x0), ld(x1) if x1 is not None else 0, ld(xm) if xm is not None else 0, ld(dout), Cout,
           kw.get("in_mode"), kw.get("C1"), kw.get("xm_off", 0), x0.device)
    q = cp._defer
    if q and q[0][0] != key:
        cp.flush_deferred()
    cp._defer.append((key, tensors, x0, taps, dout, dw, Cout, kw))
    if len(cp._defer) >= _WGRAD_DEFER:
        cp.flush_deferred()


_ZERO_BATCH = None


def _zero_later(t):
    if _ZERO_BATCH is None:
        t.zero_()
    else:
        _ZERO_BATCH.append(t)


class _Engine:
    dirty = []
    task = -1
    side_used = None

    @classmethod
    def enter(cls):
        tid = torch._C._current_graph_task_id()
        if tid != cls.task:
            if cls.dirty:
                cls.reset()
            cls.task = tid
            if tid != -1:
                torch.autograd.Variable._execution_engine.queue_callback(cls.flush)

    @classmethod
    def mark(cls, cp):
        cls.enter()
        if not cp._dirty:
            cp._dirty = True
            cls.dirty.append(cp)

    @classmethod
    def _join(cls):
        for dev in _DECODE_USED:
            torch.cuda.current_stream(dev).wait_stream(_DECODE[dev])
        if cls.side_used is not None:
            torch.cuda.current_stream().wait_event(_side_stream(cls.side_used).record_event())
            cls.side_used = None

    @classmethod
    def flush(cls):
        for cp in cls.dirty:
            cp.flush_deferred()
        cls._join()
        dirty, cls.dirty, cls.task = cls.dirty, [], -1
        hook = _FINALIZE_HOOK if (_FINALIZE_HOOK is not None and not (torch.cuda.is_available() and torch.cuda.is_current_stream_capturing())) else None
        if hook is not None:
            hook.begin(dirty)
        global _ZERO_BATCH
        _ZERO_BATCH = []
        try:
            for cp in dirty:
                cp.finalize()
                if hook is not None:
                    hook.finalized(cp)
        finally:
            zs, _ZERO_BATCH = _ZERO_BATCH, None
            zs = [z for z in zs if z.numel() > 0]
            if zs:
                torch._foreach_zero_(zs)
        if hook is not None and hasattr(hook, "end"):
            hook.end()

    @classmethod
    def reset(cls):
        for cp in cls.dirty:
            cp._defer = []
        cls._join()
        dirty, cls.dirty, cls.task = cls.dirty, [], -1
        for cp in dirty:
            cp.discard()


_FINALIZE_HOOK = None

# ... 1819 lines not shown
```

Measured before the change: 246.5 samples/s.

## Add 128-column F(2x3) fold-Winograd conv variant with two-pass weight walk

Adds an NCQ=8 instantiation of the fold Winograd F(2x3) kernel, so each workgroup covers 128 output channels (or two 64-column pair halves) with K=32 chunks. Each chunk is consumed in two weight passes, with a new LDS swizzle. The aim is to reuse each transformed input tile across twice as many output channels, which cuts redundant input transforms and loads. An auto heuristic enables it only when the workgroup wave count does not grow. The cost is fewer workgroups, more LDS and register pressure per workgroup, and no k-split.

```diff
diff --git a/include/ramnet_hip.h b/include/ramnet_hip.h
--- a/include/ramnet_hip.h
+++ b/include/ramnet_hip.h
@@ -143,6 +143,7 @@
 int ramnet_pack_weight_fold_wino_dgrad(const float *w_oihw, float *wp, int Cout, int Cin, void *stream);
 int ramnet_pack_border_weights(const float *w_oihw, float *rows, float *cols, float *rows_t, float *cols_t, int Cout, int Cin, void *stream);
 int ramnet_fold_wino_variant(const ramnet_conv_desc *d, int force);
+int ramnet_fold_wino_n128(const ramnet_conv_desc *d);
 size_t ramnet_packed_weight_elems_fold_wino2x3(int Cout, int Cin);
 int ramnet_pack_weight_fold_wino2x3(const float *w_oihw, float *wp, int Cout, int Cin, void *stream);
 int ramnet_pack_weight_fold_wino2x3_dgrad(const float *w_oihw, float *wp, int Cout, int Cin, void *stream);
diff --git a/rpg_ramnet_amd/_hip.py b/rpg_ramnet_amd/_hip.py
--- a/rpg_ramnet_amd/_hip.py
+++ b/rpg_ramnet_amd/_hip.py
@@ -104,6 +104,7 @@
     "ramnet_pack_weight_fold_wino": (C.c_int, [_fp, _fp, C.c_int, C.c_int, _fp]),
     "ramnet_pack_weight_fold_wino_dgrad": (C.c_int, [_fp, _fp, C.c_int, C.c_int, _fp]),
     "ramnet_fold_wino_variant": (C.c_int, [C.POINTER(ConvDesc), C.c_int]),
+    "ramnet_fold_wino_n128": (C.c_int, [C.POINTER(ConvDesc)]),
     "ramnet_packed_weight_elems_fold_wino2x3": (C.c_size_t, [C.c_int, C.c_int]),
     "ramnet_pack_weight_fold_wino2x3": (C.c_int, [_fp, _fp, C.c_int, C.c_int, _fp]),
     "ramnet_pack_weight_fold_wino2x3_dgrad": (C.c_int, [_fp, _fp, C.c_int, C.c_int, _fp]),
diff --git a/rpg_ramnet_amd/csrc/common.hpp b/rpg_ramnet_amd/csrc/common.hpp
--- a/rpg_ramnet_amd/csrc/common.hpp
+++ b/rpg_ramnet_amd/csrc/common.hpp
@@ -13,7 +13,7 @@
 constexpr int TWID = 16;
 constexpr int WCK = 32;
 
-extern int g_opt_voxel_sorted, g_opt_fold_pair, g_opt_wgrad_blocks, g_opt_wgrad_wino_blocks, g_opt_wino_ksplit, g_opt_wgrad_wino_nf, g_opt_pred_si_cap, g_opt_pred_si_bwd_cap, g_opt_ordered_only;
+extern int g_opt_voxel_sorted, g_opt_fold_pair, g_opt_wgrad_blocks, g_opt_wgrad_wino_blocks, g_opt_wino_ksplit, g_opt_wgrad_wino_nf, g_opt_pred_si_cap, g_opt_pred_si_bwd_cap, g_opt_ordered_only, g_opt_fold_n128;
 void set_error(const char *fmt, ...);
 void note_kernel(const char *fmt, ...);
 int launch_wino(const ramnet_conv_desc &d, hipStream_t st);
diff --git a/rpg_ramnet_amd/csrc/conv_wino24.hip b/rpg_ramnet_amd/csrc/conv_wino24.hip
--- a/rpg_ramnet_amd/csrc/conv_wino24.hip
+++ b/rpg_ramnet_amd/csrc/conv_wino24.hip
@@ -42,20 +42,22 @@
 
 template <int NCQ, bool DG, int TXW, bool PAIR = false, int TW = 2>
 __global__ void __launch_bounds__(512, 1) conv_wino24_kernel(const ramnet_conv_desc p, const Wino24Params q) {
-    static_assert(!PAIR || (NCQ == 4 && !DG), "pair mode: forward, 64-column workgroups");
-    static_assert(TW == 2 || (TW == 3 && NCQ == 4), "F(2x3): 64-column workgroups");
+    static_assert(!PAIR || ((NCQ == 4 || NCQ == 8) && !DG), "pair mode: forward, 64- or 128-column workgroups");
+    static_assert(TW == 2 ? NCQ != 8 : (TW == 3 && NCQ >= 4), "F(2x3): 64- or 128-column workgroups; 128 columns: F(2x3) only");
     constexpr int WC = TW + 3, NP = 5 * WC;
     constexpr int VSZ = NP * W24_PS;
-    constexpr int W24_K = NCQ == 4 ? 16 : 8;
-    constexpr int W24_TX = TXW, W24_TY = (NCQ == 4 ? 32 : 64) / TXW;
-    constexpr int VEC = W24_K / 4;
-    constexpr int W24_U = NP * NCQ * 64 * VEC;
+    constexpr int W24_K = NCQ == 8 ? 32 : NCQ == 4 ? 16 : 8;
+    constexpr int NPASS = NCQ == 8 ? 2 : 1;
+    constexpr int W24_TX = TXW, W24_TY = (NCQ == 8 ? 16 : NCQ == 4 ? 32 : 64) / TXW;
+    constexpr int VEC = W24_K / (4 * NPASS);
+    constexpr int PCQ = NCQ == 8 ? 4 : NCQ;
+    constexpr int W24_U = NP * PCQ * 64 * VEC;
     extern __shared__ __attribute__((aligned(16))) float smem[];
     float *V = smem;
     const int tid = threadIdx.x, lane = tid & 63;
     const int wave = __builtin_amdgcn_readfirstlane(tid >> 6);
     const int l15 = lane & 15, ks = lane >> 4;
-    const int th = NCQ == 4 ? wave & 1 : wave & 3, cq = NCQ == 4 ? wave >> 1 : wave >> 2;
+    const int th = NCQ == 8 ? 0 : NCQ == 4 ? wave & 1 : wave & 3, cq = NCQ == 8 ? wave : NCQ == 4 ? wave >> 1 : wave >> 2;
 
     int bid = blockIdx.x;
     const int cls = DG ? 0 : PAIR ? bid & 1 : bid & 3;
@@ -93,7 +95,9 @@
     const int ksp = (DG || TW != 2) ? 1 : q.ksplit;
     const int cps = ((q.nchunks / 2 + ksp - 1) / ksp) * 2, cbeg = DG ? 0 : (int)blockIdx.y * cps;
     const auto xrs = make_rsrc(q.x + cbeg * W24_K, q.xbytes - (unsigned)cbeg * W24_K * 4u);
-    const int vdst = NCQ == 4 ? it * 16 + (((ik >> 2) ^ ((it >> 2) & 3)) << 2) + (ik & 3) : it * 8 + (((ik >> 1) ^ ((it >> 3) & 1)) << 1) + (ik & 1);
+    const int vdst = NCQ == 8   ? it * 32 + (((ik >> 2) ^ ((it >> 1) & 7)) << 2) + (ik & 3)
+                     : NCQ == 4 ? it * 16 + (((ik >> 2) ^ ((it >> 2) & 3)) << 2) + (ik & 3)
+                                : it * 8 + (((ik >> 1) ^ ((it >> 3) & 1)) << 1) + (ik & 1);
     float raw[5 * WC];
     auto load_raw = [&](int chunk) {
         int soff = chunk * (W24_K * 4);
@@ -152,10 +156,14 @@
     };
 
     const int tile = th * 16 + l15;
-    const int aoff = NCQ == 4 ? tile * 16 + ((ks ^ ((tile >> 2) & 3)) << 2) : tile * 8 + ((ks ^ ((tile >> 3) & 1)) << 1);
-    constexpr int WPOS = NCQ * 64 * VEC;
+    const int aoff = NCQ == 8   ? tile * 32 + ((ks ^ ((tile >> 1) & 7)) << 2)
+                     : NCQ == 4 ? tile * 16 + ((ks ^ ((tile >> 2) & 3)) << 2)
+                                : tile * 8 + ((ks ^ ((tile >> 3) & 1)) << 1);
+    constexpr int WPOS = PCQ * 64 * VEC;
     const auto wrs = make_rsrc(q.wp, q.wbytes);
-    const int wsrc = (((cls * q.nchunks + cbeg) * q.nblk + nb) * W24_U + cq * (64 * VEC)) * 4;
+    const int pnblk = (NCQ == 8 && !PAIR) ? 2 * q.nblk : q.nblk, pnb = (NCQ == 8 && !PAIR) ? 2 * nb + (cq >> 2) : nb;
+    const int pcls = (NCQ == 8 && PAIR) ? 2 * cls + (cq >> 2) : cls, pcq = NCQ == 8 ? cq & 3 : cq;
+    const int wsrc = (((pcls * (q.nchunks * NPASS) + cbeg) * pnblk + pnb) * W24_U + pcq * (64 * VEC)) * 4;
     const int wlane = lane * VEC * 4;
     auto ldv = [&](const float *ptr) {
         if (VEC == 4) return ld4(ptr);
@@ -170,7 +178,7 @@
             return make_float4(t.x, t.y, 0.f, 0.f);
         }
     };
-    const int wchunk = q.nblk * W24_U * 4;
+    const int wchunk = pnblk * W24_U * 4;
     int abuf1 = VSZ + aoff, dbuf1 = VSZ + vdst;
     if constexpr (TW == 3) asm volatile("" : "+v"(abuf1), "+v"(dbuf1));
 
@@ -178,11 +186,11 @@
 #pragma unroll
     for (int i = 0; i < NP; ++i) acc[i] = f32x4{0.f, 0.f, 0.f, 0.f};
 
-    const int nch = DG ? q.nchunks : min(cps, q.nchunks - cbeg);
+    const int nch = (DG || NCQ == 8) ? q.nchunks : min(cps, q.nchunks - cbeg);
     W24_STAMP(16, 0);
     load_raw(0);
     constexpr int RING = TW == 2 || DG ? 10 : 6, DIST = RING - 2;
-    static_assert((2 * NP) % RING == 0, "ring slots repeat every chunk pair");
+    static_assert((2 * NP) % RING == 0 && (NPASS == 1 || NP % RING == 0), "ring slots repeat every chunk pair (128 columns: every walk, the chunk count may be odd)");
     float4 bq[RING];
 #pragma unroll
     for (int i = 0; i < DIST; ++i) bq[i] = ldw(wsrc + i * (WPOS * 4));
@@ -198,58 +206,65 @@
 #pragma unroll
         for (int half = 0; half < 2; ++half) {
             const int chunk = chunk0 + half;
+            if (NCQ == 8 && half && chunk >= nch) break;
             const float *vb = V + half * VSZ;
             float *vn = TW == 2 ? V + (half ^ 1) * VSZ : V + (half ? vdst : dbuf1);
+            int h = 0;
             auto lda = [&](int pos) {
                 if constexpr (TW == 2) return ldv(vb + pos * W24_PS + aoff);
+                else if constexpr (NCQ == 8) return ldv(V + ((half ? abuf1 : aoff) ^ (h << 4)) + pos * W24_PS);
                 else return ldv(V + (half ? abuf1 : aoff) + pos * W24_PS);
             };
             const int cnext = min(chunk + 1, nch - 1), cnext2 = min(chunk + 2, nch - 1);
-            const int wcur = wsrc + chunk * wchunk, wnext = wsrc + cnext * wchunk;
             W24_STAMP(chunk, 0);
-            float4 aq[2][2];
-            aq[0][0] = lda(0), aq[0][1] = lda(1);
-#pragma unroll
-            for (int pp = 0; pp < (NP + 1) / 2; ++pp) {
-                const int pos = 2 * pp, g = half * NP + pos;
-                const bool two = pos + 1 < NP;
-                if (pos + 2 < NP) aq[(pp + 1) & 1][0] = lda(pos + 2);
-                if (pos + 3 < NP) aq[(pp + 1) & 1][1] = lda(pos + 3);
-                const float4 a0 = aq[pp & 1][0], a1 = aq[pp & 1][1];
+#pragma unroll
+            for (h = 0; h < NPASS; ++h) {
+                const int wcur = wsrc + (chunk * NPASS + h) * wchunk, wnext = h + 1 < NPASS ? wcur + wchunk : wsrc + cnext * NPASS * wchunk;
+                float4 aq[2][2];
+                aq[0][0] = lda(0), aq[0][1] = lda(1);
+#pragma unroll
+                for (int pp = 0; pp < (NP + 1) / 2; ++pp) {
+                    const int pos = 2 * pp, g = (half * NPASS + h) * NP + pos;
+                    const bool two = pos + 1 < NP;
+                    if (pos + 2 < NP) aq[(pp + 1) & 1][0] = lda(pos + 2);
+                    if (pos + 3 < NP) aq[(pp + 1) & 1][1] = lda(pos + 3);
+                    const float4 a0 = aq[pp & 1][0], a1 = aq[pp & 1][1];
 #if !defined(W24_ABLATE) || !(W24_ABLATE & 2)
-                bq[(g + DIST) % RING] = pos + DIST < NP ? ldw(wcur + (pos + DIST) * (WPOS * 4)) : ldw(wnext + (pos + DIST - NP) * (WPOS * 4));
-                if (two) bq[(g + 1 + DIST) % RING] = pos + 1 + DIST < NP ? ldw(wcur + (pos + 1 + DIST) * (WPOS * 4)) : ldw(wnext + (pos + 1 + DIST - NP) * (WPOS * 4));
+                    bq[(g + DIST) % RING] = pos + DIST < NP ? ldw(wcur + (pos + DIST) * (WPOS * 4)) : ldw(wnext + (pos + DIST - NP) * (WPOS * 4));
+                    if (two) bq[(g + 1 + DIST) % RING] = pos + 1 + DIST < NP ? ldw(wcur + (pos + 1 + DIST) * (WPOS * 4)) : ldw(wnext + (pos + 1 + DIST - NP) * (WPOS * 4));
 #endif
-                const float4 b0 = bq[g % RING], b1 = bq[(g + 1) % RING];
-                __builtin_amdgcn_sched_barrier(0);
-                acc[pos] = __builtin_amdgcn_mfma_f32_16x16x4f32(a0.x, b0.x, acc[pos], 0, 0, 0);
-                if (two) acc[pos + 1] = __builtin_amdgcn_mfma_f32_16x16x4f32(a1.x, b1.x, acc[pos + 1], 0, 0, 0);
-                acc[pos] = __builtin_amdgcn_mfma_f32_16x16x4f32(a0.y, b0.y, acc[pos], 0, 0, 0);
-                if (two) acc[pos + 1] = __builtin_amdgcn_mfma_f32_16x16x4f32(a1.y, b1.y, acc[pos + 1], 0, 0, 0);
-                __builtin_amdgcn_sched_barrier(0);
-                constexpr int R0 = 4 + WC;
-                auto slot = [&](int sl) {
-                    if (sl == 4) W24_STAMP(chunk, 1);
-                    if (sl >= 4 && sl < R0) tr_col(sl - 4);
-                    if (sl == R0) W24_STAMP(chunk, 2);
-                    if (sl >= R0 && sl <= R0 + 8 && !((sl - R0) & 1)) tr_row(vn, (sl - R0) >> 1);
+                    const float4 b0 = bq[g % RING], b1 = bq[(g + 1) % RING];
+                    __builtin_amdgcn_sched_barrier(0);
+                    acc[pos] = __builtin_amdgcn_mfma_f32_16x16x4f32(a0.x, b0.x, acc[pos], 0, 0, 0);
+                    if (two) acc[pos + 1] = __builtin_amdgcn_mfma_f32_16x16x4f32(a1.x, b1.x, acc[pos + 1], 0, 0, 0);
+                    acc[pos] = __builtin_amdgcn_mfma_f32_16x16x4f32(a0.y, b0.y, acc[pos], 0, 0, 0);
+                    if (two) acc[pos + 1] = __builtin_amdgcn_mfma_f32_16x16x4f32(a1.y, b1.y, acc[pos + 1], 0, 0, 0);
+                    __builtin_amdgcn_sched_barrier(0);
+                    constexpr int R0 = 4 + WC;
+                    auto slot = [&](int sl) {
+                        if (sl == 4) W24_STAMP(chunk, 1);
+                        if (sl >= 4 && sl < R0) tr_col(sl - 4);
+                        if (sl == R0) W24_STAMP(chunk, 2);
+                        if (sl >= R0 && sl <= R0 + 8 && !((sl - R0) & 1)) tr_row(vn, (sl - R0) >> 1);
 #if !defined(W24_ABLATE) || !(W24_ABLATE & 1)
-                    if (sl == R0 + 1) load_row_begin(cnext2);
-                    if (sl > R0 && sl <= R0 + 9 && ((sl - R0) & 1)) load_row((sl - R0 - 1) >> 1);
+                        if (sl == R0 + 1) load_row_begin(cnext2);
+                        if (sl > R0 && sl <= R0 + 9 && ((sl - R0) & 1)) load_row((sl - R0 - 1) >> 1);
 #endif
-                    if (sl == R0 + 9) W24_STAMP(chunk, 3);
-                };
-                slot(2 * pp);
-                __builtin_amdgcn_sched_barrier(0);
-                if (VEC == 4) {
-                    acc[pos] = __builtin_amdgcn_mfma_f32_16x16x4f32(a0.z, b0.z, acc[pos], 0, 0, 0);
-                    if (two) acc[pos + 1] = __builtin_amdgcn_mfma_f32_16x16x4f32(a1.z, b1.z, acc[pos + 1], 0, 0, 0);
-                    acc[pos] = __builtin_amdgcn_mfma_f32_16x16x4f32(a0.w, b0.w, acc[pos], 0, 0, 0);
-                    if (two) acc[pos + 1] = __builtin_amdgcn_mfma_f32_16x16x4f32(a1.w, b1.w, acc[pos + 1], 0, 0, 0);
+                        if (sl == R0 + 9) W24_STAMP(chunk, 3);
+                    };
+                    if constexpr (NPASS == 1) slot(2 * pp);
+                    else slot(h * (NP / 2) + pp);
+                    __builtin_amdgcn_sched_barrier(0);
+                    if (VEC == 4) {
+                        acc[pos] = __builtin_amdgcn_mfma_f32_16x16x4f32(a0.z, b0.z, acc[pos], 0, 0, 0);
+                        if (two) acc[pos + 1] = __builtin_amdgcn_mfma_f32_16x16x4f32(a1.z, b1.z, acc[pos + 1], 0, 0, 0);
+                        acc[pos] = __builtin_amdgcn_mfma_f32_16x16x4f32(a0.w, b0.w, acc[pos], 0, 0, 0);
+                        if (two) acc[pos + 1] = __builtin_amdgcn_mfma_f32_16x16x4f32(a1.w, b1.w, acc[pos + 1], 0, 0, 0);
+                    }
+                    __builtin_amdgcn_sched_barrier(0);
+                    if constexpr (NPASS == 1) slot(2 * pp + 1);
+                    __builtin_amdgcn_sched_barrier(0);
                 }
-                __builtin_amdgcn_sched_barrier(0);
-                slot(2 * pp + 1);
-                __builtin_amdgcn_sched_barrier(0);
             }
             W24_STAMP(chunk, 4);
             __syncthreads();
@@ -259,7 +274,7 @@
     W24_STAMP(16, 2);
 
     const int ncol = n0 + cq * 16 + l15;
-    const int pxc = PAIR ? ncol >> 5 : px, n = PAIR ? ncol & 31 : ncol;
+    const int pxc = PAIR ? (NCQ == 8 ? cq >> 2 : ncol >> 5) : px, n = PAIR ? (NCQ == 8 ? nb * 64 + (cq & 3) * 16 + l15 : ncol & 31) : ncol;
     if (n >= p.Cout) return;
     const int epi = p.epi;
     const float bias_n = (!DG && p.bias) ? p.bias[n] : 0.f;
@@ -433,6 +448,56 @@
     return 0;
 }
 
+static long wino23n_tile(int Ho, int Wt, int &tx) {
+    const int shapes[3] = {4, 2, 8};
+    long best = -1;
+    for (int s = 0; s < 3; ++s) {
+        const int t = shapes[s], th = 2 * (16 / t), tw = 3 * t;
+        const long a = (long)cdiv(Ho, th) * th * cdiv(Wt, tw) * tw;
+        if (best < 0 || a < best) best = a, tx = t;
+    }
+    return best;
+}
+
+static int fold_wino_n128_form(const ramnet_conv_desc &d) {
+    if (d.algo != RAMNET_ALGO_WINOGRAD24_2X3 || d.stride != 1 || d.C0 % 32 != 0) return 0;
+    if (d.in_mode == RAMNET_IN_PARITY4) return d.Cout % 128 == 0 ? 1 : 0;
+    if (d.in_mode != RAMNET_IN_PLAIN || fold_wino_pair(d.Cout, d.C0) || d.Cout % 64 != 0) return 0;
+    return d.Cout % 128 == 0 ? 1 : 2;
+}
+
+static long fold_wino23_wgs(const ramnet_conv_desc &d, bool n128) {
+    const int form = fold_wino_n128_form(d);
+    const bool dg = d.in_mode == RAMNET_IN_PARITY4, pair = n128 ? form == 2 : fold_wino_pair(d.Cout, d.C0);
+    const int Wt = pair ? d.Wo + 1 : d.Wo;
+    int tx;
+    const long tiles = n128 ? wino23n_tile(d.Ho, Wt, tx) / 96 : wino23_tile(d.Ho, Wt, tx) / 192;
+    const int nblk = n128 ? (form == 2 ? d.Cout / 64 : d.Cout / 128) : (pair ? 1 : d.Cout / 64);
+    return tiles * d.B * nblk * (dg ? 1 : pair ? 2 : 4);
+}
+
+static int fold_wino_n128(const ramnet_conv_desc &d) {
+    const int form = fold_wino_n128_form(d);
+    if (!form || !g_opt_fold_n128) return 0;
+    if (g_opt_fold_n128 == 2) return form;
+    const long w128 = fold_wino23_wgs(d, true), w64 = fold_wino23_wgs(d, false);
+    return w128 >= 256 && (w128 + 255) / 256 <= (w64 + 255) / 256 ? form : 0;
+}
+
+template <bool DG, bool PAIR>
+static int launch_wino23n(int tx, dim3 grid, size_t lds, const ramnet_conv_desc &d, const Wino24Params &q, hipStream_t st) {
+#define W23N_GO(T)                                                                                                        \
+    if (tx == T) {                                                                                                        \
+        RAMNET_FULL_LDS((conv_wino24_kernel<8, DG, T, PAIR, 3>));                                                           \
+        note_kernel("conv_wino24_kernel<8,%d,%d,%d,3>", (int)DG, T, (int)PAIR);                                            \
+        hipLaunchKernelGGL((conv_wino24_kernel<8, DG, T, PAIR, 3>), grid, dim3(512), lds, st, d, q);                        \
+    }
+    W23N_GO(2) W23N_GO(4) W23N_GO(8)
+#undef W23N_GO
+    RAMNET_LAUNCH_CHECK();
+    return 0;
+}
+
 static int launch_wino24_dgrad(const ramnet_conv_desc &d, hipStream_t st) {
     RAMNET_CHECK_ARG(d.stride == 1 && d.C0 % 16 == 0 && d.Cout % 64 == 0);
     RAMNET_CHECK_ARG(d.Hin % 2 == 0 && d.Win % 2 == 0 && d.Ho == d.Hin / 2 + 4 && d.Wo == d.Win / 2 + 4 && d.HoF == d.Ho && d.WoF == d.Wo);
@@ -446,6 +511,13 @@
     const size_t xb = (size_t)d.B * d.Hin * d.Win * d.ld0 * sizeof(float), wb = (size_t)(w23 ? 120 : 100) * d.C0 * d.Cout * sizeof(float);
     RAMNET_CHECK_ARG(xb < 0x40000000ull && wb < 0x7fffffffull);
     q.xbytes = (unsigned)xb, q.wbytes = (unsigned)wb;
+    if (w23 && fold_wino_n128(d)) {
+        int tx;
+        wino23n_tile(d.Ho, d.Wo, tx);
+        q.cpc = d.C0 / 32, q.nchunks = 4 * q.cpc, q.nblk = d.Cout / 128;
+        q.tiles_x = cdiv(d.Wo, 3 * tx), q.tiles_y = cdiv(d.Ho, 32 / tx);
+        return launch_wino23n<true, false>(tx, dim3((unsigned)(q.tiles_x * q.tiles_y * d.B * q.nblk)), (size_t)2 * W23_V * sizeof(float), d, q, st);
+    }
     if (w23) {
         int tx;
         wino23_tile(d.Ho, d.Wo, tx);
@@ -536,6 +608,17 @@
     const size_t xb = (size_t)d.B * d.Hin * d.Win * d.ld0 * sizeof(float), wb = (size_t)(w23 ? 120 : 100) * d.C0 * d.Cout * sizeof(float);
     RAMNET_CHECK_ARG(xb < 0xffffffffull && wb < 0x7fffffffull);
     q.xbytes = (unsigned)xb, q.wbytes = (unsigned)wb;
+    if (const int form = w23 ? fold_wino_n128(d) : 0) {
+        const bool pair128 = form == 2;
+        int tx;
+        wino23n_tile(d.Ho, pair128 ? d.Wo + 1 : d.Wo, tx);
+        q.nchunks = d.C0 / 32, q.nblk = pair128 ? d.Cout / 64 : d.Cout / 128;
+        q.tiles_x = cdiv(pair128 ? d.Wo + 1 : d.Wo, 3 * tx), q.tiles_y = cdiv(d.Ho, 32 / tx);
+        q.ksplit = 1, q.ws = nullptr, q.cnt = nullptr;
+        const dim3 grid((unsigned)(q.tiles_x * q.tiles_y * d.B * q.nblk * (pair128 ? 2 : 4)));
+        const size_t lds = (size_t)2 * W23_V * sizeof(float);
+        return pair128 ? launch_wino23n<false, true>(tx, grid, lds, d, q, st) : launch_wino23n<false, false>(tx, grid, lds, d, q, st);
+    }
     if (w23) {
         int tx;
         wino23_tile(d.Ho, pair ? d.Wo + 1 : d.Wo, tx);
@@ -724,6 +807,8 @@
 
 extern "C" int ramnet_fold_wino_variant(const ramnet_conv_desc *d, int force) { return d ? fold_wino_variant(*d, force) : 0; }
 
+extern "C" int ramnet_fold_wino_n128(const ramnet_conv_desc *d) { return d ? fold_wino_n128(*d) : 0; }
+
 extern "C" int ramnet_pack_border_weights(const float *w, float *rows, float *cols, float *rows_t, float *cols_t, int Cout, int Cin, void *stream) {
     RAMNET_CHECK_ARG(w && rows && cols && rows_t && cols_t && Cout > 0 && Cin > 0);
     const size_t total = (size_t)2 * 5 * Cin * 2 * Cout;
diff --git a/rpg_ramnet_amd/csrc/pointwise.hip b/rpg_ramnet_amd/csrc/pointwise.hip
--- a/rpg_ramnet_amd/csrc/pointwise.hip
+++ b/rpg_ramnet_amd/csrc/pointwise.hip
@@ -958,7 +958,7 @@
 extern "C" int ramnet_abi_version(void) { return RAMNET_ABI_VERSION; }
 
 namespace ramnet {
-int g_opt_voxel_sorted = 1, g_opt_fold_pair = 1, g_opt_wgrad_blocks = 512, g_opt_wgrad_wino_blocks = 384, g_opt_wino_ksplit = 1, g_opt_wgrad_wino_nf = 1, g_opt_pred_si_cap = 256, g_opt_pred_si_bwd_cap = 1024, g_opt_ordered_only = 0;
+int g_opt_voxel_sorted = 1, g_opt_fold_pair = 1, g_opt_wgrad_blocks = 512, g_opt_wgrad_wino_blocks = 384, g_opt_wino_ksplit = 1, g_opt_wgrad_wino_nf = 1, g_opt_pred_si_cap = 256, g_opt_pred_si_bwd_cap = 1024, g_opt_ordered_only = 0, g_opt_fold_n128 = 1;
 }
 extern "C" int ramnet_set_option(const char *name, int value) {
     RAMNET_CHECK_ARG(name != nullptr);
@@ -971,6 +971,7 @@
     else if (!strcmp(name, "pred_si_bwd_cap")) { RAMNET_CHECK_ARG(value >= 8 && value <= 65536); ramnet::g_opt_pred_si_bwd_cap = value; }
     else if (!strcmp(name, "pred_si_cap")) { RAMNET_CHECK_ARG(value >= 8 && value <= 65536); ramnet::g_opt_pred_si_cap = value; }
     else if (!strcmp(name, "ordered_only")) ramnet::g_opt_ordered_only = value != 0;
+    else if (!strcmp(name, "fold_n128")) { RAMNET_CHECK_ARG(value >= 0 && value <= 2); ramnet::g_opt_fold_n128 = value; }
     else RAMNET_CHECK_ARG(!"ramnet_set_option: unknown option");
     return 0;
 }
@@ -985,6 +986,7 @@
     if (!strcmp(name, "pred_si_bwd_cap")) return ramnet::g_opt_pred_si_bwd_cap;
     if (!strcmp(name, "pred_si_cap")) return ramnet::g_opt_pred_si_cap;
     if (!strcmp(name, "ordered_only")) return ramnet::g_opt_ordered_only;
+    if (!strcmp(name, "fold_n128")) return ramnet::g_opt_fold_n128;
     return -1;
 }
 
diff --git a/rpg_ramnet_amd/ops.py b/rpg_ramnet_amd/ops.py
--- a/rpg_ramnet_amd/ops.py
+++ b/rpg_ramnet_amd/ops.py
@@ -165,6 +165,16 @@
     global _FOLD_2X3
     assert mode in ("auto", "off", "force")
     _FOLD_2X3 = mode
+
+
+_FOLD_N128 = "auto"
+
+
+def set_fold_winograd_n128(mode):
+    global _FOLD_N128
+    assert mode in ("auto", "off", "force")
+    H.check(H.lib().ramnet_set_option(b"fold_n128", {"off": 0, "auto": 1, "force": 2}[mode]), "set_option")
+    _FOLD_N128 = mode
 
 
 _FOLD_WGRAD_2X3 = "auto"
@@ -337,7 +347,7 @@
     key = (id(taps), id(w.cp) if is_ref else 0, w.transposed if is_ref else -1, id(ws_owner), Cout, stride, in_mode, C0, C1, Hin, Win, epi, beta, Ho,
            Wo, os, out_off, frame, out_s2d, wino24, xm_off, tuple(x0.shape), x0.stride(2), _sd(x1), _sd(xm), out.shape[1], out.shape[2],
            out.stride(2), _sd(e0), _sd(e1), _sd(o1), _sd(o2), bias is None, al & 15, _WINOGRAD, _WINO_2X4, _SPLIT_OPERANDS, _HEAD, _S2D_SPARSE, _S2D_2X4,
-           _FOLD_2X3, _DESC_EPOCH, x0.device.index)
+           _FOLD_2X3, _FOLD_N128, _DESC_EPOCH, x0.device.index)
     hit = _DESC_CACHE.get(key) if _DESC_CACHE_ON else None
     if hit is not None and (not is_ref or hit[3]() is w.cp) and (ws_owner is None or hit[4]() is ws_owner):
         tmpl, kind, nsplit = hit[0], hit[1], hit[2]
@@ -360,7 +370,7 @@
     if len(_DESC_CACHE) > 4096:
         _DESC_CACHE.clear()
     _DESC_CACHE[key] = (H.ConvDesc.from_buffer_copy(d), meta[0], meta[1], weakref.ref(w.cp) if is_ref else None,
-                        weakref.ref(ws_owner) if ws_owner is not None else None)
+                        weakref.ref(ws_owner) if ws_owner is not None else None, meta[2])
     return d
 
 
@@ -368,7 +378,7 @@
                      C0=None, C1=0, Hin=None, Win=None, bias=None, epi=H.EPI_LINEAR, beta=0.0, e0=None, e1=None,
                      o1=None, o2=None, Ho=None, Wo=None, os=(1, 1, 0, 0), out_off=0, frame=0, out_s2d=0, wino24=False, ws_owner=None):
     B = x0.shape[0]
-    kind, nsplit = None, 0
+    kind, nsplit, n128 = None, 0, 0
     d = H.ConvDesc()
     d.x0, d.x1, d.xm = _p(x0), _p(x1), _p(xm, xm_off)
     d.ld0, d.ld1, d.ldm = ld(x0), (ld(x1) if x1 is not None else 0), (ld(xm) if xm is not None else 0)
@@ -414,12 +424,13 @@
         kind = "f23d" if in_mode == H.IN_PARITY4 else "f23"
         d.algo = H.ALGO_WINOGRAD24_2X3
         d.w = _p(cp.pack_fold_wino2x3_dgrad() if kind == "f23d" else cp.pack_fold_wino2x3())
+        n128 = H.lib().ramnet_fold_wino_n128(C.byref(d))
     if d.algo in (H.ALGO_WINOGRAD, H.ALGO_WINOGRAD24) and cp is not None:
         n = H.lib().ramnet_conv_splitk_floats(C.byref(d))
         if n:
             d.splitk_ws, d.splitk_floats = _p(cp.splitk_ws(n, x0.device)), n
             nsplit = n
-    meta[:] = [kind, nsplit]
+    meta[:] = [kind, nsplit, n128]
     return d
 
 
```

After: 247.6 samples/s (median of 6 runs). No clear change (+0.4%).
